# MAC-VO/MAC-VO

Measured on AMD Instinct MI355X. Metric: stereo frames/sec at 640x480 (hot path: cost volume + lookup, keypoint selection, covariance, PGO), higher is better.
Workload: dtype f32 via f16x2 (volume: fp32 operands row-scaled by powers of two and split into two fp16 pieces, three products, fp32 accumulate, scales undone exactly) + f32 (lookup/covariance) + f64 (PGO)

## Files before the change

include/macvo_hip.h:

```cpp
#ifndef MACVO_HIP_H
#define MACVO_HIP_H

#include <stddef.h>
#include <stdint.h>

#ifdef __cplusplus
extern "C" {
#endif

typedef void* mvStream_t;

enum {
    MV_OK = 0,
    MV_ERR_INVALID_ARG = -1,
    MV_ERR_UNSUPPORTED = -2,
    MV_ERR_LAUNCH = -3,
    MV_ERR_WORKSPACE = -4
};

enum {
    MV_F32 = 0,
    MV_F16 = 1,
    MV_BF16 = 2,
    MV_BF16X3 = 3,
// ... 23 lines not shown
int mv_cost_patch_embed_supported(int H2, int W2);
int mv_cost_patch_embed(const float* cost_maps, const void* packed, float* out, int S, int H2, int W2, int token_layout, int operand_type,
                        mvStream_t stream);
int mv_cost_patch_embed_t(const void* cost_maps, int in_dtype, const void* packed, void* out, int out_dtype, int S, int H2, int W2, int token_layout,
                          int operand_type, mvStream_t stream);
size_t mv_volume_pack_bytes(int B, int C, int N, int mode);
int mv_volume_pack(const float* f1, const float* f2, void* packed1, void* packed2, int B, int C, int N1, int N2, int layout,
                   int mode, mvStream_t stream);
int mv_volume_pack_tiled(const float* f1, const float* f2, void* packed1, void* packed2, int B, int C, int N1, int H2, int W2,
                         int layout, int mode, mvStream_t stream);
int mv_corr_volume_packed_supported(int B, int C, int N1, int N2, int mode);
int mv_corr_volume_packed(const void* packed1, const void* packed2, float* out, int B, int C, int N1, int N2, int mode,
                          mvStream_t stream);
int mv_corr_volume_packed_shared(const void* packed1, const void* packed2, float* out, int B, int C, int N1, int N2, int mode, int free_cus,
                                 mvStream_t stream);

const char* mv_corr_volume_last_kernel(void);

int mv_corr_lookup(const float* vol, const float* coords, float* out, int B, int H1, int W1,
                   int H2, int W2, int radius, mvStream_t stream);

int mv_corr_volume_out16_supported(int B, int C, int N1, int N2, int in_dtype, int layout);
int mv_corr_volume_out16(const void* f1, const void* f2, void* out, int B, int C, int N1, int N2, int in_dtype, int layout, mvStream_t stream);
int mv_corr_lookup_vol16(const void* vol_f16, const float* coords, float* out, int B, int H1, int W1, int H2, int W2, int radius,
                         mvStream_t stream);

int mv_corr_lookup_tiled(const float* vol, const float* coords, float* out, int B, int H1, int W1,
                         int H2, int W2, int radius, mvStream_t stream);

int mv_tiled_slice_cells(int H, int W);
int mv_fmap_tile_rows16(const void* f, void* out, int B, int C, int H, int W, mvStream_t stream);
int mv_corr_lookup_tiled_vol16(const void* vol_f16, const float* coords, float* out, int B, int H1, int W1, int H2, int W2, int radius,
                               mvStream_t stream);

int mv_frontend_epilogue(const float* flow, const float* logcov, int cov_is_log, int H, int W,
                         float bl_fx, float bl_fx_sq, float* disparity, float* disparity_cov,
                         float* depth, float* depth_cov, uint8_t* bad_mask, float* match_flow,
                         float* match_cov, mvStream_t stream);

int mv_convex_upsample(const float* flow, const float* mask, float* out, int B, int h, int w,
                       float mask_scale, int exp2_out, mvStream_t stream);
int mv_convex_upsample_m(const float* flow, const void* mask, int mask_dtype, float* out, int B, int h, int w,
                         float mask_scale, int exp2_out, mvStream_t stream);

enum { MV_KP_NODEPTH = 0, MV_KP_FULL = 1, MV_KP_MAPPING = 2,
       MV_KP_RANDOM = 3,
       MV_KP_GRID = 4,
       MV_KP_EXPLICIT = 5
};

typedef struct {
    int32_t H, W;
    int32_t mode;
    int32_t kernel_size;
    int32_t mask_width;
    float max_depth;
    float max_depth_cov;
    float max_match_cov;
} mvKpSelectParams;

size_t mv_kp_select_workspace_bytes(int H, int W);

int mv_kp_select(const float* flow_cov, const float* depth0, const float* depth0_cov,
                 const float* depth1, const float* depth1_cov, const uint8_t* mask_a,
                 const uint8_t* mask_b, const mvKpSelectParams* params , void* workspace,
                 size_t workspace_bytes, int32_t* out_cand, int32_t* out_count, float* out_stats,
// ... 210 lines not shown
    const float *kp0, *kp1;
    const float* vals;
    const float *sigma0, *sigma1;
    const double *cov0, *cov1;
    const float* pos_Tw;
    const double* cov0_world;
    const uint8_t* color;
    const float* K;
    const float* T_BS;
    const float* prior_pose;
    float baseline;
} mvMapFrameLanes;
int mv_map_append_lanes(const mvMapFrameLanes* frames , const mvMapStores* stores_dev , mvStream_t stream);
int mv_map_append_skipped_lanes(const mvMapStores* stores_dev , int lanes, const float* K_dev, const float* T_BS_dev, const float* pose_dev,
                                float baseline, const int64_t* time_ns , mvStream_t stream);
int mv_map_set_pose_lanes(const mvMapStores* stores_dev , int lanes, int frame_idx, const float* pose_dev, mvStream_t stream);

int mv_frontend_epilogue_lanes(const float* flow, const float* logcov, int cov_is_log, int H, int W, float bl_fx,
                               float bl_fx_sq, float* disparity, float* disparity_cov, float* depth, float* depth_cov,
                               uint8_t* bad_mask, float* match_flow, float* match_cov, int lanes, mvStream_t stream);
int mv_kp_select_lanes(const float* flow_cov, const float* depth0, const float* depth0_cov, const float* depth1,
                       const float* depth1_cov, const uint8_t* mask_a, const uint8_t* mask_b,
                       const mvKpSelectParams* params , void* workspace, size_t workspace_bytes,
                       int32_t* out_cand , int32_t* out_count ,
                       float* out_stats , int lanes, mvStream_t stream);
int mv_pose_apply_lanes(const float* pose, const float* pos_Tc, const double* cov, int lanes, const int32_t* n_live ,
                        int cap, float* pos_Tw, double* rot, double* cov_rot, mvStream_t stream);
int mv_frontend_epilogue_select_lanes(const float* flow, const float* logcov, int cov_is_log, float bl_fx, float bl_fx_sq,
                                      float* disparity, float* disparity_cov, float* depth, float* depth_cov,
                                      uint8_t* bad_mask, float* match_flow, float* match_cov, const uint8_t* mask_a,
                                      const uint8_t* mask_b, const mvKpSelectParams* params , void* workspace,
                                      size_t workspace_bytes, int32_t* out_cand, int32_t* out_count, float* out_stats,
                                      int lanes, mvStream_t stream);
int mv_kp_gather_lanes(const int32_t* cand, size_t cand_lane_stride, const int64_t* perm , int lanes,
                       const int32_t* n_live , int cap, int W, int64_t* out_uv ,
                       mvStream_t stream);
int mv_kp_front_lanes(const int32_t* cand, size_t cand_lane_stride, const int64_t* perm_dev, const int64_t* perm_host ,
                      int lanes, const int32_t* n_live , int cap, const float* match_flow, const float* match_cov,
                      const float* depth0, const float* disp0, const float* sdisp0, const float* sdd0, const float* depth1,
                      const float* disp1, const float* sdisp1, const float* sdd1, int H, int W, int edge, float match_cov_default,
                      float fx, float fy, float cx, float cy, int64_t* out_kp0_uv , float* out_kp0,
                      float* out_kp1, uint8_t* out_inbound, float* out_vals , float* out_sigma0,
                      float* out_sigma1, float* out_pos_Tc , mvStream_t stream);
int mv_backend_front_lanes(const int32_t* cand, size_t cand_lane_stride, const int64_t* perm_dev, const int64_t* perm_host, int lanes,
                           const int32_t* n_live, int cap, const float* match_flow, const float* match_cov, const float* depth0,
                           const float* disp0, const float* sdisp0, const float* sdd0, const float* depth1, const float* disp1,
                           const float* sdisp1, const float* sdd1, int edge, float match_cov_default, const mvMatchCovParams* cov_params,
                           int64_t* out_kp0_uv, float* out_kp0, float* out_kp1, uint8_t* out_inbound, float* out_vals, float* out_sigma0,
                           float* out_sigma1, float* out_pos_Tc, double* out_cov0, double* out_cov1, mvStream_t stream);
int mv_backend_front_draw_lanes(const int32_t* cand, size_t cand_lane_stride, const int32_t* count_dev, int count_stride, const uint32_t* state_in,
                                uint32_t* state_out, int num_point, int lanes, int cap, const float* match_flow, const float* match_cov,
                                const float* depth0, const float* disp0, const float* sdisp0, const float* sdd0, const float* depth1,
                                const float* disp1, const float* sdisp1, const float* sdd1, int edge, float match_cov_default,
                                const mvMatchCovParams* cov_params, int64_t* out_perm, int32_t* out_live, int64_t* out_kp0_uv, float* out_kp0,
                                float* out_kp1, uint8_t* out_inbound, float* out_vals, float* out_sigma0, float* out_sigma1, float* out_pos_Tc,
                                double* out_cov0, double* out_cov1, mvStream_t stream);
int mv_kp_track_lanes(const int64_t* kp0_uv, int lanes, const int32_t* n_live , int cap, const float* match_flow,
                      const float* match_cov, const float* depth0, const float* disp0, const float* sdisp0,
                      const float* sdd0, const float* depth1, const float* disp1, const float* sdisp1, const float* sdd1,
                      int H, int W, int edge, float match_cov_default, float* out_kp0, float* out_kp1,
                      uint8_t* out_inbound, float* out_vals , float* out_sigma0, float* out_sigma1,
                      mvStream_t stream);
int mv_backproject_lanes(const float* kp_uv, const float* depth_vals, int depth_stride, size_t depth_lane_stride, float fx,
                         float fy, float cx, float cy, const float* pose, int lanes, const int32_t* n_live ,
                         int cap, float* pos_Tc, float* pos_Tw, double* rot, mvStream_t stream);
int mv_match_cov_pair_lanes(const float* depth_map0, const float* kp_uv0, float* flow_cov0, const double* rot0,
// ... 44 lines not shown
typedef struct {
    const void* fmap1;
    const void* fmap2;
    const float* coords;
    const float* flow;
    const float* logcov;
    const float* flow8;
    const float* cov8;
    const float* up_mask;
    const float* cov_mask;
} mvFrameInputs;

enum {
    MV_FB_VOLUME = 0, MV_FB_TOKENS, MV_FB_DISPARITY, MV_FB_DISPARITY_COV, MV_FB_DEPTH, MV_FB_DEPTH_COV, MV_FB_MATCH_FLOW,
    MV_FB_MATCH_COV, MV_FB_CAND, MV_FB_COUNT, MV_FB_STATS,
    MV_FB_KP0, MV_FB_KP0F, MV_FB_KP1, MV_FB_INBOUND, MV_FB_VALS, MV_FB_SIGMA0, MV_FB_SIGMA1, MV_FB_POS_TC, MV_FB_POS_TW,
    MV_FB_ROT, MV_FB_COV0, MV_FB_COV0W, MV_FB_COV1, MV_FB_VALID, MV_FB_NVALID, MV_FB_POSE64, MV_FB_INFO,
    MV_FB_POSE,
    MV_FB_MAP_UV, MV_FB_MAP_D, MV_FB_MAP_SDD, MV_FB_MAP_TC, MV_FB_MAP_TW, MV_FB_MAP_COV , MV_FB_MAP_COLOR ,
    MV_FB_PERM, MV_FB_LIVE,
    MV_FB_MOTION_IN, MV_FB_PRIOR
};

size_t mv_frame_pipe_arena_bytes(const mvFramePipeConfig* cfg);
int mv_frame_pipe_max_pending(void);
int mv_frame_pipe_default_depth(int lanes, int mapping);
int mv_frame_pipe_create(const mvFramePipeConfig* cfg, void* arena, size_t arena_bytes, mvFramePipe** out);
void mv_frame_pipe_destroy(mvFramePipe* p);
int mv_frame_pipe_set_pose(mvFramePipe* p, const float* pose7_host);
int mv_frame_pipe_enqueue(mvFramePipe* p, const mvFrameInputs* in, mvStream_t in_stream, int with_selector);
int mv_frame_pipe_wait_motion_input(mvFramePipe* p, mvStream_t stream);
int mv_frame_pipe_set_motion(mvFramePipe* p, const float* motion_dev, mvStream_t stream);
int mv_frame_pipe_enqueue_volume(mvFramePipe* p, const mvFrameInputs* in, mvStream_t in_stream);
int mv_frame_pipe_wait_candidates(mvFramePipe* p, int32_t* n_cand );
int mv_frame_pipe_finish(mvFramePipe* p, const int64_t* perm_host, const int32_t* n_sel, float* pose_sink);
int mv_frame_pipe_wait_tracked(mvFramePipe* p, int32_t* n_valid, int32_t* n_cand_map);
int mv_frame_pipe_map_points(mvFramePipe* p, const int64_t* perm_host, int n_sel, const float* image_dev,
                             const mvMapStores* stores );
int mv_frame_pipe_seed_lanes(mvFramePipe* p, const uint64_t* seeds );
int mv_randperm_heads(uint64_t seed, const int64_t* n, int calls, int k, int64_t* out);
int mv_frame_pipe_finish_seeded(mvFramePipe* p, float* pose_sink, int32_t* n_cand_out, int32_t* n_sel_out);
int mv_randperm_state_words(void);
int mv_randperm_max_head(void);
int mv_mt19937_seed(uint64_t seed, uint32_t* state_host);
int mv_randperm_head_lanes(uint32_t* state, const int32_t* n_dev, int n_stride, int lanes, int k, int cap, int64_t* out_perm, int32_t* out_n_sel,
                           int n_sel_stride, mvStream_t stream);
int mv_randperm_heads_emulated(uint64_t seed, const int64_t* n, int calls, int k, int threads, int64_t* out);
int mv_frame_pipe_device_draw(const mvFramePipe* p);
int mv_frame_pipe_volume_tiled(const mvFramePipe* p);
int mv_frame_pipe_host_threads(const mvFramePipe* p);
int mv_frame_pipe_finish_device(mvFramePipe* p, float* pose_sink);
int mv_kp_random_max_point(void);
int mv_kp_random_lanes(uint32_t* state, int lanes, int num_point, int H, int W, int mask_width, int64_t* out_uv, mvStream_t stream);
int mv_kp_random_emulated(uint64_t seed, int calls, int num_point, int H, int W, int mask_width, int threads, int64_t* out);
int mv_kp_random_then_randperm_emulated(uint64_t seed, int calls, int num_point, int H, int W, int mask_width, int threads, int64_t* out, int64_t perm_n,
                                        int perm_k, int64_t* out_perm);
int mv_kp_random_heads(uint64_t seed, int calls, int num_point, int H, int W, int mask_width, int64_t* out);
int mv_kp_grid_count(int H, int W, int mask_width, int num_point);
int mv_kp_grid(int H, int W, int mask_width, int num_point, int64_t* out_uv, mvStream_t stream);
#define MV_KP_TABLE_MAX 4096
int mv_frame_pipe_table_rows(const mvFramePipeConfig* cfg);
int mv_frame_pipe_finish_keypoints(mvFramePipe* p, const int64_t* kp_uv_host, const int32_t* n_sel, float* pose_sink);
int mv_frame_pipe_finish_keypoints_dev(mvFramePipe* p, const int64_t* kp_uv_dev, const int32_t* n_sel_dev, mvStream_t stream, float* pose_sink);
int mv_frame_pipe_finished_counts(mvFramePipe* p, int age, int32_t* n_cand, int32_t* n_sel);
int mv_frame_pipe_wait_finished(mvFramePipe* p, int lag);
int mv_frame_pipe_map_append(mvFramePipe* p, const mvMapStores* stores , int frame_idx, int prev_frame,
// ... 26 lines not shown
```

mac-vo_amd/_lib.py:

```python
from __future__ import annotations

import ctypes as C
import os
import threading

_HERE = os.path.dirname(os.path.abspath(__file__))
LIB_PATH = os.path.join(_HERE, "libmacvo_hip.so")

MV_OK = 0
MV_F32, MV_F16, MV_BF16, MV_BF16X3, MV_BF16X2, MV_PACK_BF16X3, MV_PACK_F16X2 = 0, 1, 2, 3, 4, 5, 6
MV_VOL_ENC16 = 16
MV_LAYOUT_CHW, MV_LAYOUT_HWC = 0, 1
MV_KP_NODEPTH, MV_KP_FULL, MV_KP_MAPPING = 0, 1, 2
MV_KP_RANDOM, MV_KP_GRID, MV_KP_EXPLICIT = 3, 4, 5
MV_KP_TABLE_MAX = 4096
MV_GRAPH_ICP, MV_GRAPH_REPROJ, MV_GRAPH_DISP = 0, 1, 2
MV_COV_MATCH, MV_COV_GMM, MV_COV_NONE = 0, 1, 2
MV_COVMOD_DIAG, MV_COVMOD_NORMALIZE = 1, 2
MV_MOTION_STATIC, MV_MOTION_TARTAN = 0, 1
MV_SOLVE_WORLD, MV_SOLVE_LOCAL = 0, 1
MV_NOCOV_DEPTH, MV_NOCOV_MATCH = 1, 2
ABI_VERSION = 8
MV_MAX_LANES = 64

# ... 27 lines not shown

class mvFramePipeConfig(C.Structure):
    _fields_ = [(n, C.c_int32) for n in (
        "H", "W", "C", "pairs", "iters", "radius", "feat_dtype", "layout", "volume_split", "selector_mode",
        "kp_kernel_size", "kp_mask_width", "num_point", "edgewidth", "min_num_point", "graph_type", "filters",
        "cov_kernel_size", "mapping", "map_num_point", "map_mask_width", "async_backend")] + [(n, C.c_float) for n in (
        "fx", "fy", "cx", "cy", "baseline", "bl_fx", "bl_fx_sq", "match_cov_default", "max_match_cov", "max_depth_cov",
        "max_depth", "min_flow_cov_sq", "min_depth_cov", "filter_min_depth", "map_max_depth", "map_max_depth_cov")] + [("lm", mvLMParams)] + [
        (n, C.c_int32) for n in ("cov_model", "cov_modifiers", "motion_model", "frontend_nocov")] + [("cov_match_cov_default", C.c_float)]


class mvMapStores(C.Structure):
    _fields_ = [(n, C.c_void_p) for n in (
        "K", "baseline", "pose", "T_BS", "need_interp", "time_ns", "pos_Tw", "cov_Tw", "color",
        "pixel1_uv", "pixel2_uv", "pixel1_d", "pixel2_d", "pixel1_disp", "pixel2_disp", "pixel1_disp_cov", "pixel2_disp_cov",
        "obs1_covTc", "obs2_covTc", "pixel1_uv_cov", "pixel2_uv_cov", "pixel1_d_cov", "pixel2_d_cov",
        "frame2match_ranges", "frame2match_num", "frame2map_ranges", "frame2map_num", "match2frame1", "match2frame2",
        "match2point", "point2match_edges", "point2match_deg", "counts")] + [("max_pt_obs", C.c_int32), ("max_frame_range", C.c_int32)] + \
        [("cap_frames", C.c_int64), ("cap_match", C.c_int64), ("cap_points", C.c_int64)] + \
        [("mp_pos_Tw", C.c_void_p), ("mp_cov_Tw", C.c_void_p), ("mp_color", C.c_void_p), ("cap_map_points", C.c_int64)]


class mvMapFrame(C.Structure):
    _fields_ = [("n_rows", C.c_int32), ("table_stride", C.c_int32), ("prev_frame", C.c_int32), ("min_num_point", C.c_int32)] + \
        [(n, C.c_void_p) for n in ("valid", "kp0", "kp1", "vals", "sigma0", "sigma1", "cov0", "cov1", "pos_Tw", "cov0_world",
                                   "color", "K", "T_BS", "prior_pose")] + \
        [("baseline", C.c_float), ("time_ns", C.c_int64), ("out_frame_idx", C.c_void_p)]


class mvMapFrameLanes(C.Structure):
    _fields_ = [("lanes", C.c_int32), ("cap", C.c_int32), ("prev_frame", C.c_int32), ("min_num_point", C.c_int32)] + \
        [(n, C.c_void_p) for n in ("n_rows", "time_ns", "valid", "kp0", "kp1", "vals", "sigma0", "sigma1", "cov0", "cov1", "pos_Tw", "cov0_world",
                                   "color", "K", "T_BS", "prior_pose")] + [("baseline", C.c_float)]


class mvFrameInputs(C.Structure):
    _fields_ = [(n, C.c_void_p) for n in ("fmap1", "fmap2", "coords", "flow", "logcov", "flow8", "cov8", "up_mask",
                                          "cov_mask")]


FB_NAMES = ("VOLUME", "TOKENS", "DISPARITY", "DISPARITY_COV", "DEPTH", "DEPTH_COV", "MATCH_FLOW", "MATCH_COV", "CAND",
            "COUNT", "STATS", "KP0", "KP0F", "KP1", "INBOUND", "VALS", "SIGMA0", "SIGMA1", "POS_TC", "POS_TW", "ROT", "COV0",
            "COV0W", "COV1", "VALID", "NVALID", "POSE64", "INFO", "POSE", "MAP_UV", "MAP_D", "MAP_SDD", "MAP_TC", "MAP_TW", "MAP_COV",
            "MAP_COLOR", "PERM", "LIVE", "MOTION_IN", "PRIOR")
FB = {n: i for i, n in enumerate(FB_NAMES)}

_P = C.c_void_p
SIGNATURES = {
    "mv_abi_version": (C.c_int, []),
    "mv_error_string": (C.c_char_p, [C.c_int]),
    "mv_corr_volume": (C.c_int, [_P, _P, _P, C.c_int, C.c_int, C.c_int, C.c_int, C.c_int, C.c_int, _P]),
    "mv_split_bf16x3": (C.c_int, [_P, _P, C.c_size_t, _P]),
    "mv_corr_volume_last_kernel": (C.c_char_p, []),
    "mv_volume_pack_bytes": (C.c_size_t, [C.c_int, C.c_int, C.c_int, C.c_int]),
    "mv_volume_pack": (C.c_int, [_P, _P, _P, _P, C.c_int, C.c_int, C.c_int, C.c_int, C.c_int, C.c_int, _P]),
    "mv_corr_volume_packed_supported": (C.c_int, [C.c_int, C.c_int, C.c_int, C.c_int, C.c_int]),
    "mv_corr_volume_packed": (C.c_int, [_P, _P, _P, C.c_int, C.c_int, C.c_int, C.c_int, C.c_int, _P]),
    "mv_corr_volume_packed_shared": (C.c_int, [_P, _P, _P, C.c_int, C.c_int, C.c_int, C.c_int, C.c_int, C.c_int, _P]),
    "mv_corr_lookup": (C.c_int, [_P, _P, _P, C.c_int, C.c_int, C.c_int, C.c_int, C.c_int, C.c_int, _P]),
    "mv_corr_lookup_tiled": (C.c_int, [_P, _P, _P, C.c_int, C.c_int, C.c_int, C.c_int, C.c_int, C.c_int, _P]),
    "mv_corr_lookup_vol16": (C.c_int, [_P, _P, _P, C.c_int, C.c_int, C.c_int, C.c_int, C.c_int, C.c_int, _P]),
    "mv_corr_lookup_tiled_vol16": (C.c_int, [_P, _P, _P, C.c_int, C.c_int, C.c_int, C.c_int, C.c_int, C.c_int, _P]),
    "mv_fmap_tile_rows16": (C.c_int, [_P, _P, C.c_int, C.c_int, C.c_int, C.c_int, _P]),
    "mv_tiled_slice_cells": (C.c_int, [C.c_int, C.c_int]),
    "mv_corr_volume_out16_supported": (C.c_int, [C.c_int, C.c_int, C.c_int, C.c_int, C.c_int, C.c_int]),
    "mv_corr_volume_out16": (C.c_int, [_P, _P, _P, C.c_int, C.c_int, C.c_int, C.c_int, C.c_int, C.c_int, _P]),
    "mv_volume_pack_tiled": (C.c_int, [_P, _P, _P, _P, C.c_int, C.c_int, C.c_int, C.c_int, C.c_int, C.c_int, C.c_int, _P]),
    "mv_frontend_epilogue": (C.c_int, [_P, _P, C.c_int, C.c_int, C.c_int, C.c_float, C.c_float,
                                       _P, _P, _P, _P, _P, _P, _P, _P]),
    "mv_convex_upsample": (C.c_int, [_P, _P, _P, C.c_int, C.c_int, C.c_int, C.c_float, C.c_int, _P]),
    "mv_convex_upsample_m": (C.c_int, [_P, _P, C.c_int, _P, C.c_int, C.c_int, C.c_int, C.c_float, C.c_int, _P]),
    "mv_kp_select_workspace_bytes": (C.c_size_t, [C.c_int, C.c_int]),
    "mv_kp_select": (C.c_int, [_P, _P, _P, _P, _P, _P, _P, C.POINTER(mvKpSelectParams), _P, C.c_size_t,
                               _P, _P, _P, _P]),
    "mv_kp_gather": (C.c_int, [_P, _P, C.c_int, C.c_int, _P, _P]),
    "mv_kp_track": (C.c_int, [_P, C.c_int, _P, _P, _P, _P, _P, _P, _P, _P, _P, _P, C.c_int, C.c_int, C.c_int,
                              C.c_float, _P, _P, _P, _P, _P, _P, _P]),
    "mv_match_cov": (C.c_int, [_P, _P, _P, _P, _P, C.POINTER(mvMatchCovParams), C.c_int, _P, _P, _P, _P]),
    "mv_match_cov_pair": (C.c_int, [_P, _P, _P, _P, _P, _P, _P, _P, _P, _P, C.POINTER(mvMatchCovParams), C.c_int, _P]),
    "mv_obs_cov": (C.c_int, [C.c_int, C.c_int32, _P, _P, _P, _P, _P, _P, C.POINTER(mvMatchCovParams), C.c_int, _P, _P, _P, _P]),
    "mv_obs_cov_pair_lanes": (C.c_int, [C.c_int, C.c_int32] + [_P] * 12 + [C.POINTER(mvMatchCovParams), C.c_int, _P, C.c_int, _P]),
    "mv_obs_cov_pair_nomatch_lanes": (C.c_int, [C.c_int, C.c_int32] + [_P] * 11 + [C.c_float, _P, C.POINTER(mvMatchCovParams), C.c_int, _P, C.c_int, _P]),
    "mv_motion_input_lanes": (C.c_int, [C.c_int, C.c_int, C.c_int, _P, C.c_longlong, _P, C.c_longlong] + [C.c_float] * 5 + [_P, _P]),
    "mv_pose_exp_compose": (C.c_int, [C.c_int, _P, _P, C.c_longlong, _P, _P, _P]),
    "mv_pgo_solve_posed_motion": (C.c_int, [C.c_int, _P, _P, C.c_int, C.c_int] + [_P] * 15 + [C.c_int, C.c_float, C.c_float, _P, _P, _P, _P, C.c_int,
                                                                                         C.POINTER(mvLMParams)] + [_P] * 5),
    "mv_pgo_solve_posed_motion_dev": (C.c_int, [C.c_int, _P, _P, C.c_int, C.c_int, C.c_int] + [_P] * 15 + [C.c_int, C.c_float, C.c_float, _P, _P, _P, _P,
                                                                                                         C.c_int, C.POINTER(mvLMParams)] + [_P] * 5),
    "mv_frame_pipe_wait_motion_input": (C.c_int, [_P, _P]),
    "mv_frame_pipe_set_motion": (C.c_int, [_P, _P, _P]),
    "mv_lm_default_params": (None, [C.POINTER(mvLMParams)]),
    "mv_pgo_solve": (C.c_int, [C.c_int, _P, C.c_int, _P, _P, _P, _P, _P, _P, _P, _P, _P, _P, _P, _P, C.c_int,
                               C.POINTER(mvLMParams), _P, _P, _P, _P]),
    "mv_pgo_solve_posed": (C.c_int, [C.c_int, _P, _P, C.c_int, C.c_int] + [_P] * 14 + [C.c_int, C.c_float, C.c_float, _P, _P, _P, _P, C.c_int,
                                     C.POINTER(mvLMParams)] + [_P] * 5),
    "mv_pgo_solve_posed_dev": (C.c_int, [C.c_int, _P, _P, C.c_int, C.c_int, C.c_int] + [_P] * 14 + [C.c_int, C.c_float, C.c_float, _P, _P, _P, _P, C.c_int,
                                         C.POINTER(mvLMParams)] + [_P] * 5),
    "mv_pgo_solve_local": (C.c_int, [C.c_int, _P, C.c_int, _P, _P, _P, _P, _P, _P, _P, _P, _P, _P, _P, _P, _P, C.c_int,
                                     C.POINTER(mvLMParams), _P, _P, _P, _P]),
    "mv_pgo_solve_posed_local": (C.c_int, [C.c_int, _P, _P, C.c_int, C.c_int] + [_P] * 16 + [C.c_int, C.c_float, C.c_float, _P, _P, _P, _P, C.c_int,
                                           C.POINTER(mvLMParams)] + [_P] * 5),
    "mv_pgo_solve_posed_local_dev": (C.c_int, [C.c_int, _P, _P, C.c_int, C.c_int, C.c_int] + [_P] * 16 + [C.c_int, C.c_float, C.c_float, _P, _P, _P, _P, C.c_int,
                                               C.POINTER(mvLMParams)] + [_P] * 5),
    "mv_backend_front_draw_lanes": (C.c_int, [_P, C.c_size_t, _P, C.c_int, _P, _P, C.c_int, C.c_int, C.c_int] + [_P] * 10 +
                                    [C.c_int, C.c_float, C.POINTER(mvMatchCovParams)] + [_P] * 13),
    "mv_backend_front_lanes": (C.c_int, [_P, C.c_size_t, _P, _P, C.c_int, _P, C.c_int] + [_P] * 10 + [C.c_int, C.c_float, C.POINTER(mvMatchCovParams)] +
                               [_P] * 11),
    "mv_backproject": (C.c_int, [_P, _P, C.c_int, C.c_float, C.c_float, C.c_float, C.c_float, _P, C.c_int,
                                 _P, _P, _P, _P]),
    "mv_obs_filter": (C.c_int, [_P, _P, _P, _P, C.c_int, C.c_float, C.c_float, C.c_int, _P, _P, _P]),
    "mv_map_points": (C.c_int, [_P, C.c_int, _P, _P, _P, C.c_int, C.c_int, C.c_float, C.c_float, C.c_float, C.c_float, _P,
                                C.c_float, _P, _P, _P, _P, _P, _P, _P, _P]),
    "mv_local_corr81": (C.c_int, [_P, _P, _P, C.c_int, C.c_int, C.c_int, C.c_int, _P]),
    "mv_map_append": (C.c_int, [C.POINTER(mvMapFrame), C.POINTER(mvMapStores), _P]),
    "mv_body_poses": (C.c_int, [_P, _P, C.c_int, _P, _P]),
    "mv_motion_interpolate": (C.c_int, [_P, _P, C.c_int, _P, _P, _P]),
    "mv_frontend_epilogue_lanes": (C.c_int, [_P, _P, C.c_int, C.c_int, C.c_int, C.c_float, C.c_float,
                                             _P, _P, _P, _P, _P, _P, _P, C.c_int, _P]),
    "mv_pose_apply_lanes": (C.c_int, [_P, _P, _P, C.c_int, _P, C.c_int, _P, _P, _P, _P]),
    "mv_frontend_epilogue_select_lanes": (C.c_int, [_P, _P, C.c_int, C.c_float, C.c_float, _P, _P, _P, _P, _P, _P, _P, _P, _P,
                                                    C.POINTER(mvKpSelectParams), _P, C.c_size_t, _P, _P, _P, C.c_int, _P]),
    "mv_kp_select_lanes": (C.c_int, [_P, _P, _P, _P, _P, _P, _P, C.POINTER(mvKpSelectParams), _P, C.c_size_t,
                                     _P, _P, _P, C.c_int, _P]),
    "mv_kp_gather_lanes": (C.c_int, [_P, C.c_size_t, _P, C.c_int, _P, C.c_int, C.c_int, _P, _P]),
    "mv_kp_track_lanes": (C.c_int, [_P, C.c_int, _P, C.c_int, _P, _P, _P, _P, _P, _P, _P, _P, _P, _P, C.c_int, C.c_int,
                                    C.c_int, C.c_float, _P, _P, _P, _P, _P, _P, _P]),
    "mv_backproject_lanes": (C.c_int, [_P, _P, C.c_int, C.c_size_t, C.c_float, C.c_float, C.c_float, C.c_float, _P,
                                       C.c_int, _P, C.c_int, _P, _P, _P, _P]),
    "mv_match_cov_pair_lanes": (C.c_int, [_P, _P, _P, _P, _P, _P, _P, _P, _P, _P, C.POINTER(mvMatchCovParams), C.c_int, _P,
                                          C.c_int, _P]),
    "mv_obs_filter_lanes": (C.c_int, [_P, _P, _P, _P, C.c_int, C.c_float, C.c_float, C.c_int, _P, C.c_int, _P, _P, _P]),
    "mv_patch_embed_packed_bytes": (C.c_size_t, []),
    "mv_patch_embed_pack": (C.c_int, [_P, _P, _P, _P, _P, _P, _P, C.c_int, _P]),
    "mv_cost_patch_embed_supported": (C.c_int, [C.c_int, C.c_int]),
    "mv_cost_patch_embed": (C.c_int, [_P, _P, _P, C.c_int, C.c_int, C.c_int, C.c_int, C.c_int, _P]),
    "mv_cost_patch_embed_t": (C.c_int, [_P, C.c_int, _P, _P, C.c_int, C.c_int, C.c_int, C.c_int, C.c_int, C.c_int, _P]),
    "mv_frame_pipe_arena_bytes": (C.c_size_t, [C.POINTER(mvFramePipeConfig)]),
    "mv_frame_pipe_max_pending": (C.c_int, []),
    "mv_frame_pipe_default_depth": (C.c_int, [C.c_int, C.c_int]),
    "mv_frame_pipe_create": (C.c_int, [C.POINTER(mvFramePipeConfig), _P, C.c_size_t, C.POINTER(_P)]),
    "mv_frame_pipe_destroy": (None, [_P]),
    "mv_frame_pipe_set_pose": (C.c_int, [_P, _P]),
    "mv_frame_pipe_enqueue": (C.c_int, [_P, C.POINTER(mvFrameInputs), _P, C.c_int]),
    "mv_frame_pipe_enqueue_volume": (C.c_int, [_P, C.POINTER(mvFrameInputs), _P]),
    "mv_frame_pipe_wait_candidates": (C.c_int, [_P, _P]),
    "mv_frame_pipe_finish": (C.c_int, [_P, _P, _P, _P]),
    "mv_map_append_points": (C.c_int, [_P, C.c_int, _P, _P, _P, _P]),
    "mv_map_append_skipped": (C.c_int, [C.POINTER(mvMapStores), _P, _P, _P, C.c_float, C.c_int64, _P]),
    "mv_frame_pipe_set_solve_frame": (C.c_int, [_P, C.c_int]),
    "mv_frame_pipe_skip": (C.c_int, [_P]),
    "mv_frame_pipe_map_skip": (C.c_int, [_P, C.POINTER(mvMapStores), C.c_int, _P, _P, C.c_float, C.c_int64]),
    "mv_kp_front_lanes": (C.c_int, [_P, C.c_size_t, _P, _P, C.c_int, _P, C.c_int] + [_P] * 10 + [C.c_int, C.c_int, C.c_int] +
                          [C.c_float] * 5 + [_P] * 8 + [_P]),
    "mv_frame_pipe_wait_tracked": (C.c_int, [_P, _P, _P]),
    "mv_frame_pipe_map_points": (C.c_int, [_P, _P, C.c_int, _P, _P]),
    "mv_frame_pipe_seed_lanes": (C.c_int, [_P, _P]),
    "mv_frame_pipe_finish_seeded": (C.c_int, [_P, _P, _P, _P]),
    "mv_frame_pipe_map_append": (C.c_int, [_P, C.POINTER(mvMapStores), C.c_int, C.c_int, _P, _P, C.c_float, C.c_int64, _P]),
    "mv_frame_pipe_release": (C.c_int, [_P, _P]),
    "mv_frame_pipe_sync": (C.c_int, [_P, _P, C.c_int]),
    "mv_frame_pipe_time_volume": (C.c_int, [_P, C.c_int]),
    "mv_frame_pipe_volume_times": (C.c_int, [_P, _P, C.c_int, C.POINTER(C.c_int)]),
    "mv_frame_pipe_volume_starts": (C.c_int, [_P, _P, C.c_int, C.POINTER(C.c_int)]),
    "mv_frame_pipe_time_detail": (C.c_int, [_P, C.c_int]),
    "mv_randperm_heads": (C.c_int, [C.c_uint64, _P, C.c_int, C.c_int, _P]),
    "mv_frame_pipe_device_draw": (C.c_int, [_P]),
    "mv_frame_pipe_volume_tiled": (C.c_int, [_P]),
    "mv_frame_pipe_host_threads": (C.c_int, [_P]),
    "mv_frame_pipe_finish_device": (C.c_int, [_P, _P]),
    "mv_frame_pipe_finished_counts": (C.c_int, [_P, C.c_int, _P, _P]),
    "mv_frame_pipe_wait_finished": (C.c_int, [_P, C.c_int]),
    "mv_randperm_state_words": (C.c_int, []),
    "mv_randperm_max_head": (C.c_int, []),
    "mv_mt19937_seed": (C.c_int, [C.c_uint64, _P]),
    "mv_randperm_head_lanes": (C.c_int, [_P, _P, C.c_int, C.c_int, C.c_int, C.c_int, _P, _P, C.c_int, _P]),
    "mv_randperm_heads_emulated": (C.c_int, [C.c_uint64, _P, C.c_int, C.c_int, C.c_int, _P]),
    "mv_kp_random_max_point": (C.c_int, []),
# ... 65 lines not shown
```

mac-vo_amd/csrc/corr_lookup.hip:

```cpp
#include "common.h"

namespace {

struct AxisEntry { float w; int c; };

template <int K, int QPW, int STRIDE, int CELLS>
__device__ __forceinline__ void tap_pairs(const float* blk, const AxisEntry (*ax)[2 * K], int lane, float (&res)[(QPW * K * K + 63) / 64]) {
    constexpr int KK = K * K, NPAIR = QPW * KK, NR = (NPAIR + 63) / 64;
#pragma unroll
    for (int r = 0; r < NR; ++r) {
        const int pair = min(r * 64 + lane, NPAIR - 1);
        const int s = pair / KK, tap = pair - s * KK;
        const int ti = tap / K, tj = tap - ti * K;
        const AxisEntry X = ax[s][ti], Y = ax[s][K + tj];
        const float w = X.w, n = Y.w;
        const bool inblk = ((X.c & Y.c) & 256) != 0;
        const float* p = &blk[s * CELLS + (Y.c & 255) * STRIDE + (X.c & 255)];
        const float e = 1.f - w, so = 1.f - n;
        const float vnw = inblk ? p[0] : 0.f, vne = inblk ? p[1] : 0.f;
        const float vsw = inblk ? p[STRIDE] : 0.f, vse = inblk ? p[STRIDE + 1] : 0.f;
        float r0 = vnw * (so * e);
        r0 = r0 + vne * (so * w);
        r0 = r0 + vsw * (n * e);
        r0 = r0 + vse * (n * w);
        res[r] = r0;
    }
}

template <int K, int QPW, int QPB>
__device__ __forceinline__ void tap_pairs_out(float (*outs)[QPB + 1], int wave, int lane, const float (&res)[(QPW * K * K + 63) / 64]) {
    constexpr int KK = K * K, NPAIR = QPW * KK, NR = (NPAIR + 63) / 64;
#pragma unroll
    for (int r = 0; r < NR; ++r) {
        const int pair = r * 64 + lane;
        if (pair < NPAIR) {
            const int s = pair / KK, tap = pair - s * KK;
            outs[tap][wave * QPW + s] = res[r];
        }
    }
}

template <int R, int QPW, int QPB, typename VT = float>
__global__ __launch_bounds__(64 * (QPB / QPW)) void corr_lookup_kernel(const VT* __restrict__ vol,
                                                                        const float* __restrict__ coords,
                                                                        float* __restrict__ out, int N1, int H2, int W2) {
    constexpr int K = 2 * R + 1;
    constexpr int KK = K * K;
    constexpr int BS = K + 3;
    constexpr int CELLS = BS * BS;
    constexpr int NWAVE = QPB / QPW;
    constexpr int NTHR = 64 * NWAVE;
    constexpr int RPR = 64 / BS;
    constexpr int LPR = RPR * BS;
    constexpr int NROUND = (BS + RPR - 1) / RPR;
    constexpr bool TRIM = (BS - 2) % RPR == 0;
    constexpr int NINNER = (BS - 2) / RPR;
    constexpr int QPA = 64 / (2 * K);
    constexpr int APASS = (QPW + QPA - 1) / QPA;
    static_assert(QPW <= 32 && (QPW & (QPW - 1)) == 0 && QPB % QPW == 0, "bad lookup tiling");

    constexpr int BLK_STRIDE = QPW * CELLS;
    constexpr int BLK_FLOATS = NWAVE * BLK_STRIDE;
    constexpr int OUT_FLOATS = KK * (QPB + 1);
    __shared__ float smem[BLK_FLOATS > OUT_FLOATS ? BLK_FLOATS : OUT_FLOATS];
    float* blk = smem + (threadIdx.x >> 6) * BLK_STRIDE;
    float (*outs)[QPB + 1] = reinterpret_cast<float (*)[QPB + 1]>(smem);

    MV_SMALL_KERNEL_PRIO();
    const int b = blockIdx.y;
    const int q0 = blockIdx.x * QPB;
    const int t = threadIdx.x, lane = t & 63, wave = t >> 6;
    const int slice = H2 * W2;

    const int qmine = q0 + wave * QPW + (lane & (QPW - 1));
    float x = 0.f, y = 0.f;
    if (qmine < N1) {
        x = coords[((size_t)b * 2 + 0) * N1 + qmine];
        y = coords[((size_t)b * 2 + 1) * N1 + qmine];
    }
    const float xc = fminf(fmaxf(x, -1.0e6f), 1.0e6f), yc = fminf(fmaxf(y, -1.0e6f), 1.0e6f);
    const int bx = ((xc == xc) ? (int)floorf(xc) : 0) - R - 1;
    const int by = ((yc == yc) ? (int)floorf(yc) : 0) - R - 1;
    const float frx = xc - floorf(xc), fry = yc - floorf(yc);
    const int margin = ((frx < 0.01f) ? 1 : 0) | ((frx > 0.99f) ? 2 : 0) | ((fry < 0.01f) ? 4 : 0) | ((fry > 0.99f) ? 8 : 0);

    const int cyl = lane / BS, cxl = lane - cyl * BS;
    float v[QPW][NROUND];
#pragma unroll
    for (int s = 0; s < QPW; ++s) {
        const int sbx = __builtin_amdgcn_readlane(bx, s), sby = __builtin_amdgcn_readlane(by, s);
        const int q = q0 + wave * QPW + s;
        const VT* __restrict__ base = vol + ((size_t)b * N1 + q) * slice;
        const int gx = sbx + cxl;
        if (TRIM) {
            const int mg = __builtin_amdgcn_readlane(margin, s);
            const bool okx = lane < LPR && q < N1 && gx >= 0 && gx < W2 && (cxl != 0 || (mg & 1)) && (cxl != BS - 1 || (mg & 2));
#pragma unroll
            for (int k = 0; k < NINNER; ++k) {
                const int row = 1 + k * RPR + cyl, gy = sby + row;
                const bool ok = okx && gy >= 0 && gy < H2;
                v[s][k] = ok ? (float)base[gy * W2 + gx] : 0.f;
            }
// ... 36 lines not shown
    }

#pragma unroll
    for (int s = 0; s < QPW; ++s) {
        if (TRIM) {
#pragma unroll
            for (int k = 0; k < NINNER; ++k)
                if (lane < LPR) blk[s * CELLS + BS + k * LPR + lane] = v[s][k];
            if (lane < 2 * BS) blk[s * CELLS + (lane < BS ? lane : (BS - 2) * BS + lane)] = v[s][NROUND - 1];
        } else {
#pragma unroll
            for (int k = 0; k < NROUND; ++k)
                if (lane < LPR && k * LPR + lane < CELLS) blk[s * CELLS + k * LPR + lane] = v[s][k];
        }
    }
    __syncthreads();

    float res[(QPW * KK + 63) / 64];
    tap_pairs<K, QPW, BS, CELLS>(blk, ax, lane, res);
    __syncthreads();
    tap_pairs_out<K, QPW, QPB>(outs, wave, lane, res);
    __syncthreads();

    for (int idx = t; idx < KK * QPB; idx += NTHR) {
        const int k = idx / QPB, c = idx - k * QPB;
        if (q0 + c < N1) out[((size_t)b * KK + k) * N1 + q0 + c] = outs[k][c];
    }
}


template <int QPW, int QPB, typename VT = float>
__global__ __launch_bounds__(64 * (QPB / QPW)) void corr_lookup_tiled_kernel(const VT* __restrict__ vol,
                                                                              const float* __restrict__ coords,
                                                                              float* __restrict__ out, int N1, int H2, int W2) {
    constexpr int R = 4, K = 9, KK = 81;
    constexpr int BS = 16;
    constexpr int BSP = 18, CELLS = BS * BSP;
    constexpr int NWAVE = QPB / QPW, NTHR = 64 * NWAVE;
    constexpr int QPA = 64 / (2 * K);
    constexpr int APASS = (QPW + QPA - 1) / QPA;
    constexpr int BLK_STRIDE = QPW * CELLS;
    constexpr int BLK_FLOATS = NWAVE * BLK_STRIDE;
    constexpr int OUT_FLOATS = KK * (QPB + 1);
    __shared__ float smem[BLK_FLOATS > OUT_FLOATS ? BLK_FLOATS : OUT_FLOATS];
    float* blk = smem + (threadIdx.x >> 6) * BLK_STRIDE;
    float (*outs)[QPB + 1] = reinterpret_cast<float (*)[QPB + 1]>(smem);

    MV_SMALL_KERNEL_PRIO();
    const int b = blockIdx.y;
    const int q0 = blockIdx.x * QPB;
    const int t = threadIdx.x, lane = t & 63, wave = t >> 6;
    const int tpr = W2 >> 2, tpc = (H2 + 3) >> 2, slice = tpc * tpr * 16;

    const int qmine = q0 + wave * QPW + (lane & (QPW - 1));
    float x = 0.f, y = 0.f;
    if (qmine < N1) {
        x = coords[((size_t)b * 2 + 0) * N1 + qmine];
        y = coords[((size_t)b * 2 + 1) * N1 + qmine];
    }
    const float xc = fminf(fmaxf(x, -1.0e6f), 1.0e6f), yc = fminf(fmaxf(y, -1.0e6f), 1.0e6f);
    const int bx = ((xc == xc) ? (int)floorf(xc) : 0) - R - 1;
    const int by = ((yc == yc) ? (int)floorf(yc) : 0) - R - 1;
    const float frx = xc - floorf(xc), fry = yc - floorf(yc);
    const int x_lo = bx + ((frx < 0.01f) ? 0 : 1), x_hi = bx + ((frx > 0.99f) ? K + 2 : K + 1);
    const int y_lo = by + ((fry < 0.01f) ? 0 : 1), y_hi = by + ((fry > 0.99f) ? K + 2 : K + 1);
    const int tox = bx >> 2, toy = by >> 2;

    constexpr bool H16 = sizeof(VT) == 2;
    constexpr int NLD = H16 ? 2 : 4;
    const int ti = H16 ? (lane >> 3) & 3 : lane >> 4, cell = H16 ? (lane & 7) * 2 : lane & 15;
    const int half_row = H16 ? lane >> 5 : 0;
    float v[QPW][4];
#pragma unroll
    for (int s = 0; s < QPW; ++s) {
        const int stx = __builtin_amdgcn_readlane(tox, s), sty = __builtin_amdgcn_readlane(toy, s);
        const int sxl = __builtin_amdgcn_readlane(x_lo, s), sxh = __builtin_amdgcn_readlane(x_hi, s);
        const int syl = __builtin_amdgcn_readlane(y_lo, s), syh = __builtin_amdgcn_readlane(y_hi, s);
        const int q = q0 + wave * QPW + s;
        const VT* __restrict__ base = vol + ((size_t)b * N1 + q) * slice;
        const int tx = stx + ti;
        const bool okx = q < N1 && tx >= 0 && tx < tpr && 4 * tx + 3 >= sxl && 4 * tx <= sxh;
#pragma unroll
// ... 37 lines not shown
#pragma unroll
        for (int k = 0; k < NLD; ++k) {
            if constexpr (H16)
                *reinterpret_cast<float2*>(&blk[s * CELLS + (4 * (2 * k + half_row) + (cell >> 2)) * BSP + 4 * ti + (cell & 3)]) =
                    make_float2(v[s][2 * k], v[s][2 * k + 1]);
            else
                blk[s * CELLS + (4 * k + (cell >> 2)) * BSP + 4 * ti + (cell & 3)] = v[s][k];
        }
    __syncthreads();

    float res[(QPW * KK + 63) / 64];
    tap_pairs<K, QPW, BSP, CELLS>(blk, ax, lane, res);
    __syncthreads();
    tap_pairs_out<K, QPW, QPB>(outs, wave, lane, res);
    __syncthreads();
    for (int idx = t; idx < KK * QPB; idx += NTHR) {
        const int k = idx / QPB, c = idx - k * QPB;
        if (q0 + c < N1) out[((size_t)b * KK + k) * N1 + q0 + c] = outs[k][c];
    }
}

}

#include <stdlib.h>
static int lookup_small_threshold() {
    static int v = -1;
    if (v < 0) {
        const char* e = getenv("MV_LOOKUP_SMALL");
        v = e ? atoi(e) : 65536;
    }
    return v;
}

extern "C" int mv_corr_lookup(const float* vol, const float* coords, float* out, int B, int H1, int W1,
                              int H2, int W2, int radius, mvStream_t stream) {
    MV_CHECK_ARG(vol && coords && out);
    MV_CHECK_ARG(B > 0 && H1 > 0 && W1 > 0 && H2 > 1 && W2 > 1);
    if (radius < 1 || radius > 4) return MV_ERR_UNSUPPORTED;
    if (B > 65535) return MV_ERR_UNSUPPORTED;
    const int N1 = H1 * W1;
    hipStream_t s = (hipStream_t)stream;
    const bool small = (size_t)B * N1 <= (size_t)lookup_small_threshold();
    static int small_qpb = -1;
    if (small_qpb < 0) { const char* e = getenv("MV_LOOKUP_QPB"); small_qpb = (e && atoi(e) == 8) ? 8 : 16; }
#define MV_LOOKUP(R)                                                                                                  \
    if (small && small_qpb == 8)                                                                                      \
        hipLaunchKernelGGL((corr_lookup_kernel<R, 2, 8>), dim3(mv_ceil_div(N1, 8), B), dim3(256), 0, s, vol, coords,  \
                           out, N1, H2, W2);                                                                          \
    else if (small)                                                                                                   \
        hipLaunchKernelGGL((corr_lookup_kernel<R, 2, 16>), dim3(mv_ceil_div(N1, 16), B), dim3(512), 0, s, vol, coords, \
                           out, N1, H2, W2);                                                                          \
    else                                                                                                              \
        hipLaunchKernelGGL((corr_lookup_kernel<R, 4, 32>), dim3(mv_ceil_div(N1, 32), B), dim3(512), 0, s, vol, coords, \
                           out, N1, H2, W2)
    switch (radius) {
        case 1: MV_LOOKUP(1); break;
        case 2: MV_LOOKUP(2); break;
        case 3: MV_LOOKUP(3); break;
        default: MV_LOOKUP(4); break;
    }
#undef MV_LOOKUP
    return mv_launch_status();
}

extern "C" int mv_corr_lookup_vol16(const void* vol, const float* coords, float* out, int B, int H1, int W1, int H2, int W2, int radius,
                                    mvStream_t stream) {
    MV_CHECK_ARG(vol && coords && out);
    MV_CHECK_ARG(B > 0 && H1 > 0 && W1 > 0 && H2 > 1 && W2 > 1);
    if (radius != 4 || B > 65535) return MV_ERR_UNSUPPORTED;
    const int N1 = H1 * W1;
    hipStream_t s = (hipStream_t)stream;
    const _Float16* v = reinterpret_cast<const _Float16*>(vol);
    if ((size_t)B * N1 <= (size_t)lookup_small_threshold())
        hipLaunchKernelGGL((corr_lookup_kernel<4, 2, 16, _Float16>), dim3(mv_ceil_div(N1, 16), B), dim3(512), 0, s, v, coords, out, N1, H2, W2);
    else
        hipLaunchKernelGGL((corr_lookup_kernel<4, 4, 32, _Float16>), dim3(mv_ceil_div(N1, 32), B), dim3(512), 0, s, v, coords, out, N1, H2, W2);
    return mv_launch_status();
}

extern "C" int mv_corr_lookup_tiled(const float* vol, const float* coords, float* out, int B, int H1, int W1, int H2, int W2,
                                    int radius, mvStream_t stream) {
    MV_CHECK_ARG(vol && coords && out);
    MV_CHECK_ARG(B > 0 && H1 > 0 && W1 > 0 && H2 > 1 && W2 > 1);
    if (radius != 4 || (H2 % 4) || (W2 % 4) || B > 65535) return MV_ERR_UNSUPPORTED;
    const int N1 = H1 * W1;
    hipStream_t s = (hipStream_t)stream;
    if ((size_t)B * N1 <= (size_t)lookup_small_threshold())
        hipLaunchKernelGGL((corr_lookup_tiled_kernel<2, 16>), dim3(mv_ceil_div(N1, 16), B), dim3(512), 0, s, vol, coords, out, N1, H2, W2);
    else
        hipLaunchKernelGGL((corr_lookup_tiled_kernel<4, 32>), dim3(mv_ceil_div(N1, 32), B), dim3(512), 0, s, vol, coords, out, N1, H2, W2);
    return mv_launch_status();
}


extern "C" int mv_corr_lookup_tiled_vol16(const void* vol, const float* coords, float* out, int B, int H1, int W1, int H2, int W2, int radius,
                                          mvStream_t stream) {
    MV_CHECK_ARG(vol && coords && out);
    MV_CHECK_ARG(B > 0 && H1 > 0 && W1 > 0 && H2 > 1 && W2 > 1);
    MV_CHECK_ARG(((uintptr_t)vol & 31) == 0);
    if (radius != 4 || (W2 % 4) || B > 65535) return MV_ERR_UNSUPPORTED;
    const int N1 = H1 * W1;
    hipStream_t s = (hipStream_t)stream;
    const _Float16* v = reinterpret_cast<const _Float16*>(vol);
    if ((size_t)B * N1 <= (size_t)lookup_small_threshold())
        hipLaunchKernelGGL((corr_lookup_tiled_kernel<2, 16, _Float16>), dim3(mv_ceil_div(N1, 16), B), dim3(512), 0, s, v, coords, out, N1, H2, W2);
    else
        hipLaunchKernelGGL((corr_lookup_tiled_kernel<4, 32, _Float16>), dim3(mv_ceil_div(N1, 32), B), dim3(512), 0, s, v, coords, out, N1, H2, W2);
    return mv_launch_status();
}

namespace {
__global__ __launch_bounds__(256) void fmap_tile_rows16_kernel(const uint4* __restrict__ f, uint4* __restrict__ out, int H, int W, int n_out, int cpr, size_t total) {
    const int tpr = W >> 2;
    const size_t n_in = (size_t)H * W;
    for (size_t i = (size_t)blockIdx.x * blockDim.x + threadIdx.x; i < total; i += (size_t)gridDim.x * blockDim.x) {
        const size_t rowi = i / cpr;
        const int ch = (int)(i - rowi * cpr);
        const size_t b = rowi / n_out;
        const int j = (int)(rowi - b * n_out);
        const int tile = j >> 4, cell = j & 15;
        const int ty = tile / tpr, tx = tile - ty * tpr;
        const int y = 4 * ty + (cell >> 2);
        out[i] = y < H ? f[(b * n_in + (size_t)y * W + 4 * tx + (cell & 3)) * cpr + ch] : make_uint4(0u, 0u, 0u, 0u);
    }
}
}

extern "C" int mv_tiled_slice_cells(int H, int W) { return (H > 0 && W > 0 && (W % 4) == 0) ? ((H + 3) / 4) * 4 * W : 0; }

extern "C" int mv_fmap_tile_rows16(const void* f, void* out, int B, int C, int H, int W, mvStream_t stream) {
    MV_CHECK_ARG(f && out && f != out && B > 0 && C > 0 && H > 0 && W > 0);
    MV_CHECK_ARG(((uintptr_t)f & 15) == 0 && ((uintptr_t)out & 15) == 0);
    if ((C % 8) || (W % 4)) return MV_ERR_UNSUPPORTED;
    const int cpr = C / 8, n_out = mv_tiled_slice_cells(H, W);
    const size_t total = (size_t)B * n_out * cpr;
    const int blocks = (int)((total + 255) / 256 < 8192 ? (total + 255) / 256 : 8192);
    hipLaunchKernelGGL(fmap_tile_rows16_kernel, dim3(blocks), dim3(256), 0, (hipStream_t)stream, (const uint4*)f, (uint4*)out, H, W, n_out, cpr, total);
    return mv_launch_status();
}
```

mac-vo_amd/csrc/frame_pipe.hip:

```cpp
#include "common.h"
#include "motion_dev.h"
#include "kp_draw_dev.h"
#include <atomic>
#include <chrono>
#include <stdio.h>
#include <condition_variable>
#include <deque>
#include <mutex>
#include <random>
#include <thread>
#include <vector>
#include <new>
#include <stdlib.h>
#include <string.h>
#if defined(__linux__)
#include <sched.h>
#endif

#define MV_HIP(call)                                   \
    do {                                               \
        if ((call) != hipSuccess) return MV_ERR_LAUNCH; \
    } while (0)
#define MV_TRY(call)               \
    do {                           \
        const int rc_ = (call);    \
        if (rc_ != MV_OK) return rc_; \
    } while (0)

namespace {

#ifndef MV_MAX_PENDING
#define MV_MAX_PENDING 3
#endif
constexpr int MAX_PENDING = MV_MAX_PENDING, N_MAPS = MAX_PENDING + 2, N_CAND = MAX_PENDING + 1, N_PERM = 4, N_INEV = 8, MAX_VOL = 4, MAX_LK = 2;
constexpr int N_MOT = 8;
constexpr int N_BEV = 8;

inline bool kp_new_mode(int m) { return m == MV_KP_RANDOM || m == MV_KP_GRID || m == MV_KP_EXPLICIT; }
inline int frame_rows(const mvFramePipeConfig& c) {
    return c.selector_mode == MV_KP_GRID ? mvkp::grid_of(c.H, c.W, c.kp_mask_width, c.num_point, nullptr) : c.num_point;
}
inline int table_rows(const mvFramePipeConfig& c) {
    const int g = frame_rows(c);
    return g > c.num_point ? g : c.num_point;
}
inline int cap_of(const mvFramePipeConfig& c) {
    const int r = table_rows(c);
    return r > 0 ? r : 1;
}
enum { KPJ_PERM = 0, KPJ_HOST = 1, KPJ_DEV = 2, KPJ_RANDOM = 3, KPJ_GRID = 4 };

struct Maps {
    float *disparity, *disparity_cov, *depth, *depth_cov, *match_flow, *match_cov;
    uint8_t* bad_mask;
    mvDepthMaps dm;
};

struct Backend {
    int64_t *perm, *kp0;
    float *kp0f, *kp1, *vals, *sigma0, *sigma1, *pos_Tc, *pos_Tw;
    uint8_t *inbound, *valid;
    double *rot, *cov0, *cov0w, *cov1, *pose64, *info;
    int32_t* n_valid;
    int32_t* live_dev;
    int32_t n_sel[MV_MAX_LANES];
    mvFrontTables front;
    mvPosedSolve solve;
};
// ... 27 lines not shown
    const int64_t* kp_dev = nullptr;
    const int32_t* nsel_dev = nullptr;
    bool device = false;
    std::vector<int64_t> perm;
    float* pose_sink;
    double t_count = 0, t_submit = 0;
    bool has_sel;
    SelSeg sel;
};

struct Carver {
    char* base;
    size_t off = 0;
    template <typename T>
    T* take(size_t n) {
        off = (off + 255) & ~(size_t)255;
        T* p = base ? reinterpret_cast<T*>(base + off) : nullptr;
        off += n * sizeof(T);
        return p;
    }
};

}

struct mvFramePipe {
    mvFramePipeConfig c;
    int plane, h8, w8, n8, KK;
    int lanes;
    char* arena;
    size_t arena_bytes;
    float* vol[MAX_VOL];
    int n_volbuf;
    float* tok[2 * MAX_LK];
    void* planes[2];
    void* pk[2][2];
    int n2t;
    void* tile16;
    size_t pk_bytes;
    bool packed;
    bool vol16;
    bool tiled;
    int pack_on;
    int sel_on_back;
    hipEvent_t e_lk[N_CAND];
    hipEvent_t e_packed[2];
    float *up_flow, *up_cov;
    Maps maps[N_MAPS];
    void* kp_ws;
    size_t kp_ws_bytes;
    int32_t* cand[N_CAND];
    int32_t* count[N_CAND];
    float* stats[N_CAND];
    Backend be[2];
    mvCovConfig cov;
    float* pose[3];
    float *intr, *bl;
    int32_t* offs;
    int fuse_backend;
    int32_t* h_count[N_CAND];
    int64_t* h_perm[N_PERM];
    hipStream_t s_vol, s_main, s_back, s_side;
    hipStream_t s_lk[MAX_LK];
    int n_lk;
    int alt;
    int free_cus;
    hipEvent_t e_seg[N_INEV];
    bool seg_valid[N_INEV];
    int alt_indep;
    void* kp_ws2;
    int lean_chain;
    bool cand_recorded[N_CAND];
    hipEvent_t vol_free_ev[MAX_VOL];
    int front_on_decoder;

    hipStream_t s_sel;
    SelSeg deferred;
    bool deferred_valid;
    hipEvent_t e_rest[N_INEV];
    hipEvent_t e_in[N_INEV], e_vol_done[MAX_VOL], e_vol_free[MAX_VOL], e_cand[N_CAND], e_backend[N_BEV], e_pgo, e_perm[N_PERM];
    hipEvent_t e_kpin[N_BEV];
    hipEvent_t e_release;
    bool release_valid;
    hipEvent_t e_posed[2];
    hipEvent_t e_solved[2];
    bool vol_free_valid[MAX_VOL], backend_valid[N_BEV], pgo_valid, perm_valid[N_PERM], solved_valid[2];
    long n_enq, n_fin;
    long n_vol;
    hipEvent_t e_in_of[MAX_VOL];
    int lookups_on_main;
    int pose_cur;
    int prior_slot;
    int solve_frame = MV_SOLVE_WORLD;
    bool skipped = false;
    hipEvent_t e_map;
    hipEvent_t e_mapl[2];
    bool mapl_valid[2];
    int newest_maps;
    std::deque<Pending> pending;
    int32_t* cand_m[N_CAND];
    int32_t* count_m[N_CAND];
    float* stats_m[N_CAND];
    int32_t* h_count_m[N_CAND];
// ... 45 lines not shown
    float* pose_norm;
    hipEvent_t e_motion_set[N_MOT], e_motion_used[N_MOT];
    bool motion_used_valid[N_MOT];
    long motion_g[N_MOT];
};

static int wait_if_pending(hipStream_t s, hipEvent_t e) {
    const hipError_t q = hipEventQuery(e);
    if (q == hipSuccess) return MV_OK;
    if (q != hipErrorNotReady) return MV_ERR_LAUNCH;
    return hipStreamWaitEvent(s, e, 0) == hipSuccess ? MV_OK : MV_ERR_LAUNCH;
}

static int affinity_cores() {
#if defined(__linux__)
    cpu_set_t set;
    CPU_ZERO(&set);
    if (sched_getaffinity(0, sizeof(set), &set) == 0) return CPU_COUNT(&set);
#endif
    const unsigned n = std::thread::hardware_concurrency();
    return n ? (int)n : 1;
}

static inline double now_us() {
    return std::chrono::duration<double, std::micro>(std::chrono::steady_clock::now().time_since_epoch()).count();
}

#define MV_ASYNC_DEFAULT(p) (1)
static int wait_issued(mvFramePipe* p, long n);
static int flush_deferred(mvFramePipe* p);
static int issue_selector_segment(mvFramePipe* p, const SelSeg& d);
static int flush_jobs(mvFramePipe* p);
static void launch_thread_main(mvFramePipe* p);

static int layout_alt(int lanes, int mapping) {
    const char* e = getenv("MV_PIPE_LAYOUT");
    if (e && strcmp(e, "classic") == 0) return 0;
    const char* lk = getenv("MV_PIPE_LOOKUPS_ON");
    if (lanes > 2 || mapping || (lk && strcmp(lk, "vol") == 0) || getenv("MV_PIPE_SELECTOR_ON")) return 0;
    return 1;
}

extern "C" int mv_frame_pipe_default_depth(int lanes, int mapping) { return (lanes > 2 || layout_alt(lanes, mapping)) ? 3 : 2; }

static int volbufs_for(int lanes, int mapping) {
    return layout_alt(lanes, mapping) ? 4 : 3;
}

static size_t carve(mvFramePipe* p, char* base) {
    const mvFramePipeConfig& c = p->c;
    Carver a{base};
    const size_t L = p->lanes;
    const size_t plane = p->plane, n8 = p->n8, B = c.pairs, N = (size_t)cap_of(c);
    for (int k = 0; k < p->n_volbuf; ++k) p->vol[k] = a.take<float>(B * n8 * n8);
    for (int k = 0; k < 2 * (L <= 2 ? MAX_LK : 1); ++k) p->tok[k] = a.take<float>(B * p->KK * n8);
    for (int k = 0; k < 2; ++k)
        p->planes[k] = (c.volume_split == 2 || c.volume_split == 3) ? (void*)a.take<uint16_t>(3 * B * n8 * c.C) : nullptr;
    p->pk_bytes = p->packed ? mv_volume_pack_bytes((int)B, c.C, (int)n8, c.volume_split) : 0;
    for (int k = 0; k < 2; ++k)
        for (int o = 0; o < 2; ++o) p->pk[k][o] = p->packed ? (void*)a.take<char>(p->pk_bytes) : nullptr;
    p->tile16 = (c.volume_split == MV_VOL_ENC16 && c.radius == 4 && p->w8 % 4 == 0) ? (void*)a.take<uint16_t>(B * (size_t)mv_tiled_slice_cells(p->h8, p->w8) * c.C) : nullptr;
    const bool no_d = (c.frontend_nocov & MV_NOCOV_DEPTH) != 0, no_m = (c.frontend_nocov & MV_NOCOV_MATCH) != 0;
    p->up_flow = a.take<float>(B * 2 * plane);
    p->up_cov = (no_d && no_m) ? nullptr : a.take<float>(B * 2 * plane);
    for (int k = 0; k < N_MAPS; ++k) {
        Maps& m = p->maps[k];
        m.disparity = a.take<float>(L * plane);
        m.disparity_cov = no_d ? nullptr : a.take<float>(L * plane);
        m.depth = a.take<float>(L * plane);
        m.depth_cov = no_d ? nullptr : a.take<float>(L * plane);
        m.match_flow = a.take<float>(L * 2 * plane);
        m.match_cov = no_m ? nullptr : a.take<float>(L * 3 * plane);
        m.bad_mask = a.take<uint8_t>(L * plane);
    }
    p->kp_ws_bytes = L * mv_kp_select_workspace_bytes(c.H, c.W);
    p->kp_ws = a.take<char>(p->kp_ws_bytes);
    p->kp_ws2 = L <= 2 ? a.take<char>(p->kp_ws_bytes) : nullptr;

    for (int k = 0; k < N_CAND; ++k) {
        p->cand[k] = a.take<int32_t>(L * plane);
        p->count[k] = a.take<int32_t>(L * 4);
        p->stats[k] = a.take<float>(L * 4);
    }
    for (int k = 0; k < 2; ++k) {
        Backend& b = p->be[k];
        b.perm = a.take<int64_t>(L * N);
        b.kp0 = a.take<int64_t>(L * 2 * N);
        b.kp0f = a.take<float>(L * 2 * N);
        b.kp1 = a.take<float>(L * 2 * N);
        b.vals = a.take<float>(L * 11 * N);
        b.sigma0 = a.take<float>(L * 3 * N);
        b.sigma1 = a.take<float>(L * 3 * N);
        b.pos_Tc = a.take<float>(L * 3 * N);
        b.pos_Tw = a.take<float>(L * 3 * N);
        b.inbound = a.take<uint8_t>(L * N);
        b.valid = a.take<uint8_t>(L * N);
        b.rot = a.take<double>(L * 9);
        b.cov0 = a.take<double>(L * 9 * N);
        b.cov0w = a.take<double>(L * 9 * N);
        b.cov1 = a.take<double>(L * 9 * N);
        b.pose64 = a.take<double>(L * 7);
        b.info = a.take<double>(L * 4);
        b.n_valid = a.take<int32_t>(L);
        b.live_dev = a.take<int32_t>(2 * L);
    }
    for (int k = 0; k < 2; ++k) p->rp_state[k] = a.take<uint32_t>(L * (size_t)mv_randperm_state_words());
    if (c.mapping) {
        const size_t MP = c.map_num_point > 0 ? c.map_num_point : 1;
        for (int k = 0; k < N_CAND; ++k) {
            p->cand_m[k] = a.take<int32_t>(plane);
// ... 193 lines not shown
        for (auto& e : p->e_motion_used) MV_HIP(mk(&e));
    }
    for (auto& g : p->motion_g) g = -1;
    for (int k = 0; k < 2; ++k) {
        MV_HIP(mk(&p->e_posed[k]));
        MV_HIP(mk(&p->e_solved[k]));
    }
    MV_HIP(mk(&p->e_pgo));
    for (int k = 0; k < N_CAND; ++k) MV_HIP(mk(&p->e_lk[k]));
    for (auto& e : p->e_seg) MV_HIP(mk(&e));
    MV_HIP(mk(&p->e_maptail));
    for (int k = 0; k < 2; ++k) {
        MV_HIP(mk(&p->e_nvalid[k]));
        MV_HIP(hipHostMalloc((void**)&p->h_nvalid[k], (size_t)p->lanes * sizeof(int32_t), hipHostMallocDefault));
    }
    if (c.mapping) {
        for (int k = 0; k < N_CAND; ++k) MV_HIP(hipHostMalloc((void**)&p->h_count_m[k], 4 * sizeof(int32_t), hipHostMallocDefault));
        MV_HIP(hipHostMalloc((void**)&p->h_perm_m, (size_t)c.map_num_point * sizeof(int64_t), hipHostMallocDefault));
    }
    MV_HIP(mk(&p->e_packed[0]));
    MV_HIP(mk(&p->e_packed[1]));
    MV_HIP(mk(&p->e_map));
    for (int k = 0; k < 2; ++k) {
        MV_HIP(mk(&p->e_mapl[k]));
        p->mapl_valid[k] = false;
    }
    MV_HIP(mk(&p->e_release));
    const size_t N = (size_t)cap_of(c);
    for (int k = 0; k < N_PERM; ++k) {
        MV_HIP(mk(&p->e_perm[k]));
        MV_HIP(hipHostMalloc((void**)&p->h_perm[k], (size_t)p->lanes * N * 2 * sizeof(int64_t), hipHostMallocDefault));
    }
    MV_HIP(hipMemsetAsync(p->kp_ws, 0, p->kp_ws_bytes, p->s_main));
    if (p->kp_ws2) MV_HIP(hipMemsetAsync(p->kp_ws2, 0, p->kp_ws_bytes, p->s_main));
    const int L = p->lanes;
    std::vector<float> ident((size_t)L * 7, 0.f), intr((size_t)L * 4), bl((size_t)L, c.baseline);
    std::vector<int32_t> offs((size_t)L + 1);
    for (int l = 0; l < L; ++l) {
        ident[7 * l + 6] = 1.f;
        intr[4 * l] = c.fx; intr[4 * l + 1] = c.fy; intr[4 * l + 2] = c.cx; intr[4 * l + 3] = c.cy;
    }
    for (int l = 0; l <= L; ++l) offs[l] = (int32_t)(l * N);
    MV_HIP(hipMemcpyAsync(p->pose[0], ident.data(), ident.size() * sizeof(float), hipMemcpyHostToDevice, p->s_main));
    MV_HIP(hipMemcpyAsync(p->intr, intr.data(), intr.size() * sizeof(float), hipMemcpyHostToDevice, p->s_main));
    MV_HIP(hipMemcpyAsync(p->bl, bl.data(), bl.size() * sizeof(float), hipMemcpyHostToDevice, p->s_main));
    MV_HIP(hipMemcpyAsync(p->offs, offs.data(), offs.size() * sizeof(int32_t), hipMemcpyHostToDevice, p->s_main));
    static const float pose_norm[6] = {0.13f, 0.13f, 0.13f, 0.013f, 0.013f, 0.013f};
    if (p->pose_norm) MV_HIP(hipMemcpyAsync(p->pose_norm, pose_norm, sizeof(pose_norm), hipMemcpyHostToDevice, p->s_main));
    { const char* e = getenv("MV_PIPE_FUSE_BACKEND"); p->fuse_backend = (e && atoi(e) == 0) ? 0 : 1; }
    p->time_detail = 1;
    MV_HIP(hipStreamSynchronize(p->s_main));
    return MV_OK;
}

extern "C" int mv_frame_pipe_create(const mvFramePipeConfig* cfg, void* arena, size_t arena_bytes, mvFramePipe** out) {
    MV_CHECK_ARG(out && arena);
    MV_TRY(check_config(cfg));
    mvFramePipe* p = new (std::nothrow) mvFramePipe{};
    if (!p) return MV_ERR_WORKSPACE;
    p->c = *cfg;
    p->plane = cfg->H * cfg->W;
    p->h8 = cfg->H / 8;
    p->w8 = cfg->W / 8;
    p->n8 = p->h8 * p->w8;
    p->KK = (2 * cfg->radius + 1) * (2 * cfg->radius + 1);
    p->lanes = cfg->pairs / 2;
    p->n_volbuf = volbufs_for(p->lanes, cfg->mapping);
    p->packed = (cfg->volume_split == MV_PACK_BF16X3 || cfg->volume_split == MV_PACK_F16X2) &&
                mv_corr_volume_packed_supported(cfg->pairs, cfg->C, p->n8, p->n8, cfg->volume_split);
    p->vol16 = cfg->volume_split == MV_VOL_ENC16 && mv_corr_volume_out16_supported(cfg->pairs, cfg->C, p->n8, p->n8, cfg->feat_dtype, cfg->layout);
    {
        const char* e = getenv("MV_PIPE_TILED");
        const bool want = e ? atoi(e) != 0 : p->vol16;
        p->tiled = want && cfg->radius == 4 && (p->w8 % 4) == 0 &&
                   (p->vol16 ? mv_corr_volume_out16_supported(cfg->pairs, cfg->C, p->n8, mv_tiled_slice_cells(p->h8, p->w8), cfg->feat_dtype, cfg->layout) != 0
                             : (p->packed && (p->h8 % 4) == 0));
        p->n2t = (p->tiled && p->vol16) ? mv_tiled_slice_cells(p->h8, p->w8) : p->n8;
    }
    {
        const char* e = getenv("MV_PIPE_SELECTOR_ON");
        p->sel_on_back = e ? (strcmp(e, "back") == 0 ? 1 : strcmp(e, "own") == 0 ? 2 : strcmp(e, "vol") == 0 ? 3 : strcmp(e, "late") == 0 ? 4 : 0)
                           : (p->lanes <= 2 ? 1 : 0);
    }
    {
        const char* e = getenv("MV_PIPE_PACK_ON");
        p->pack_on = (e && strcmp(e, "back") == 0) ? 1 : (e && strcmp(e, "main") == 0) ? 2 : (e && strcmp(e, "side") == 0) ? 3 : 0;
    }
    p->arena = (char*)arena;
    p->arena_bytes = arena_bytes;
    if (((uintptr_t)arena & 255) != 0 || carve(p, p->arena) > arena_bytes) {
        delete p;
        return MV_ERR_WORKSPACE;
    }
    describe_backend(p);
    p->newest_maps = -1;
    for (auto& r : p->cand_recorded) r = true;
    {
        const char* e = getenv("MV_PIPE_LOOKUPS_ON");
        p->lookups_on_main = (e && strcmp(e, "vol") == 0) ? 0 : 1;
    }
    {
        p->alt = layout_alt(p->lanes, cfg->mapping);
        p->n_lk = p->alt ? 2 : 1;
        if (p->alt) p->sel_on_back = 0;
        p->free_cus = p->alt ? 32 : 0;
        if (const char* e = getenv("MV_PIPE_FREE_CUS")) p->free_cus = atoi(e);
        p->alt_indep = p->alt;
        { const char* e = getenv("MV_PIPE_LEAN"); p->lean_chain = (p->alt && !(e && atoi(e) == 0)) ? 1 : 0; }
        { const char* e = getenv("MV_PIPE_FRONT_ON"); p->front_on_decoder = (p->alt && !(e && strcmp(e, "side") == 0)) ? 1 : 0; }
    }
    const int rc = create_impl(p);
    if (rc != MV_OK) {
        mv_frame_pipe_destroy(p);
        return rc;
    }
    {
        const char* e = getenv("MV_PIPE_ASYNC_BACKEND");
        const int want = cfg->async_backend ? cfg->async_backend : (e ? (atoi(e) ? 1 : -1) : MV_ASYNC_DEFAULT(p));
        p->async_backend = want > 0 ? 1 : 0;
        p->async_explicit = (cfg->async_backend || e) ? 1 : 0;
        if (hipGetDevice(&p->device) != hipSuccess) p->async_backend = 0;
        {
            const char* e3 = getenv("MV_PIPE_LAUNCH_SPIN_US");
            p->spin_us = e3 ? atof(e3) : (affinity_cores() >= 3 ? 250.0 : 0.0);
        }
        { const char* e4 = getenv("MV_PIPE_HOST_STATS"); p->host_stats = e4 ? atoi(e4) : 0; }
        if (p->async_backend) p->worker = std::thread(launch_thread_main, p);
    }
    *out = p;
    return MV_OK;
}

extern "C" int mv_frame_pipe_set_pose(mvFramePipe* p, const float* pose7_host) {
    MV_CHECK_ARG(p && pose7_host);
    MV_TRY(flush_jobs(p));
    if (p->pgo_valid) MV_HIP(hipEventSynchronize(p->e_pgo));
    MV_HIP(hipMemcpy(p->pose[p->pose_cur], pose7_host, (size_t)p->lanes * 7 * sizeof(float), hipMemcpyHostToDevice));
    return MV_OK;
}

typedef int (*mvLookupFn)(const float*, const float*, float*, int, int, int, int, int, int, mvStream_t);
static int lookup_vol16_as_float_ptr(const float* vol, const float* coords, float* out, int B, int H1, int W1, int H2, int W2, int radius, mvStream_t s) {
    return mv_corr_lookup_vol16(vol, coords, out, B, H1, W1, H2, W2, radius, s);
}
static int lookup_tiled_vol16_as_float_ptr(const float* vol, const float* coords, float* out, int B, int H1, int W1, int H2, int W2, int radius, mvStream_t s) {
    return mv_corr_lookup_tiled_vol16(vol, coords, out, B, H1, W1, H2, W2, radius, s);
}
static mvLookupFn lookup_of(const mvFramePipe* p) {
    if (p->vol16) return p->tiled ? lookup_tiled_vol16_as_float_ptr : lookup_vol16_as_float_ptr;
    return p->tiled ? mv_corr_lookup_tiled : mv_corr_lookup;
}

static int issue_volume(mvFramePipe* p, const mvFrameInputs* in, mvStream_t in_stream) {
    const mvFramePipeConfig& c = p->c;
    const long f = p->n_vol;
    const int k = (int)(f % p->n_volbuf);
    const int B = c.pairs;
    hipEvent_t e_in = p->e_in[f % N_INEV];
    MV_HIP(hipEventRecord(e_in, (hipStream_t)in_stream));
    p->e_in_of[k] = e_in;
    MV_TRY(wait_if_pending(p->s_vol, e_in));
    if (p->vol_free_valid[k]) MV_TRY(wait_if_pending(p->s_vol, p->vol_free_ev[k] ? p->vol_free_ev[k] : p->e_vol_free[k]));
    const bool timed = p->n_timed < p->timed_cap;
    if (timed && !p->packed) MV_HIP(hipEventRecord(p->tv0[p->n_timed], p->s_vol));
    if (p->packed) {
        void** pk = p->pk[f & 1];
        hipStream_t sp = p->pack_on == 0 ? p->s_vol : p->pack_on == 1 ? p->s_back : p->pack_on == 2 ? p->s_main : p->s_side;
        if (sp != p->s_vol) {
            MV_TRY(wait_if_pending(sp, e_in));
            if (f >= 2) MV_TRY(wait_if_pending(sp, p->e_vol_done[(f - 2) % p->n_volbuf]));
        }
        if (p->tiled)
            MV_TRY(mv_volume_pack_tiled((const float*)in->fmap1, (const float*)in->fmap2, pk[0], pk[1], B, c.C, p->n8, p->h8, p->w8,
                                        c.layout, c.volume_split, sp));
        else
            MV_TRY(mv_volume_pack((const float*)in->fmap1, (const float*)in->fmap2, pk[0], pk[1], B, c.C, p->n8, p->n8, c.layout,
                                  c.volume_split, sp));
        if (sp != p->s_vol) {
            MV_HIP(hipEventRecord(p->e_packed[f & 1], sp));
            MV_HIP(hipStreamWaitEvent(p->s_vol, p->e_packed[f & 1], 0));
        }
        if (timed) MV_HIP(hipEventRecord(p->tv0[p->n_timed], p->s_vol));
        MV_TRY(mv_corr_volume_packed_shared(pk[0], pk[1], p->vol[k], B, c.C, p->n8, p->n8, c.volume_split, p->free_cus, p->s_vol));
    } else if (c.volume_split == 2 || c.volume_split == 3) {
        const size_t nel = (size_t)B * p->n8 * c.C;
        MV_TRY(mv_split_bf16x3((const float*)in->fmap1, p->planes[0], nel, p->s_vol));
        MV_TRY(mv_split_bf16x3((const float*)in->fmap2, p->planes[1], nel, p->s_vol));
        MV_TRY(mv_corr_volume(p->planes[0], p->planes[1], p->vol[k], B, c.C, p->n8, p->n8,
                              c.volume_split == 2 ? MV_BF16X2 : MV_BF16X3, MV_LAYOUT_HWC, p->s_vol));
    } else if (p->vol16) {
        const void* op2 = in->fmap2;
        if (p->tiled) {
            MV_TRY(mv_fmap_tile_rows16(in->fmap2, p->tile16, B, c.C, p->h8, p->w8, p->s_vol));
            op2 = p->tile16;
        }
        MV_TRY(mv_corr_volume_out16(in->fmap1, op2, p->vol[k], B, c.C, p->n8, p->n2t, c.feat_dtype, c.layout, p->s_vol));
    } else {
        MV_TRY(mv_corr_volume(in->fmap1, in->fmap2, p->vol[k], B, c.C, p->n8, p->n8, c.feat_dtype, c.layout, p->s_vol));
    }
    p->vol_timed[k] = timed ? p->n_timed : -1;
    if (timed) MV_HIP(hipEventRecord(p->tv1[p->n_timed++], p->s_vol));
    MV_HIP(hipEventRecord(p->e_vol_done[k], p->s_vol));
    p->n_vol = f + 1;
    return MV_OK;
}

extern "C" int mv_frame_pipe_enqueue_volume(mvFramePipe* p, const mvFrameInputs* in, mvStream_t in_stream) {
    MV_CHECK_ARG(p && in && in->fmap1 && in->fmap2);
    MV_CHECK_ARG(p->n_vol == p->n_enq);
    MV_CHECK_ARG(p->lookups_on_main);
    const double t_hs = p->host_stats ? now_us() : 0.0;
    MV_TRY(issue_volume(p, in, in_stream));
    if (p->host_stats) p->st_vol += now_us() - t_hs;
    return p->sel_on_back == 3 ? flush_deferred(p) : MV_OK;
}

static int ensure_chain_events(mvFramePipe* p, long f, int cand_slot) {
    if (cand_slot >= 0 && !p->cand_recorded[cand_slot]) {
        MV_HIP(hipEventRecord(p->e_cand[cand_slot], p->s_lk[f % p->n_lk]));
        p->cand_recorded[cand_slot] = true;
    }
    if (p->alt && f >= 0 && !p->seg_valid[f % N_INEV]) {
        MV_HIP(hipEventRecord(p->e_seg[f % N_INEV], p->s_lk[f % p->n_lk]));
        p->seg_valid[f % N_INEV] = true;
    }
    return MV_OK;
}

static int issue_motion_input(mvFramePipe* p, int m, hipStream_t s) {
    const mvFramePipeConfig& c = p->c;
    if (p->motion_read_valid[m]) MV_TRY(wait_if_pending(s, p->e_motion_read[m]));
    const Maps& mp = p->maps[m];
    MV_TRY(mv_motion_input_lanes(p->lanes, c.H, c.W, mp.match_flow, 2LL * p->plane, mp.depth, (long long)p->plane, c.fx, c.fy, c.cx, c.cy, c.bl_fx,
                                 p->motion_in[m], s));
    MV_HIP(hipEventRecord(p->e_motion_in[m], s));
    p->motion_in_valid[m] = true;
    return MV_OK;
}

static int issue_selector_segment(mvFramePipe* p, const SelSeg& d) {
    const mvFramePipeConfig& c = p->c;
    const mvFrameInputs* in = &d.in;
    const int k = d.k, m = d.m, ti = d.ti, B = c.pairs;
    const bool timed = d.timed, with_selector = d.with_selector, up = d.up;
    hipStream_t s = p->s_lk[d.f % p->n_lk];
    if (p->sel_on_back) {
        s = p->sel_on_back == 2 ? p->s_sel : p->sel_on_back == 3 ? p->s_vol : p->s_back;
        MV_HIP(hipStreamWaitEvent(s, p->e_lk[k], 0));
    }
    if (p->async_backend) {
        if (!with_selector) MV_TRY(flush_jobs(p));
        long issued;
        {
            const long need = d.need_issued;
            MV_TRY(wait_issued(p, need < 0 ? 0 : need));
            std::lock_guard<std::mutex> lk(p->mu);
            issued = p->issued;
        }
        const long w = p->dev_draw ? d.need_issued - 1 : issued - 1;
        if (w >= 0 && w < issued) MV_TRY(wait_if_pending(s, p->e_backend[w % N_BEV]));
    } else if (p->n_fin > 0) {
        const long w = p->dev_draw ? d.need_issued - 1 : p->n_fin - 1;
        if (w >= 0 && p->backend_valid[w % N_BEV]) MV_TRY(wait_if_pending(s, p->e_backend[w % N_BEV]));
    }
    if (p->release_valid) MV_TRY(wait_if_pending(s, p->e_release));
    const bool indep = p->alt_indep && !up && (c.selector_mode == MV_KP_NODEPTH || kp_new_mode(c.selector_mode));
    if (p->alt && !indep && d.f > 0) {
        MV_TRY(ensure_chain_events(p, d.f - 1, -1));
        MV_TRY(wait_if_pending(s, p->e_seg[(d.f - 1) % N_INEV]));
    }
    void* const kp_ws = (indep && (d.f & 1)) ? p->kp_ws2 : p->kp_ws;
    Maps& mp = p->maps[m];
    constexpr bool fuse_epi = true;
    const int nocov = c.frontend_nocov;
    if (up) {
        MV_TRY(mv_convex_upsample(in->flow8, in->up_mask, p->up_flow, B, p->h8, p->w8, 0.25f, 0, s));
        if (!nocov) {
            MV_TRY(mv_convex_upsample(in->cov8, in->cov_mask, p->up_cov, B, p->h8, p->w8, 1.0f, 1, s));
        } else if (nocov != (MV_NOCOV_DEPTH | MV_NOCOV_MATCH)) {
            for (int l = 0; l < p->lanes; ++l) {
                const size_t pr = 2 * (size_t)l + ((nocov & MV_NOCOV_DEPTH) ? 1 : 0);
                MV_TRY(mv_convex_upsample(in->cov8 + pr * 2 * p->n8, in->cov_mask + pr * 576 * p->n8, p->up_cov + pr * 2 * p->plane, 1, p->h8, p->w8,
                                          1.0f, 1, s));
            }
        }
        MV_TRY(mv_frontend_epilogue_lanes(p->up_flow, p->up_cov, 0, c.H, c.W, c.bl_fx, c.bl_fx_sq, mp.disparity,
                                          mp.disparity_cov, mp.depth, mp.depth_cov, nullptr, mp.match_flow, mp.match_cov,
                                          p->lanes, s));
    } else if (nocov || !(fuse_epi && with_selector && c.selector_mode == MV_KP_NODEPTH)) {
        MV_TRY(mv_frontend_epilogue_lanes(in->flow, in->logcov, 1, c.H, c.W, c.bl_fx, c.bl_fx_sq, mp.disparity,
                                          mp.disparity_cov, mp.depth, mp.depth_cov, nullptr, mp.match_flow, mp.match_cov,
                                          p->lanes, s));
    }
    const Pending pd{m, d.maps_prev, k, with_selector, ti};
    if (with_selector && c.motion_model == MV_MOTION_TARTAN && !(c.selector_mode == MV_KP_NODEPTH && fuse_epi && !up && !nocov)) MV_TRY(issue_motion_input(p, m, s));
    if (with_selector) {
        mvKpSelectParams sp{c.H, c.W, c.selector_mode, c.kp_kernel_size, c.kp_mask_width, c.max_depth, c.max_depth_cov,
                            c.max_match_cov};
        const bool sel_kernels = !kp_new_mode(c.selector_mode);
        if (!sel_kernels) {
        } else if (c.selector_mode == MV_KP_NODEPTH && fuse_epi && !up && !nocov) {
            MV_TRY(mv_frontend_epilogue_select_lanes(in->flow, in->logcov, 1, c.bl_fx, c.bl_fx_sq, mp.disparity, mp.disparity_cov,
                                                     mp.depth, mp.depth_cov, nullptr, mp.match_flow, mp.match_cov, nullptr,
                                                     nullptr, &sp, kp_ws, p->kp_ws_bytes, p->cand[k], p->count[k],
// ... 35 lines not shown
static int flush_deferred(mvFramePipe* p) {
    if (!p->deferred_valid) return MV_OK;
    p->deferred_valid = false;
    return issue_selector_segment(p, p->deferred);
}
static int selector_of_front_issued(mvFramePipe* p) {
    if (p->sel_on_back != 4 || p->pending.size() <= 1) MV_TRY(flush_deferred(p));
    const long sj = p->pending.empty() ? -1 : p->pending.front().sel_job;
    return sj >= 0 ? wait_issued(p, sj + 1) : MV_OK;
}

extern "C" int mv_frame_pipe_enqueue(mvFramePipe* p, const mvFrameInputs* in, mvStream_t in_stream, int with_selector) {
    MV_CHECK_ARG(p && in && in->fmap1 && in->fmap2);
    const mvFramePipeConfig& c = p->c;
    MV_CHECK_ARG(c.iters == 0 || in->coords);
    const bool up = in->flow8 != nullptr;
    const bool any_cov = c.frontend_nocov != (MV_NOCOV_DEPTH | MV_NOCOV_MATCH);
    MV_CHECK_ARG(up ? (in->up_mask && (!any_cov || (in->cov8 && in->cov_mask))) : (in->flow && (!any_cov || in->logcov)));
    const long f = p->n_enq;
    const int k = (int)(f % N_CAND), m = (int)(f % N_MAPS);
    MV_CHECK_ARG(!with_selector || p->newest_maps >= 0);
    MV_CHECK_ARG(!with_selector || (int)p->pending.size() < MAX_PENDING);
    const int B = c.pairs;
    const double t_hs0 = p->host_stats ? now_us() : 0.0;
    MV_TRY(flush_deferred(p));

    const bool ahead = p->n_vol != f;
    if (!ahead) MV_TRY(issue_volume(p, in, in_stream));
    const int kv = (int)(f % p->n_volbuf);
    const int ti = p->time_detail ? p->vol_timed[kv] : -1;
    const bool timed = ti >= 0;

    const size_t coord_stride = (size_t)B * 2 * p->n8;
    const int lk = (int)(f % p->n_lk);
    hipStream_t s = p->s_lk[lk];
    float* const* tok = p->tok + 2 * lk;
    if (ahead) {
        hipEvent_t e = p->e_rest[f % N_INEV];
        MV_HIP(hipEventRecord(e, (hipStream_t)in_stream));
        MV_TRY(wait_if_pending(s, e));
    }
    if (p->lookups_on_main) {
        MV_HIP(hipStreamWaitEvent(s, p->e_vol_done[kv], 0));
        for (int it = 0; it < c.iters; ++it)
            MV_TRY(lookup_of(p)(p->vol[kv], in->coords + it * coord_stride, tok[it & 1], B, p->h8, p->w8, p->h8, p->w8, c.radius, s));
        const bool lean = p->lean_chain && p->dev_draw && with_selector && c.num_point > 0 && p->n_volbuf > MAX_PENDING;
        if (lean) {
            p->vol_free_ev[kv] = p->e_backend[(p->n_fin + (long)p->pending.size()) % N_BEV];
        } else {
            MV_HIP(hipEventRecord(p->e_vol_free[kv], s));
            p->vol_free_ev[kv] = p->e_vol_free[kv];
        }
        p->vol_free_valid[kv] = true;
        if (timed) MV_HIP(hipEventRecord(p->tv2[ti], s));
    } else {
        for (int it = 0; it < c.iters; ++it)
            MV_TRY(lookup_of(p)(p->vol[kv], in->coords + it * coord_stride, tok[it & 1], B, p->h8, p->w8, p->h8, p->w8, c.radius, p->s_vol));
        MV_HIP(hipEventRecord(p->e_vol_done[kv], p->s_vol));
        MV_HIP(hipStreamWaitEvent(s, p->e_vol_done[kv], 0));
        p->vol_free_valid[kv] = false;
    }

    const double t_hs1 = p->host_stats ? now_us() : 0.0;
    SelSeg d{*in, f, k, m, ti, p->newest_maps, timed, with_selector != 0, up,
             p->n_fin - MAX_PENDING + (long)p->pending.size()};
    if (p->sel_on_back) MV_HIP(hipEventRecord(p->e_lk[k], s));
    const bool late = p->sel_on_back == 4 && with_selector && p->pending.size() >= 2;
    if ((p->sel_on_back == 3 && with_selector) || late) {
        p->deferred = d;
        p->deferred_valid = true;
    } else {
        MV_TRY(issue_selector_segment(p, d));
    }
    if (with_selector) p->pending.push_back(Pending{m, p->newest_maps, k, true, ti, -1, f});
    p->newest_maps = m;
    p->n_enq = f + 1;
    if (p->host_stats) {
        const double t_hs2 = now_us();
        p->st_enq += t_hs2 - t_hs0;
        p->st_enq_lookups += t_hs1 - t_hs0;
        p->st_enq_seg += t_hs2 - t_hs1;
    }
    return MV_OK;
}

extern "C" int mv_frame_pipe_wait_motion_input(mvFramePipe* p, mvStream_t stream) {
    MV_CHECK_ARG(p && p->c.motion_model == MV_MOTION_TARTAN && !p->pending.empty() && p->pending.back().f == p->n_enq - 1);
    const long sj = p->pending.back().sel_job;
    if (sj >= 0) MV_TRY(wait_issued(p, sj + 1));
    else MV_TRY(flush_deferred(p));
    const int m = (int)((p->n_enq - 1) % N_MAPS);
    MV_CHECK_ARG(p->motion_in_valid[m]);
    MV_HIP(hipStreamWaitEvent((hipStream_t)stream, p->e_motion_in[m], 0));
    return MV_OK;
}

extern "C" int mv_frame_pipe_set_motion(mvFramePipe* p, const float* motion_dev, mvStream_t stream) {
    MV_CHECK_ARG(p && motion_dev && p->c.motion_model == MV_MOTION_TARTAN && !p->pending.empty() && p->pending.back().f == p->n_enq - 1);
    const long g = p->n_fin + (long)p->pending.size() - 1;
    const int k = (int)(g % N_MOT);
    hipStream_t s = (hipStream_t)stream;
    if (p->motion_used_valid[k]) {
        MV_TRY(wait_issued(p, g - N_MOT + 1));
        MV_HIP(hipStreamWaitEvent(s, p->e_motion_used[k], 0));
    }
    MV_HIP(hipMemcpyAsync(p->motion_raw[k], motion_dev, (size_t)p->lanes * 6 * sizeof(float), hipMemcpyDeviceToDevice, s));
    MV_HIP(hipEventRecord(p->e_motion_set[k], s));
    p->motion_g[k] = g;
    const int m = (int)((p->n_enq - 1) % N_MAPS);
// ... 119 lines not shown
    src.state_in = p->rp_state[j.g & 1]; src.state_out = p->rp_state[(j.g + 1) & 1];
    if (j.kp == KPJ_PERM) {
        src.kind = j.device ? MV_KPSRC_DRAW : MV_KPSRC_PERM;
        src.cand = p->cand[j.pd.cand]; src.cand_lane_stride = (size_t)p->plane;
        if (j.device) {
            src.n_live_dev = p->count[j.pd.cand]; src.n_live_stride = 4;
            src.out_perm = b.perm; src.out_live = b.live_dev;
        } else {
            src.perm_dev = b.perm; src.perm_host = perm_in_args ? p->h_perm[ps] : nullptr;
            src.n_live = j.n_sel;
        }
    } else if (j.kp == KPJ_RANDOM || j.kp == KPJ_GRID) {
        src.kind = j.kp == KPJ_RANDOM ? MV_KPSRC_RANDOM : MV_KPSRC_GRID;
    } else if (j.kp == KPJ_DEV) {
        src.kind = MV_KPSRC_ROWS;
        src.rows = j.kp_dev; src.n_live_dev = j.nsel_dev; src.n_live_stride = 1; src.out_live = b.live_dev;
    } else {
        src.kind = MV_KPSRC_ROWS;
        src.rows = b.kp0; src.n_live = j.n_sel;
    }
    return src;
}

static int finish_issue(mvFramePipe* p, const FinishJob& j, const int64_t* perm_host) {
    const mvFramePipeConfig& c = p->c;
    const int L = p->lanes, cap = cap_of(c);
    const int n_max = j.n_max;
    const Pending& pd = j.pd;
    const long g = j.g;
    const int k = (int)(g & 1);
    Backend& b = p->be[k];
    const int32_t* n_sel = j.n_sel;
    const bool on_dec = j.device && p->front_on_decoder && p->alt && !p->sel_on_back;
    hipStream_t s = on_dec ? p->s_lk[j.pd.f % p->n_lk] : p->s_back;
    const auto pass_generators = [&] {
        return hipMemcpyAsync(p->rp_state[(g + 1) & 1], p->rp_state[g & 1], (size_t)L * (size_t)mv_randperm_state_words() * sizeof(uint32_t), hipMemcpyDeviceToDevice, s);
    };
    if (n_max == 0 && p->dev_draw) MV_HIP(pass_generators());
    const bool motion = c.motion_model == MV_MOTION_TARTAN;
    float* const prior = motion ? p->prior[g % N_MOT] : nullptr;
    if (motion) {
        MV_HIP(hipStreamWaitEvent(p->s_side, p->e_motion_set[g % N_MOT], 0));
        MV_TRY(mv_pose_exp_compose(L, p->pose[j.pose_from], p->motion_raw[g % N_MOT], 6, p->pose_norm, prior, p->s_side));
        MV_HIP(hipEventRecord(p->e_motion_used[g % N_MOT], p->s_side));
        p->motion_used_valid[g % N_MOT] = true;
    }
    if (n_max == 0) {
        MV_HIP(hipMemcpyAsync(p->pose[j.pose_to], motion ? prior : p->pose[j.pose_from], (size_t)L * 7 * sizeof(float), hipMemcpyDeviceToDevice,
                              p->s_side));
        if (j.pose_sink)
            MV_HIP(hipMemcpyAsync(j.pose_sink, p->pose[j.pose_to], (size_t)L * 7 * sizeof(float), hipMemcpyDeviceToDevice, p->s_side));
        MV_HIP(hipEventRecord(p->e_posed[k], p->s_side));
        MV_HIP(hipEventRecord(p->e_pgo, p->s_side));
        MV_HIP(hipEventRecord(p->e_solved[k], p->s_side));
        MV_TRY(wait_if_pending(s, p->e_cand[pd.cand]));
        MV_HIP(hipEventRecord(p->e_backend[g % N_BEV], s));
        p->pgo_valid = true;
        p->solved_valid[k] = true;
        p->backend_valid[g % N_BEV] = true;
        p->nvalid_valid[k] = false;
        return MV_OK;
    }
    const mvFrontMaps fm{p->maps[pd.maps].match_flow, p->maps[pd.maps].match_cov, p->maps[pd.maps_prev].dm, p->maps[pd.maps].dm};
    const mvFrontTables& t = b.front;

    if (p->solved_valid[k] && s != p->s_side) MV_TRY(wait_if_pending(s, p->e_solved[k]));
    if (p->release_valid) MV_TRY(wait_if_pending(s, p->e_release));
    if (p->mapl_valid[k] && s != p->s_back) MV_TRY(wait_if_pending(s, p->e_mapl[k]));
    const int ps = (int)(g % N_PERM);
    if (!j.device && p->dev_draw) MV_HIP(pass_generators());
    const bool host_rows = !j.device && (j.kp == KPJ_PERM || j.kp == KPJ_HOST);
    const size_t rw = j.kp == KPJ_HOST ? 2 : 1;
    if (host_rows) {
        if (p->perm_valid[ps]) MV_HIP(hipEventSynchronize(p->e_perm[ps]));
        for (int l = 0; l < L; ++l)
            memcpy(p->h_perm[ps] + (size_t)l * cap * rw, perm_host + (size_t)l * cap * rw, (size_t)n_sel[l] * rw * sizeof(int64_t));
    }
    if (j.kp == KPJ_DEV) MV_HIP(hipStreamWaitEvent(s, p->e_kpin[g % N_BEV], 0));
    if (!on_dec) MV_TRY(wait_if_pending(s, p->e_cand[pd.cand]));
    else if (g > 0 && p->backend_valid[(g - 1) % N_BEV]) MV_TRY(wait_if_pending(s, p->e_backend[(g - 1) % N_BEV]));
    const bool prev_here = p->alt && p->last_backend_frame == pd.f - 1;
    if (p->alt && pd.f > 0 && !prev_here) MV_TRY(wait_if_pending(s, p->e_seg[(pd.f - 1) % N_INEV]));
    p->last_backend_frame = pd.f;
    const int ti = pd.ti;
    if (ti >= 0) MV_HIP(hipEventRecord(p->tv4[ti], s));
    const bool perm_in_args = j.kp == KPJ_PERM && L == 1 && n_max <= 256;
    if (!perm_in_args && host_rows) {
        const size_t perm_bytes = ((size_t)(L - 1) * cap + n_sel[L - 1]) * rw * sizeof(int64_t);
        MV_HIP(hipMemcpyAsync(j.kp == KPJ_HOST ? b.kp0 : b.perm, p->h_perm[ps], perm_bytes, hipMemcpyHostToDevice, s));
        MV_HIP(hipEventRecord(p->e_perm[ps], s));
        p->perm_valid[ps] = true;
    }
    const bool fused = p->fuse_backend != 0;
    const mvKpSource src = kp_source_of(p, j, b, ps, perm_in_args);
    const auto obs_filter = [&] {
        return mv_obs_filter_lanes(t.inbound, t.cov0, t.cov1, t.vals, c.filters, c.filter_min_depth, c.max_depth, L, n_sel, cap, b.valid, b.n_valid, s);
    };
    if (fused || src.kind != MV_KPSRC_PERM) {
        MV_TRY(mv_backend_front(src, L, cap, fm, p->cov, t, s));
        if (c.mapping && src.kind != MV_KPSRC_DRAW) MV_TRY(obs_filter());
    } else {
        MV_TRY(mv_kp_front_lanes(src.cand, src.cand_lane_stride, src.perm_dev, src.perm_host, L, n_sel, cap, fm.match_flow, fm.match_cov, fm.f0.depth,
                                 fm.f0.disp, fm.f0.sdisp, fm.f0.sdd, fm.f1.depth, fm.f1.disp, fm.f1.sdisp, fm.f1.sdd, c.H, c.W, c.edgewidth,
                                 c.match_cov_default, c.fx, c.fy, c.cx, c.cy, t.kp0_uv, t.kp0, t.kp1, t.inbound, t.vals, t.sigma0, t.sigma1, t.pos_Tc, s));
    }
    if (!fused) {
        if (c.frontend_nocov & MV_NOCOV_MATCH)
            MV_TRY(mv_obs_cov_pair_nomatch_lanes(c.cov_model, c.cov_modifiers, fm.f0.depth, fm.f0.sdd, t.kp0, t.sigma0, nullptr, t.cov0, nullptr, fm.f1.depth,
                                                 fm.f1.sdd, t.kp1, fm.f1.sdd ? t.vals + 7 * (size_t)L * cap : nullptr, c.cov_match_cov_default, t.cov1,
                                                 &p->cov.cp, L, n_sel, cap, s));
        else
            MV_TRY(mv_obs_cov_pair_lanes(c.cov_model, c.cov_modifiers, fm.f0.depth, fm.f0.sdd, t.kp0, t.sigma0, nullptr, t.cov0, nullptr, fm.f1.depth,
                                         fm.f1.sdd, t.kp1, t.sigma1, t.cov1, &p->cov.cp, L, n_sel, cap, s));
        MV_TRY(obs_filter());
    }
    if (c.mapping) {
        MV_HIP(hipMemcpyAsync(p->h_nvalid[k], b.n_valid, (size_t)L * sizeof(int32_t), hipMemcpyDeviceToHost, s));
        MV_HIP(hipEventRecord(p->e_nvalid[k], s));
        p->nvalid_valid[k] = true;
    }
    MV_HIP(hipEventRecord(p->e_backend[g % N_BEV], s));
    p->backend_valid[g % N_BEV] = true;
    if (ti >= 0) MV_HIP(hipEventRecord(p->tv5[ti], s));

    hipStream_t ss = p->s_side;
    if (ss != s) MV_HIP(hipStreamWaitEvent(ss, p->e_backend[g % N_BEV], 0));
    if (ti >= 0) MV_HIP(hipEventRecord(p->tv6[ti], ss));
    mvPosedSolve sv = b.solve;
    sv.init_pose = p->pose[j.pose_from];
    sv.out_pose_f32 = p->pose[j.pose_to];
    if (p->solve_frame == MV_SOLVE_LOCAL) {
        sv.ref_pose = !j.skipped || g == 0 ? p->pose[j.pose_from] : motion ? p->prior[(g - 1) % N_MOT] : p->pose[(j.pose_from + 2) % 3];
    }
    if (fused) {
        sv.start_pose = prior;
        sv.pose_sink = j.pose_sink;
        sv.n_live = src.out_live ? nullptr : n_sel;
        sv.n_live_dev = src.out_live; sv.n_live_stride = 2;
        MV_TRY(mv_posed_solve(sv, ss));
    } else {
        MV_TRY(mv_pose_apply_lanes(sv.init_pose, sv.pos_Tc, sv.cov_Tc, L, n_sel, cap, sv.pos_Tw, sv.out_rot, sv.cov_Tw, ss));
        MV_HIP(hipEventRecord(p->e_posed[k], ss));
        if (sv.ref_pose)
            MV_TRY(mv_pgo_solve_local(L, sv.offsets, sv.graph_type, motion ? prior : sv.init_pose, sv.ref_pose, sv.intrinsics, sv.baseline, sv.pos_Tw, sv.cov_Tw,
                                      sv.pixel2_uv, sv.pixel2_d, sv.pixel2_disp, sv.pixel2_disp_cov, sv.pixel2_uv_cov, sv.obs2_covTc, sv.valid, sv.min_points,
                                      sv.params, sv.out_pose, sv.out_info, sv.out_pose_f32, ss));
        else
        MV_TRY(mv_pgo_solve(L, sv.offsets, sv.graph_type, motion ? prior : sv.init_pose, sv.intrinsics, sv.baseline, sv.pos_Tw, sv.cov_Tw, sv.pixel2_uv,
                            sv.pixel2_d, sv.pixel2_disp, sv.pixel2_disp_cov, sv.pixel2_uv_cov, sv.obs2_covTc, sv.valid, sv.min_points, sv.params,
                            sv.out_pose, sv.out_info, sv.out_pose_f32, ss));
        if (j.pose_sink)
            MV_HIP(hipMemcpyAsync(j.pose_sink, p->pose[j.pose_to], (size_t)L * 7 * sizeof(float), hipMemcpyDeviceToDevice, ss));
    }
    MV_HIP(hipEventRecord(p->e_solved[k], ss));
    MV_HIP(hipEventRecord(p->e_pgo, ss));
// ... 496 lines not shown

extern "C" int mv_frame_pipe_timeline_backend(mvFramePipe* p, float* ms, int cap_frames, int* n) {
    MV_CHECK_ARG(p && n && cap_frames >= 0 && (cap_frames == 0 || ms));
    MV_TRY(flush_jobs(p));
    if (!p->time_detail) { *n = 0; return MV_OK; }
    MV_HIP(hipStreamSynchronize(p->s_back));
    MV_HIP(hipStreamSynchronize(p->s_side));
    for (int k = 0; k < p->n_lk; ++k) MV_HIP(hipStreamSynchronize(p->s_lk[k]));
    const int m = p->n_timed < cap_frames ? p->n_timed : cap_frames;
    for (int i = 0; i < m; ++i) {
        hipEvent_t evs[4] = {p->tv4[i], p->tv5[i], p->tv6[i], p->tv7[i]};
        for (int j = 0; j < 4; ++j)
            if (hipEventElapsedTime(&ms[4 * i + j], p->tv0[0], evs[j]) != hipSuccess) ms[4 * i + j] = -1.f;
    }
    *n = m;
    return MV_OK;
}

extern "C" int mv_frame_pipe_buffer(mvFramePipe* p, int which, int age, void** ptr, size_t* count) {
    MV_CHECK_ARG(p && ptr && count && age >= 0);
    const mvFramePipeConfig& c = p->c;
    const size_t L = p->lanes, plane = L * p->plane;
    *ptr = nullptr;
    *count = 0;
    const long f = p->n_enq - 1 - age, g = p->n_fin - 1 - age;
    auto front = [&](int depth) { return f >= 0 && age < depth; };
    auto back = [&]() { return g >= 0 && age < 2; };
    const Backend* b = back() ? &p->be[g & 1] : nullptr;
    const size_t N = L * (size_t)cap_of(c);
    switch (which) {
        case MV_FB_VOLUME:
            if (!front(p->n_vol > p->n_enq ? 1 : 2)) break;
            *ptr = p->vol[f % p->n_volbuf]; *count = (size_t)c.pairs * p->n8 * p->n2t; return MV_OK;
        case MV_FB_TOKENS: if (!front(1) || c.iters == 0) break; *ptr = p->tok[2 * (f % p->n_lk) + ((c.iters - 1) & 1)]; *count = (size_t)c.pairs * p->KK * p->n8; return MV_OK;
        case MV_FB_DISPARITY: if (!front(N_MAPS)) break; *ptr = p->maps[f % N_MAPS].disparity; *count = plane; return MV_OK;
        case MV_FB_DISPARITY_COV: if (!front(N_MAPS) || !p->maps[0].disparity_cov) break; *ptr = p->maps[f % N_MAPS].disparity_cov; *count = plane; return MV_OK;
        case MV_FB_DEPTH: if (!front(N_MAPS)) break; *ptr = p->maps[f % N_MAPS].depth; *count = plane; return MV_OK;
        case MV_FB_DEPTH_COV: if (!front(N_MAPS) || !p->maps[0].depth_cov) break; *ptr = p->maps[f % N_MAPS].depth_cov; *count = plane; return MV_OK;
        case MV_FB_MATCH_FLOW: if (!front(N_MAPS)) break; *ptr = p->maps[f % N_MAPS].match_flow; *count = 2 * plane; return MV_OK;
        case MV_FB_MATCH_COV: if (!front(N_MAPS) || !p->maps[0].match_cov) break; *ptr = p->maps[f % N_MAPS].match_cov; *count = 3 * plane; return MV_OK;
        case MV_FB_CAND: if (!front(N_CAND)) break; *ptr = p->cand[f % N_CAND]; *count = plane; return MV_OK;
        case MV_FB_COUNT: if (!front(N_CAND)) break; *ptr = p->count[f % N_CAND]; *count = 4 * L; return MV_OK;
        case MV_FB_STATS: if (!front(N_CAND)) break; *ptr = p->stats[f % N_CAND]; *count = 4 * L; return MV_OK;
        case MV_FB_KP0: if (!b) break; *ptr = b->kp0; *count = 2 * N; return MV_OK;
        case MV_FB_KP0F: if (!b) break; *ptr = b->kp0f; *count = 2 * N; return MV_OK;
        case MV_FB_KP1: if (!b) break; *ptr = b->kp1; *count = 2 * N; return MV_OK;
        case MV_FB_INBOUND: if (!b) break; *ptr = b->inbound; *count = N; return MV_OK;
        case MV_FB_VALS: if (!b) break; *ptr = b->vals; *count = 11 * N; return MV_OK;
        case MV_FB_SIGMA0: if (!b) break; *ptr = b->sigma0; *count = 3 * N; return MV_OK;
        case MV_FB_SIGMA1: if (!b) break; *ptr = b->sigma1; *count = 3 * N; return MV_OK;
        case MV_FB_POS_TC: if (!b) break; *ptr = b->pos_Tc; *count = 3 * N; return MV_OK;
        case MV_FB_POS_TW: if (!b) break; *ptr = b->pos_Tw; *count = 3 * N; return MV_OK;
        case MV_FB_ROT: if (!b) break; *ptr = b->rot; *count = 9 * L; return MV_OK;
        case MV_FB_COV0: if (!b) break; *ptr = b->cov0; *count = 9 * N; return MV_OK;
        case MV_FB_COV0W: if (!b) break; *ptr = b->cov0w; *count = 9 * N; return MV_OK;
        case MV_FB_COV1: if (!b) break; *ptr = b->cov1; *count = 9 * N; return MV_OK;
        case MV_FB_VALID: if (!b) break; *ptr = b->valid; *count = N; return MV_OK;
        case MV_FB_NVALID: if (!b) break; *ptr = b->n_valid; *count = L; return MV_OK;
        case MV_FB_POSE64: if (!b) break; *ptr = b->pose64; *count = 7 * L; return MV_OK;
        case MV_FB_INFO: if (!b) break; *ptr = b->info; *count = 4 * L; return MV_OK;
        case MV_FB_POSE: if (age > 1) break; *ptr = p->pose[(p->pose_cur + 3 - age) % 3]; *count = 7 * L; return MV_OK;
        case MV_FB_PERM: if (!b) break; *ptr = b->perm; *count = N; return MV_OK;
        case MV_FB_LIVE: if (!b || !p->dev_draw) break; *ptr = b->live_dev; *count = 2 * L; return MV_OK;
        case MV_FB_MOTION_IN: if (c.motion_model != MV_MOTION_TARTAN || !front(N_MAPS)) break; *ptr = p->motion_in[f % N_MAPS];
            *count = L * (size_t)motion::OUT_C * motion::OUT_H * motion::OUT_W; return MV_OK;
        case MV_FB_PRIOR: if (c.motion_model != MV_MOTION_TARTAN || !back()) break; *ptr = p->prior[g % N_MOT]; *count = 7 * L; return MV_OK;
        case MV_FB_MAP_UV: if (!c.mapping || age) break; *ptr = p->mp_uvf; *count = 2 * (size_t)p->mp_rows; return MV_OK;
// ... 11 lines not shown
```

mac-vo_amd/csrc/kp_select.hip:

```cpp
#include "common.h"
#include <math.h>

namespace {

#ifdef MV_KP_PROFILE
__device__ long long g_kp_stamps[16];
#define KP_STAMP(i) do { if (threadIdx.x == 0) g_kp_stamps[i] = wall_clock64(); } while (0)
#else
#define KP_STAMP(i)
#endif

constexpr int TILE_W = 64;
constexpr int TILE_H = 16;
constexpr int MAX_R = 7;
constexpr unsigned CAND_FLAG = 0x80000000u;

struct KpWs {
    unsigned long long* cand_bits;
    unsigned* rec_idx;
    float* rec_q;
    float* rec_d;
    int* counters;
    size_t lane_bytes;

    __device__ __forceinline__ KpWs lane(int l) const {
        const size_t o = (size_t)l * lane_bytes;
        return KpWs{(unsigned long long*)((char*)cand_bits + o), (unsigned*)((char*)rec_idx + o), (float*)((char*)rec_q + o),
                    (float*)((char*)rec_d + o), (int*)((char*)counters + o), lane_bytes};
    }
};

__device__ __forceinline__ float flow_quality(const float* __restrict__ fc, int plane, int idx) {
    const float c0 = fc[idx], c1 = fc[plane + idx], c2 = fc[2 * plane + idx];
    return (c0 + c1) - 2.f * c2;
}

__device__ __forceinline__ float nanmin(float a, float b) { return (a < b || a != a) ? a : b; }

template <bool FUSE>
__global__ __launch_bounds__(256) void kp_nms_kernel(const float* __restrict__ fc, const float* __restrict__ d0,
                                                      const float* __restrict__ d0c, const float* __restrict__ d1,
                                                      const float* __restrict__ d1c,
                                                      const uint8_t* __restrict__ mask_a,
                                                      const uint8_t* __restrict__ mask_b, mvKpSelectParams p,
                                                      KpWs ws_all, int words_per_row, mvEpiArgs ef) {
    MV_CHAIN_KERNEL_PRIO();
    const KpWs ws = ws_all.lane(blockIdx.z);
    {
        const size_t lp = (size_t)blockIdx.z * p.H * p.W;
        if (fc) fc += 3 * lp;
        if (d0) d0 += lp;
        if (d0c) d0c += lp;
        if (d1) d1 += lp;
        if (d1c) d1c += lp;
        if (mask_a) mask_a += lp;
        if (mask_b) mask_b += lp;
        if (FUSE) {
            ef.flow += 4 * lp; ef.logcov += 4 * lp;
            if (ef.disparity) ef.disparity += lp;
            if (ef.disparity_cov) ef.disparity_cov += lp;
            if (ef.depth) ef.depth += lp;
            if (ef.depth_cov) ef.depth_cov += lp;
            if (ef.bad_mask) ef.bad_mask += lp;
            if (ef.match_flow) ef.match_flow += 2 * lp;
            if (ef.match_cov) ef.match_cov += 3 * lp;
        }
    }
    __shared__ float tile[TILE_H + 2 * MAX_R][TILE_W + 2 * MAX_R + 1];
    __shared__ float hmin[TILE_H + 2 * MAX_R][TILE_W + 1];
    __shared__ int wg_count, wg_base;
    const int H = p.H, W = p.W, plane = H * W;
    const int r = p.kernel_size >> 1;
    const int x0 = blockIdx.x * TILE_W, y0 = blockIdx.y * TILE_H;
    const int tx = threadIdx.x, ty = threadIdx.y;
    const int tid = ty * 64 + tx;
    const bool mapping = p.mode == MV_KP_MAPPING;
    if (tid == 0) wg_count = 0;

    if (!mapping) {
        const int tw = TILE_W + 2 * r, th = TILE_H + 2 * r;
        constexpr int NST = ((TILE_W + 2 * MAX_R) * (TILE_H + 2 * MAX_R) + 255) / 256;
        float qv[NST];
// ... 387 lines not shown
    int pos = block_exclusive_scan<NT>(cnt, L.wave_tot, total);
    KP_STAMP(4);
    auto emit = [&](unsigned long long bits, int w) {
        const int row = w / words_per_row, col0 = (w - row * words_per_row) * 64;
        while (bits) {
            const int bpos = __ffsll((long long)bits) - 1;
            bits &= bits - 1;
            out_cand[pos++] = row * W + col0 + bpos;
        }
    };
    if (FAST) {
#pragma unroll
        for (int i = 0; i < WPT; ++i)
            if (cw[i]) emit(cw[i], w_begin + i);
    } else {
        for (int w = w_begin; w < w_end; ++w)
            emit(__hip_atomic_load(&ws.cand_bits[w], __ATOMIC_RELAXED, __HIP_MEMORY_SCOPE_AGENT), w);
    }
    KP_STAMP(5);
    if (tid == 0) {
        ws.counters[0] = 0;
        out_count[0] = total;
        out_count[1] = n_rec;
        out_count[2] = 0;
        out_count[3] = 0;
        out_stats[0] = med_f;
        out_stats[1] = thr_f;
        out_stats[2] = med_d;
        out_stats[3] = thr_d;
    }
}

template <int NT, int RPT, int WPT, bool USE_D>
__global__ __launch_bounds__(NT) void kp_finish_kernel(mvKpSelectParams p, KpWs ws_all, int has_flow, int words_per_row,
                                                        int32_t* __restrict__ out_cand, int32_t* __restrict__ out_count,
                                                        float* __restrict__ out_stats) {
    __shared__ MedianLds L;
    extern __shared__ unsigned long long lds_words[];
    MV_CHAIN_KERNEL_PRIO();
    const KpWs ws = ws_all.lane(blockIdx.x);
    out_cand += (size_t)blockIdx.x * p.H * p.W;
    out_count += 4 * blockIdx.x;
    out_stats += 4 * blockIdx.x;
    const int n_rec = p.mode == MV_KP_MAPPING ? 0 : ws.counters[0];
    if (n_rec <= RPT * NT && p.H * words_per_row <= WPT * NT)
        kp_finish_body<NT, true, RPT, WPT, USE_D>(p, ws, has_flow, words_per_row, out_cand, out_count, out_stats, n_rec, L,
                                                  lds_words);
    else
        kp_finish_body<NT, false, RPT, WPT, USE_D>(p, ws, has_flow, words_per_row, out_cand, out_count, out_stats, n_rec, L,
                                                   lds_words);
}

template <int NT, int RPT, int WPT, bool USE_D>
static int launch_finish(const mvKpSelectParams& p, const KpWs& ws, int has_flow, int wpr, int32_t* out_cand,
                         int32_t* out_count, float* out_stats, int lanes, hipStream_t s) {
    const size_t dyn = (size_t)WPT * (NT / (WPT > 5 * 1024 / NT ? 8 : 2)) * sizeof(unsigned long long);
    hipLaunchKernelGGL((kp_finish_kernel<NT, RPT, WPT, USE_D>), dim3(lanes), dim3(NT), dyn, s, p, ws, has_flow, wpr, out_cand,
                       out_count, out_stats);
    return MV_OK;
}

__global__ __launch_bounds__(1024) void kp_map_scan_kernel(const unsigned long long* __restrict__ cand_bits, int n_words,
                                                            int* __restrict__ word_off, int32_t* __restrict__ out_count,
                                                            float* __restrict__ out_stats) {
    __shared__ int wave_tot[16];
    const int tid = threadIdx.x;
    const int per = (n_words + 1023) / 1024;
    const int w_begin = min(tid * per, n_words), w_end = min(w_begin + per, n_words);
    int cnt = 0;
    for (int w = w_begin; w < w_end; ++w) cnt += __popcll(cand_bits[w]);
    int total;
    int pos = block_exclusive_scan<1024>(cnt, wave_tot, total);
    for (int w = w_begin; w < w_end; ++w) {
        word_off[w] = pos;
        pos += __popcll(cand_bits[w]);
    }
    if (tid == 0) {
        out_count[0] = total;
        out_count[1] = out_count[2] = out_count[3] = 0;
        out_stats[0] = NAN;
        out_stats[1] = INFINITY;
        out_stats[2] = NAN;
        out_stats[3] = INFINITY;
    }
}

__global__ __launch_bounds__(256) void kp_map_emit_kernel(const unsigned long long* __restrict__ cand_bits,
                                                           const int* __restrict__ word_off, int n_words, int words_per_row,
                                                           int W, int32_t* __restrict__ out_cand) {
    const int w = blockIdx.x * 4 + (threadIdx.x >> 6);
    if (w >= n_words) return;
    const int lane = threadIdx.x & 63;
    const unsigned long long bits = cand_bits[w];
    if ((bits >> lane) & 1ull) {
        const int rank = __popcll(bits & ((1ull << lane) - 1ull));
        const int row = w / words_per_row, col0 = (w - row * words_per_row) * 64;
        out_cand[word_off[w] + rank] = row * W + col0 + lane;
    }
}

__global__ void kp_gather_kernel(const int32_t* __restrict__ cand, const int64_t* __restrict__ perm, mvLaneCounts cnt,
                                 int cap, size_t cand_lane_stride, int W, int64_t* __restrict__ out_uv) {
    const int i = blockIdx.x * blockDim.x + threadIdx.x;
    const int n_sel = cnt.n[blockIdx.y];
    cand += (size_t)blockIdx.y * cand_lane_stride;
    perm += (size_t)blockIdx.y * cap;
    out_uv += 2 * (size_t)blockIdx.y * cap;
    if (i < n_sel) {
        const int lin = cand[perm[i]];
        out_uv[2 * i + 0] = lin % W;
        out_uv[2 * i + 1] = lin / W;
    }
}

inline size_t align_up(size_t v, size_t a) { return (v + a - 1) / a * a; }

}

extern "C" size_t mv_kp_select_workspace_bytes(int H, int W) {
    if (H <= 0 || W <= 0) return 0;
    const size_t words = (size_t)H * mv_ceil_div(W, 64);
    return align_up(words * 8, 256) + 3 * align_up((size_t)H * W * 4, 256) + 256;
}

static int kp_select_impl(const float* flow_cov, const float* depth0, const float* depth0_cov, const float* depth1,
                          const float* depth1_cov, const uint8_t* mask_a, const uint8_t* mask_b, const mvKpSelectParams* params,
                          void* workspace, size_t workspace_bytes, int32_t* out_cand, int32_t* out_count, float* out_stats,
                          int lanes, mvStream_t stream, const mvEpiArgs* fuse) {
    MV_CHECK_ARG(lanes >= 1 && lanes <= MV_MAX_LANES);
    MV_CHECK_ARG(params && workspace && out_cand && out_count && out_stats);
    const mvKpSelectParams p = *params;
    MV_CHECK_ARG(p.H > 0 && p.W > 0 && p.mask_width >= 0);
    if (p.mode == MV_KP_NODEPTH) {
        MV_CHECK_ARG(flow_cov);
    } else if (p.mode == MV_KP_FULL) {
        MV_CHECK_ARG(depth0 && depth0_cov && depth1 && depth1_cov);
    } else if (p.mode == MV_KP_MAPPING) {
        MV_CHECK_ARG(depth0 && depth0_cov);
    } else {
        return MV_ERR_INVALID_ARG;
    }
    if (p.mode != MV_KP_MAPPING) {
        MV_CHECK_ARG(p.kernel_size >= 1 && (p.kernel_size & 1));
        if (p.kernel_size > 2 * MAX_R + 1) return MV_ERR_UNSUPPORTED;
    }
    const size_t lane_bytes = mv_kp_select_workspace_bytes(p.H, p.W);
    if (workspace_bytes < lane_bytes * (size_t)lanes) return MV_ERR_WORKSPACE;
    if (((uintptr_t)workspace & 7) != 0) return MV_ERR_INVALID_ARG;
    if (p.mode == MV_KP_MAPPING && lanes != 1) return MV_ERR_UNSUPPORTED;

    const int wpr = mv_ceil_div(p.W, 64);
    const size_t words = (size_t)p.H * wpr;
    const size_t plane_bytes = align_up((size_t)p.H * p.W * 4, 256);
    char* base = (char*)workspace;
    KpWs ws;
    ws.cand_bits = (unsigned long long*)base;
    base += align_up(words * 8, 256);
    ws.rec_idx = (unsigned*)base;
    base += plane_bytes;
    ws.rec_q = (float*)base;
    base += plane_bytes;
    ws.rec_d = (float*)base;
    base += plane_bytes;
    ws.counters = (int*)base;
    ws.lane_bytes = lane_bytes;

    hipStream_t s = (hipStream_t)stream;
    dim3 grid(wpr, mv_ceil_div(p.H, TILE_H), lanes), block(64, 4);
    if (fuse)
        hipLaunchKernelGGL(kp_nms_kernel<true>, grid, block, 0, s, flow_cov, depth0, depth0_cov, depth1, depth1_cov, mask_a,
                           mask_b, p, ws, wpr, *fuse);
    else
        hipLaunchKernelGGL(kp_nms_kernel<false>, grid, block, 0, s, flow_cov, depth0, depth0_cov, depth1, depth1_cov, mask_a,
                           mask_b, p, ws, wpr, mvEpiArgs{});
    if (p.mode == MV_KP_MAPPING) {
        const int n_words = p.H * wpr;
        int* word_off = (int*)ws.rec_idx;
        hipLaunchKernelGGL(kp_map_scan_kernel, dim3(1), dim3(1024), 0, s, ws.cand_bits, n_words, word_off, out_count, out_stats);
        hipLaunchKernelGGL(kp_map_emit_kernel, dim3(mv_ceil_div(n_words, 4)), dim3(256), 0, s, ws.cand_bits, word_off, n_words,
                           wpr, p.W, out_cand);
        return mv_launch_status();
    }
    const bool big = (size_t)p.H * wpr > 5 * (size_t)1024;
    const bool full = p.mode == MV_KP_FULL;
    int rc;
    static int small_nt = -1;
    if (small_nt < 0) { const char* e = getenv("MV_KP_FINISH_SMALL_NT"); small_nt = (e && atoi(e) == 512) ? 512 : 1024; }
    if (big) rc = full ? launch_finish<1024, 24, 15, true>(p, ws, flow_cov ? 1 : 0, wpr, out_cand, out_count, out_stats, lanes, s)
                       : launch_finish<1024, 24, 15, false>(p, ws, flow_cov ? 1 : 0, wpr, out_cand, out_count, out_stats, lanes, s);
    else if (small_nt == 512)
        rc = full ? launch_finish<512, 16, 10, true>(p, ws, flow_cov ? 1 : 0, wpr, out_cand, out_count, out_stats, lanes, s)
                  : launch_finish<512, 16, 10, false>(p, ws, flow_cov ? 1 : 0, wpr, out_cand, out_count, out_stats, lanes, s);
    else rc = full ? launch_finish<1024, 16, 5, true>(p, ws, flow_cov ? 1 : 0, wpr, out_cand, out_count, out_stats, lanes, s)
                   : launch_finish<1024, 16, 5, false>(p, ws, flow_cov ? 1 : 0, wpr, out_cand, out_count, out_stats, lanes, s);
    if (rc != MV_OK) return rc;
    return mv_launch_status();
}

extern "C" int mv_kp_select_lanes(const float* flow_cov, const float* depth0, const float* depth0_cov,
                                  const float* depth1, const float* depth1_cov, const uint8_t* mask_a,
                                  const uint8_t* mask_b, const mvKpSelectParams* params, void* workspace,
                                  size_t workspace_bytes, int32_t* out_cand, int32_t* out_count, float* out_stats,
                                  int lanes, mvStream_t stream) {
    return kp_select_impl(flow_cov, depth0, depth0_cov, depth1, depth1_cov, mask_a, mask_b, params, workspace, workspace_bytes,
                          out_cand, out_count, out_stats, lanes, stream, nullptr);
}

extern "C" int mv_frontend_epilogue_select_lanes(const float* flow, const float* logcov, int cov_is_log, float bl_fx,
                                                 float bl_fx_sq, float* disparity, float* disparity_cov, float* depth,
                                                 float* depth_cov, uint8_t* bad_mask, float* match_flow, float* match_cov,
                                                 const uint8_t* mask_a, const uint8_t* mask_b, const mvKpSelectParams* params,
                                                 void* workspace, size_t workspace_bytes, int32_t* out_cand,
                                                 int32_t* out_count, float* out_stats, int lanes, mvStream_t stream) {
    MV_CHECK_ARG(flow && logcov && params && match_cov);
    if (params->mode != MV_KP_NODEPTH) return MV_ERR_UNSUPPORTED;
    const mvEpiArgs ef{flow, logcov, cov_is_log, bl_fx, bl_fx_sq, disparity, disparity_cov, depth, depth_cov, match_flow, match_cov,
                       bad_mask};
    return kp_select_impl(match_cov, nullptr, nullptr, nullptr, nullptr, mask_a, mask_b, params, workspace, workspace_bytes,
                          out_cand, out_count, out_stats, lanes, stream, &ef);
}

extern "C" int mv_kp_select(const float* flow_cov, const float* depth0, const float* depth0_cov,
                            const float* depth1, const float* depth1_cov, const uint8_t* mask_a,
                            const uint8_t* mask_b, const mvKpSelectParams* params, void* workspace,
                            size_t workspace_bytes, int32_t* out_cand, int32_t* out_count, float* out_stats,
                            mvStream_t stream) {
    return mv_kp_select_lanes(flow_cov, depth0, depth0_cov, depth1, depth1_cov, mask_a, mask_b, params, workspace,
                              workspace_bytes, out_cand, out_count, out_stats, 1, stream);
}

extern "C" int mv_kp_gather_lanes(const int32_t* cand, size_t cand_lane_stride, const int64_t* perm, int lanes,
                                  const int32_t* n_live, int cap, int W, int64_t* out_uv, mvStream_t stream) {
    MV_CHECK_ARG(lanes >= 1 && lanes <= MV_MAX_LANES && n_live && cap >= 0 && W > 0);
    mvLaneCounts c{};
    int n_max = 0;
    for (int l = 0; l < lanes; ++l) {
        MV_CHECK_ARG(n_live[l] >= 0 && n_live[l] <= cap);
        c.n[l] = n_live[l];
        n_max = n_live[l] > n_max ? n_live[l] : n_max;
    }
    if (n_max == 0) return MV_OK;
    MV_CHECK_ARG(cand && perm && out_uv);
    hipLaunchKernelGGL(kp_gather_kernel, dim3(mv_ceil_div(n_max, 256), lanes), dim3(256), 0, (hipStream_t)stream, cand, perm,
                       c, cap, cand_lane_stride, W, out_uv);
    return mv_launch_status();
}

extern "C" int mv_kp_gather(const int32_t* cand, const int64_t* perm, int n_sel, int W, int64_t* out_uv,
                            mvStream_t stream) {
    MV_CHECK_ARG(n_sel >= 0);
    const int32_t n = n_sel;
    return mv_kp_gather_lanes(cand, 0, perm, 1, &n, n_sel, W, out_uv, stream);
// ... 2 lines not shown
```

mac-vo_amd/ops.py:

```python
from __future__ import annotations

import ctypes as C
from dataclasses import dataclass

import torch

from . import _lib as L

_DT = {torch.float32: L.MV_F32, torch.float16: L.MV_F16, torch.bfloat16: L.MV_BF16}


_raw_stream = getattr(torch._C, "_cuda_getCurrentRawStream", None)


def _stream() -> int:
    if _raw_stream is not None:
        return _raw_stream(torch.cuda.current_device())
    return torch.cuda.current_stream().cuda_stream


def _ptr(t: torch.Tensor | None) -> int | None:
    return None if t is None else t.data_ptr()


# ... 125 lines not shown
    if first.shape != second.shape or first.dim() != 4:
        raise L.MacvoHipError("local_corr81: first / second must be [B,C,H,W] tensors of the same shape")
    B, Cc, H, W = first.shape
    if out is None:
        out = torch.empty((B, 81, H, W), dtype=torch.float32, device=first.device)
    L.check(lib.mv_local_corr81(first.data_ptr(), second.data_ptr(), out.data_ptr(), B, Cc, H, W, _stream()),
            "mv_local_corr81")
    return out


def corr_lookup(cost_maps: torch.Tensor, coords: torch.Tensor, radius: int = 4, out: torch.Tensor | None = None,
                tiled: bool = False, image_hw: "tuple | None" = None) -> torch.Tensor:
    lib = L.load()
    vol16 = cost_maps.dtype == torch.float16
    cost_maps = _req(cost_maps, torch.float16 if vol16 else torch.float32, "cost_maps")
    coords = _req(coords, torch.float32, "coords")
    B, two, H1, W1 = coords.shape
    assert two == 2
    BN, _, H2, W2 = cost_maps.shape
    if BN != B * H1 * W1:
        raise L.MacvoHipError("corr_lookup: cost_maps / coords shape mismatch")
    if image_hw is not None:
        if not (tiled and vol16) or image_hw[1] != W2 or lib.mv_tiled_slice_cells(int(image_hw[0]), W2) != H2 * W2:
            raise L.MacvoHipError("corr_lookup: image_hw belongs to a tiled fp16 volume of mv_tiled_slice_cells(H2, W2) cells per slice")
        H2 = int(image_hw[0])
    K = 2 * radius + 1
    if out is None:
        out = torch.empty((B, K * K, H1, W1), dtype=torch.float32, device=coords.device)
    name = "mv_corr_lookup" + ("_tiled" if tiled else "") + ("_vol16" if vol16 else "")
    L.check(getattr(lib, name)(cost_maps.data_ptr(), coords.data_ptr(), out.data_ptr(), B, H1, W1, H2, W2, radius, _stream()), name)
    return out


def fmap_tile_rows16(f: torch.Tensor, out: torch.Tensor | None = None) -> torch.Tensor:
    lib = L.load()
    if f.dtype not in (torch.float16, torch.bfloat16) or f.dim() != 4:
        raise L.MacvoHipError("fmap_tile_rows16: a [B, H, W, C] float16 / bfloat16 feature map")
    f = _req(f, f.dtype, "f")
    B, H, W, Cc = f.shape
    cells = lib.mv_tiled_slice_cells(H, W)
    if cells == 0:
        raise L.MacvoHipError("fmap_tile_rows16: W % 4 != 0")
    if out is None:
        out = torch.empty((B, cells // W, W, Cc), dtype=f.dtype, device=f.device)
    assert out.numel() >= B * cells * Cc and out.dtype == f.dtype
    L.check(lib.mv_fmap_tile_rows16(f.data_ptr(), out.data_ptr(), B, Cc, H, W, _stream()), "mv_fmap_tile_rows16")
    return out


def corr_volume_out16(f1: torch.Tensor, f2: torch.Tensor, out: torch.Tensor | None = None, tiled: bool = False,
                      scratch: torch.Tensor | None = None) -> torch.Tensor | None:
    lib = L.load()
    if f1.dtype not in (torch.float16, torch.bfloat16) or f1.dtype != f2.dtype or f1.dim() != 4:
        raise L.MacvoHipError("corr_volume_out16: [B, H, W, C] float16 / bfloat16 feature maps")
    f1, f2 = _req(f1, f1.dtype, "f1"), _req(f2, f2.dtype, "f2")
    B, H1, W1, Cc = f1.shape
    _, H2, W2, _ = f2.shape
    N1, N2 = H1 * W1, H2 * W2
    dt = _DT[f1.dtype]
    if tiled:
        N2 = lib.mv_tiled_slice_cells(H2, W2)
        if N2 == 0:
            return None
    if not lib.mv_corr_volume_out16_supported(B, Cc, N1, N2, dt, L.MV_LAYOUT_HWC):
        return None
    if out is None:
# ... 684 lines not shown
```

mac-vo_amd/pipeline.py:

```python
from __future__ import annotations

import os
import time
from dataclasses import dataclass, field, replace

import torch

from . import ops

_RANGES = os.environ.get("MV_TRACE_RANGES", "0") not in ("", "0")


def traced(name: str):
    def deco(fn):
        if not _RANGES:
            return fn
        import functools

        @functools.wraps(fn)
        def wrapped(*a, **k):
            torch.cuda.nvtx.range_push(name)
            try:
                return fn(*a, **k)
            finally:
# ... 1368 lines not shown
    def volume_starts_ms(self) -> list:
        cap = 1 << 16
        buf = (ops.C.c_float * cap)()
        n = ops.C.c_int(0)
        ops.L.check(self._lib.mv_frame_pipe_volume_starts(self._pipe, buf, cap, ops.C.byref(n)), "mv_frame_pipe_volume_starts")
        return list(buf[: n.value])

    def timeline_ms(self) -> list:
        cap = 1 << 14
        buf = (ops.C.c_float * (4 * cap))()
        n = ops.C.c_int(0)
        ops.L.check(self._lib.mv_frame_pipe_timeline(self._pipe, buf, cap, ops.C.byref(n)), "mv_frame_pipe_timeline")
        return [tuple(buf[4 * i: 4 * i + 4]) for i in range(n.value)]

    def timeline_backend_ms(self) -> list:
        cap = 1 << 14
        buf = (ops.C.c_float * (4 * cap))()
        n = ops.C.c_int(0)
        ops.L.check(self._lib.mv_frame_pipe_timeline_backend(self._pipe, buf, cap, ops.C.byref(n)), "mv_frame_pipe_timeline_backend")
        return [tuple(buf[4 * i: 4 * i + 4]) for i in range(n.value)]

    def synchronize(self) -> None:
        if self._pipe is not None:
            ops.L.check(self._lib.mv_frame_pipe_sync(self._pipe, None, 1), "mv_frame_pipe_sync")

    def run(self, frames, pose_sink: torch.Tensor | None = None, depth: int | None = None):
        depth = self._depth if depth is None else depth
        it = iter(frames) if self.cfg.keyframe_freq == 1 else self._keyframes_of(frames)
        nxt = next(it, None)
        if self._pipe is not None and (self.device_driven or self._hostless):
            i = 0
            lag = min(int(os.environ.get("MV_PIPE_DD_AHEAD", "2")), 6)
            clock = time.perf_counter
            while nxt is not None:
                t0 = clock()
                self.enqueue_frontend(nxt)
                nxt = next(it, None)
                if self._volume_ahead and nxt is not None:
                    self.enqueue_volume(nxt)
                res = self.finish(None, None if pose_sink is None else pose_sink[i])
                t1 = clock()
                i += 1
                if lag >= 0:
                    ops.L.check(self._lib.mv_frame_pipe_wait_finished(self._pipe, lag), "mv_frame_pipe_wait_finished")
                self.host_issue_s += t1 - t0
                self.host_wait_s += clock() - t1
                self.host_frames += 1
                yield res
            self.sync_all()
            return
        state = {"nxt": nxt, "vol": False, "pending": 0}

        def pump():
            while state["nxt"] is not None and state["pending"] < depth:
                self.enqueue_frontend(state["nxt"])
                state["pending"] += 1
                state["nxt"], state["vol"] = next(it, None), False
            if self._volume_ahead and state["nxt"] is not None and not state["vol"]:
                self.enqueue_volume(state["nxt"])
                state["vol"] = True

        pump()
        i = 0
        while state["pending"]:
            res = self.finish(None, None if pose_sink is None else pose_sink[i])
            state["pending"] -= 1
            i += 1
            pump()
            yield res
        self.sync_all()

    def _has_pending(self) -> bool:
        return self._n_fin < self._n_enq - 1
```

Before: 7172.

## Batch two consecutive frames into shared lookup and keypoint-select launches

```diff
diff --git a/include/macvo_hip.h b/include/macvo_hip.h
--- a/include/macvo_hip.h
+++ b/include/macvo_hip.h
@@ -79,6 +79,15 @@
 int mv_fmap_tile_rows16(const void* f, void* out, int B, int C, int H, int W, mvStream_t stream);
 int mv_corr_lookup_tiled_vol16(const void* vol_f16, const float* coords, float* out, int B, int H1, int W1, int H2, int W2, int radius,
                                mvStream_t stream);
+
+enum { MV_LOOKUP_VOL_F32 = 0, MV_LOOKUP_VOL_F16 = 1, MV_LOOKUP_VOL_TILED_F32 = 2, MV_LOOKUP_VOL_TILED_F16 = 3 };
+typedef struct mvLookupFrame {
+    const void* vol;
+    const float* coords;
+    float* out;
+} mvLookupFrame;
+int mv_corr_lookup_frames(const mvLookupFrame* frames , int n_frames , int vol_kind, int pairs_per_frame,
+                          int H1, int W1, int H2, int W2, int radius, mvStream_t stream);
 
 int mv_frontend_epilogue(const float* flow, const float* logcov, int cov_is_log, int H, int W,
                          float bl_fx, float bl_fx_sq, float* disparity, float* disparity_cov,
@@ -355,6 +364,20 @@
                                       const uint8_t* mask_b, const mvKpSelectParams* params , void* workspace,
                                       size_t workspace_bytes, int32_t* out_cand, int32_t* out_count, float* out_stats,
                                       int lanes, mvStream_t stream);
+typedef struct mvKpFrame {
+    const float *flow_cov, *depth0, *depth0_cov, *depth1, *depth1_cov;
+    const uint8_t *mask_a, *mask_b;
+    void* workspace;
+    int32_t* out_cand;
+    int32_t* out_count;
+    float* out_stats;
+    const float *flow, *logcov;
+    float *disparity, *disparity_cov, *depth, *depth_cov, *match_flow, *match_cov;
+    uint8_t* bad_mask;
+} mvKpFrame;
+int mv_kp_select_frames(const mvKpFrame* frames , int n_frames , int lanes_per_frame,
+                        const mvKpSelectParams* params , size_t workspace_bytes, int cov_is_log, float bl_fx, float bl_fx_sq,
+                        mvStream_t stream);
 int mv_kp_gather_lanes(const int32_t* cand, size_t cand_lane_stride, const int64_t* perm , int lanes,
                        const int32_t* n_live , int cap, int W, int64_t* out_uv ,
                        mvStream_t stream);
@@ -465,6 +488,9 @@
 int mv_frame_pipe_wait_motion_input(mvFramePipe* p, mvStream_t stream);
 int mv_frame_pipe_set_motion(mvFramePipe* p, const float* motion_dev, mvStream_t stream);
 int mv_frame_pipe_enqueue_volume(mvFramePipe* p, const mvFrameInputs* in, mvStream_t in_stream);
+int mv_frame_pipe_pair_ok(const mvFramePipe* p);
+int mv_frame_pipe_enqueue_pair(mvFramePipe* p, const mvFrameInputs* in_a, const mvFrameInputs* in_b, mvStream_t in_stream);
+long mv_frame_pipe_pairs(const mvFramePipe* p);
 int mv_frame_pipe_wait_candidates(mvFramePipe* p, int32_t* n_cand );
 int mv_frame_pipe_finish(mvFramePipe* p, const int64_t* perm_host, const int32_t* n_sel, float* pose_sink);
 int mv_frame_pipe_wait_tracked(mvFramePipe* p, int32_t* n_valid, int32_t* n_cand_map);
diff --git a/mac-vo_amd/_lib.py b/mac-vo_amd/_lib.py
--- a/mac-vo_amd/_lib.py
+++ b/mac-vo_amd/_lib.py
@@ -83,6 +83,16 @@
     _fields_ = [("lanes", C.c_int32), ("cap", C.c_int32), ("prev_frame", C.c_int32), ("min_num_point", C.c_int32)] + \
         [(n, C.c_void_p) for n in ("n_rows", "time_ns", "valid", "kp0", "kp1", "vals", "sigma0", "sigma1", "cov0", "cov1", "pos_Tw", "cov0_world",
                                    "color", "K", "T_BS", "prior_pose")] + [("baseline", C.c_float)]
+
+
+class mvLookupFrame(C.Structure):
+    _fields_ = [(n, C.c_void_p) for n in ("vol", "coords", "out")]
+
+
+class mvKpFrame(C.Structure):
+    _fields_ = [(n, C.c_void_p) for n in ("flow_cov", "depth0", "depth0_cov", "depth1", "depth1_cov", "mask_a", "mask_b", "workspace", "out_cand",
+                                          "out_count", "out_stats", "flow", "logcov", "disparity", "disparity_cov", "depth", "depth_cov",
+                                          "match_flow", "match_cov", "bad_mask")]
 
 
 class mvFrameInputs(C.Structure):
@@ -112,6 +122,7 @@
     "mv_corr_lookup_tiled": (C.c_int, [_P, _P, _P, C.c_int, C.c_int, C.c_int, C.c_int, C.c_int, C.c_int, _P]),
     "mv_corr_lookup_vol16": (C.c_int, [_P, _P, _P, C.c_int, C.c_int, C.c_int, C.c_int, C.c_int, C.c_int, _P]),
     "mv_corr_lookup_tiled_vol16": (C.c_int, [_P, _P, _P, C.c_int, C.c_int, C.c_int, C.c_int, C.c_int, C.c_int, _P]),
+    "mv_corr_lookup_frames": (C.c_int, [C.POINTER(mvLookupFrame), C.c_int, C.c_int, C.c_int, C.c_int, C.c_int, C.c_int, C.c_int, C.c_int, _P]),
     "mv_fmap_tile_rows16": (C.c_int, [_P, _P, C.c_int, C.c_int, C.c_int, C.c_int, _P]),
     "mv_tiled_slice_cells": (C.c_int, [C.c_int, C.c_int]),
     "mv_corr_volume_out16_supported": (C.c_int, [C.c_int, C.c_int, C.c_int, C.c_int, C.c_int, C.c_int]),
@@ -173,6 +184,7 @@
                                                     C.POINTER(mvKpSelectParams), _P, C.c_size_t, _P, _P, _P, C.c_int, _P]),
     "mv_kp_select_lanes": (C.c_int, [_P, _P, _P, _P, _P, _P, _P, C.POINTER(mvKpSelectParams), _P, C.c_size_t,
                                      _P, _P, _P, C.c_int, _P]),
+    "mv_kp_select_frames": (C.c_int, [C.POINTER(mvKpFrame), C.c_int, C.c_int, C.POINTER(mvKpSelectParams), C.c_size_t, C.c_int, C.c_float, C.c_float, _P]),
     "mv_kp_gather_lanes": (C.c_int, [_P, C.c_size_t, _P, C.c_int, _P, C.c_int, C.c_int, _P, _P]),
     "mv_kp_track_lanes": (C.c_int, [_P, C.c_int, _P, C.c_int, _P, _P, _P, _P, _P, _P, _P, _P, _P, _P, C.c_int, C.c_int,
                                     C.c_int, C.c_float, _P, _P, _P, _P, _P, _P, _P]),
@@ -194,6 +206,9 @@
     "mv_frame_pipe_set_pose": (C.c_int, [_P, _P]),
     "mv_frame_pipe_enqueue": (C.c_int, [_P, C.POINTER(mvFrameInputs), _P, C.c_int]),
     "mv_frame_pipe_enqueue_volume": (C.c_int, [_P, C.POINTER(mvFrameInputs), _P]),
+    "mv_frame_pipe_pair_ok": (C.c_int, [_P]),
+    "mv_frame_pipe_enqueue_pair": (C.c_int, [_P, C.POINTER(mvFrameInputs), C.POINTER(mvFrameInputs), _P]),
+    "mv_frame_pipe_pairs": (C.c_long, [_P]),
     "mv_frame_pipe_wait_candidates": (C.c_int, [_P, _P]),
     "mv_frame_pipe_finish": (C.c_int, [_P, _P, _P, _P]),
     "mv_map_append_points": (C.c_int, [_P, C.c_int, _P, _P, _P, _P]),
diff --git a/mac-vo_amd/csrc/corr_lookup.hip b/mac-vo_amd/csrc/corr_lookup.hip
--- a/mac-vo_amd/csrc/corr_lookup.hip
+++ b/mac-vo_amd/csrc/corr_lookup.hip
@@ -3,6 +3,14 @@
 namespace {
 
 struct AxisEntry { float w; int c; };
+
+template <typename VT>
+struct LookupFrame2 {
+    const VT* vol;
+    const float* coords;
+    float* out;
+    int pairs_per_frame;
+};
 
 template <int K, int QPW, int STRIDE, int CELLS>
 __device__ __forceinline__ void tap_pairs(const float* blk, const AxisEntry (*ax)[2 * K], int lane, float (&res)[(QPW * K * K + 63) / 64]) {
@@ -43,7 +51,8 @@
 template <int R, int QPW, int QPB, typename VT = float>
 __global__ __launch_bounds__(64 * (QPB / QPW)) void corr_lookup_kernel(const VT* __restrict__ vol,
                                                                         const float* __restrict__ coords,
-                                                                        float* __restrict__ out, int N1, int H2, int W2) {
+                                                                        float* __restrict__ out, int N1, int H2, int W2,
+                                                                        LookupFrame2<VT> fr2) {
     constexpr int K = 2 * R + 1;
     constexpr int KK = K * K;
     constexpr int BS = K + 3;
@@ -67,7 +76,11 @@
     float (*outs)[QPB + 1] = reinterpret_cast<float (*)[QPB + 1]>(smem);
 
     MV_SMALL_KERNEL_PRIO();
-    const int b = blockIdx.y;
+    int b = blockIdx.y;
+    if (b >= fr2.pairs_per_frame) {
+        b -= fr2.pairs_per_frame;
+        vol = fr2.vol; coords = fr2.coords; out = fr2.out;
+    }
     const int q0 = blockIdx.x * QPB;
     const int t = threadIdx.x, lane = t & 63, wave = t >> 6;
     const int slice = H2 * W2;
@@ -170,7 +183,8 @@
 template <int QPW, int QPB, typename VT = float>
 __global__ __launch_bounds__(64 * (QPB / QPW)) void corr_lookup_tiled_kernel(const VT* __restrict__ vol,
                                                                               const float* __restrict__ coords,
-                                                                              float* __restrict__ out, int N1, int H2, int W2) {
+                                                                              float* __restrict__ out, int N1, int H2, int W2,
+                                                                              LookupFrame2<VT> fr2) {
     constexpr int R = 4, K = 9, KK = 81;
     constexpr int BS = 16;
     constexpr int BSP = 18, CELLS = BS * BSP;
@@ -185,7 +199,11 @@
     float (*outs)[QPB + 1] = reinterpret_cast<float (*)[QPB + 1]>(smem);
 
     MV_SMALL_KERNEL_PRIO();
-    const int b = blockIdx.y;
+    int b = blockIdx.y;
+    if (b >= fr2.pairs_per_frame) {
+        b -= fr2.pairs_per_frame;
+        vol = fr2.vol; coords = fr2.coords; out = fr2.out;
+    }
     const int q0 = blockIdx.x * QPB;
     const int t = threadIdx.x, lane = t & 63, wave = t >> 6;
     const int tpr = W2 >> 2, tpc = (H2 + 3) >> 2, slice = tpc * tpr * 16;
@@ -289,82 +307,83 @@
     return v;
 }
 
+static int lookup_launch(int kind, const mvLookupFrame* fr, int n_frames, int B, int H1, int W1, int H2, int W2, int radius, mvStream_t stream) {
+    MV_CHECK_ARG(fr && (n_frames == 1 || n_frames == 2));
+    for (int f = 0; f < n_frames; ++f) MV_CHECK_ARG(fr[f].vol && fr[f].coords && fr[f].out);
+    MV_CHECK_ARG(B > 0 && H1 > 0 && W1 > 0 && H2 > 1 && W2 > 1);
+    if (radius < 1 || radius > 4) return MV_ERR_UNSUPPORTED;
+    if (kind != 0 && radius != 4) return MV_ERR_UNSUPPORTED;
+    if (kind == 2 && (H2 % 4)) return MV_ERR_UNSUPPORTED;
+    if (kind >= 2 && (W2 % 4)) return MV_ERR_UNSUPPORTED;
+    if (kind == 3) for (int f = 0; f < n_frames; ++f) MV_CHECK_ARG(((uintptr_t)fr[f].vol & 31) == 0);
+    const int BT = B * n_frames;
+    if (BT > 65535) return MV_ERR_UNSUPPORTED;
+    const int N1 = H1 * W1;
+    hipStream_t s = (hipStream_t)stream;
+    const mvLookupFrame& f0 = fr[0];
+    const mvLookupFrame& f1 = fr[n_frames - 1];
+    const bool small = (size_t)BT * N1 <= (size_t)lookup_small_threshold();
+    static int small_qpb = -1;
+    if (small_qpb < 0) { const char* e = getenv("MV_LOOKUP_QPB"); small_qpb = (e && atoi(e) == 8) ? 8 : 16; }
+#define MV_LOOKUP_GO(KERNEL, VT, QPB)                                                                                                   \
+    hipLaunchKernelGGL((KERNEL), dim3(mv_ceil_div(N1, QPB), BT), dim3(QPB == 8 ? 256 : 512), 0, s, (const VT*)f0.vol, f0.coords, f0.out, N1, H2, W2, \
+                       (LookupFrame2<VT>{(const VT*)f1.vol, f1.coords, f1.out, B}))
+#define MV_LOOKUP(R)                                                                      \
+    if (small && small_qpb == 8) MV_LOOKUP_GO((corr_lookup_kernel<R, 2, 8>), float, 8);   \
+    else if (small) MV_LOOKUP_GO((corr_lookup_kernel<R, 2, 16>), float, 16);              \
+    else MV_LOOKUP_GO((corr_lookup_kernel<R, 4, 32>), float, 32)
+    if (kind == 0) {
+        switch (radius) {
+            case 1: MV_LOOKUP(1); break;
+            case 2: MV_LOOKUP(2); break;
+            case 3: MV_LOOKUP(3); break;
+            default: MV_LOOKUP(4); break;
+        }
+    } else if (kind == 1) {
+        if (small) MV_LOOKUP_GO((corr_lookup_kernel<4, 2, 16, _Float16>), _Float16, 16);
+        else MV_LOOKUP_GO((corr_lookup_kernel<4, 4, 32, _Float16>), _Float16, 32);
+    } else if (kind == 2) {
+        if (small) MV_LOOKUP_GO((corr_lookup_tiled_kernel<2, 16>), float, 16);
+        else MV_LOOKUP_GO((corr_lookup_tiled_kernel<4, 32>), float, 32);
+    } else {
+        if (small) MV_LOOKUP_GO((corr_lookup_tiled_kernel<2, 16, _Float16>), _Float16, 16);
+        else MV_LOOKUP_GO((corr_lookup_tiled_kernel<4, 32, _Float16>), _Float16, 32);
+    }
+#undef MV_LOOKUP
+#undef MV_LOOKUP_GO
+    return mv_launch_status();
+}
+
 extern "C" int mv_corr_lookup(const float* vol, const float* coords, float* out, int B, int H1, int W1,
                               int H2, int W2, int radius, mvStream_t stream) {
-    MV_CHECK_ARG(vol && coords && out);
-    MV_CHECK_ARG(B > 0 && H1 > 0 && W1 > 0 && H2 > 1 && W2 > 1);
-    if (radius < 1 || radius > 4) return MV_ERR_UNSUPPORTED;
-    if (B > 65535) return MV_ERR_UNSUPPORTED;
-    const int N1 = H1 * W1;
-    hipStream_t s = (hipStream_t)stream;
-    const bool small = (size_t)B * N1 <= (size_t)lookup_small_threshold();
-    static int small_qpb = -1;
-    if (small_qpb < 0) { const char* e = getenv("MV_LOOKUP_QPB"); small_qpb = (e && atoi(e) == 8) ? 8 : 16; }
-#define MV_LOOKUP(R)                                                                                                  \
-    if (small && small_qpb == 8)                                                                                      \
-        hipLaunchKernelGGL((corr_lookup_kernel<R, 2, 8>), dim3(mv_ceil_div(N1, 8), B), dim3(256), 0, s, vol, coords,  \
-                           out, N1, H2, W2);                                                                          \
-    else if (small)                                                                                                   \
-        hipLaunchKernelGGL((corr_lookup_kernel<R, 2, 16>), dim3(mv_ceil_div(N1, 16), B), dim3(512), 0, s, vol, coords, \
-                           out, N1, H2, W2);                                                                          \
-    else                                                                                                              \
-        hipLaunchKernelGGL((corr_lookup_kernel<R, 4, 32>), dim3(mv_ceil_div(N1, 32), B), dim3(512), 0, s, vol, coords, \
-                           out, N1, H2, W2)
-    switch (radius) {
-        case 1: MV_LOOKUP(1); break;
-        case 2: MV_LOOKUP(2); break;
-        case 3: MV_LOOKUP(3); break;
-        default: MV_LOOKUP(4); break;
-    }
-#undef MV_LOOKUP
-    return mv_launch_status();
+    const mvLookupFrame fr{vol, coords, out};
+    return lookup_launch(0, &fr, 1, B, H1, W1, H2, W2, radius, stream);
 }
 
 extern "C" int mv_corr_lookup_vol16(const void* vol, const float* coords, float* out, int B, int H1, int W1, int H2, int W2, int radius,
                                     mvStream_t stream) {
-    MV_CHECK_ARG(vol && coords && out);
-    MV_CHECK_ARG(B > 0 && H1 > 0 && W1 > 0 && H2 > 1 && W2 > 1);
-    if (radius != 4 || B > 65535) return MV_ERR_UNSUPPORTED;
-    const int N1 = H1 * W1;
-    hipStream_t s = (hipStream_t)stream;
-    const _Float16* v = reinterpret_cast<const _Float16*>(vol);
-    if ((size_t)B * N1 <= (size_t)lookup_small_threshold())
-        hipLaunchKernelGGL((corr_lookup_kernel<4, 2, 16, _Float16>), dim3(mv_ceil_div(N1, 16), B), dim3(512), 0, s, v, coords, out, N1, H2, W2);
-    else
-        hipLaunchKernelGGL((corr_lookup_kernel<4, 4, 32, _Float16>), dim3(mv_ceil_div(N1, 32), B), dim3(512), 0, s, v, coords, out, N1, H2, W2);
-    return mv_launch_status();
+    const mvLookupFrame fr{vol, coords, out};
+    return lookup_launch(1, &fr, 1, B, H1, W1, H2, W2, radius, stream);
 }
 
 extern "C" int mv_corr_lookup_tiled(const float* vol, const float* coords, float* out, int B, int H1, int W1, int H2, int W2,
                                     int radius, mvStream_t stream) {
-    MV_CHECK_ARG(vol && coords && out);
-    MV_CHECK_ARG(B > 0 && H1 > 0 && W1 > 0 && H2 > 1 && W2 > 1);
-    if (radius != 4 || (H2 % 4) || (W2 % 4) || B > 65535) return MV_ERR_UNSUPPORTED;
-    const int N1 = H1 * W1;
-    hipStream_t s = (hipStream_t)stream;
-    if ((size_t)B * N1 <= (size_t)lookup_small_threshold())
-        hipLaunchKernelGGL((corr_lookup_tiled_kernel<2, 16>), dim3(mv_ceil_div(N1, 16), B), dim3(512), 0, s, vol, coords, out, N1, H2, W2);
-    else
-        hipLaunchKernelGGL((corr_lookup_tiled_kernel<4, 32>), dim3(mv_ceil_div(N1, 32), B), dim3(512), 0, s, vol, coords, out, N1, H2, W2);
-    return mv_launch_status();
-}
-
+    const mvLookupFrame fr{vol, coords, out};
+    return lookup_launch(2, &fr, 1, B, H1, W1, H2, W2, radius, stream);
+}
 
 extern "C" int mv_corr_lookup_tiled_vol16(const void* vol, const float* coords, float* out, int B, int H1, int W1, int H2, int W2, int radius,
                                           mvStream_t stream) {
-    MV_CHECK_ARG(vol && coords && out);
-    MV_CHECK_ARG(B > 0 && H1 > 0 && W1 > 0 && H2 > 1 && W2 > 1);
-    MV_CHECK_ARG(((uintptr_t)vol & 31) == 0);
-    if (radius != 4 || (W2 % 4) || B > 65535) return MV_ERR_UNSUPPORTED;
-    const int N1 = H1 * W1;
-    hipStream_t s = (hipStream_t)stream;
-    const _Float16* v = reinterpret_cast<const _Float16*>(vol);
-    if ((size_t)B * N1 <= (size_t)lookup_small_threshold())
-        hipLaunchKernelGGL((corr_lookup_tiled_kernel<2, 16, _Float16>), dim3(mv_ceil_div(N1, 16), B), dim3(512), 0, s, v, coords, out, N1, H2, W2);
-    else
-        hipLaunchKernelGGL((corr_lookup_tiled_kernel<4, 32, _Float16>), dim3(mv_ceil_div(N1, 32), B), dim3(512), 0, s, v, coords, out, N1, H2, W2);
-    return mv_launch_status();
-}
+    const mvLookupFrame fr{vol, coords, out};
+    return lookup_launch(3, &fr, 1, B, H1, W1, H2, W2, radius, stream);
+}
+
+extern "C" int mv_corr_lookup_frames(const mvLookupFrame* frames, int n_frames, int vol_kind, int pairs_per_frame, int H1, int W1, int H2, int W2,
+                                     int radius, mvStream_t stream) {
+    MV_CHECK_ARG(vol_kind >= MV_LOOKUP_VOL_F32 && vol_kind <= MV_LOOKUP_VOL_TILED_F16);
+    return lookup_launch(vol_kind, frames, n_frames, pairs_per_frame, H1, W1, H2, W2, radius, stream);
+}
+
 
 namespace {
 __global__ __launch_bounds__(256) void fmap_tile_rows16_kernel(const uint4* __restrict__ f, uint4* __restrict__ out, int H, int W, int n_out, int cpr, size_t total) {
diff --git a/mac-vo_amd/csrc/frame_pipe.hip b/mac-vo_amd/csrc/frame_pipe.hip
--- a/mac-vo_amd/csrc/frame_pipe.hip
+++ b/mac-vo_amd/csrc/frame_pipe.hip
@@ -34,6 +34,7 @@
 #endif
 constexpr int MAX_PENDING = MV_MAX_PENDING, N_MAPS = MAX_PENDING + 2, N_CAND = MAX_PENDING + 1, N_PERM = 4, N_INEV = 8, MAX_VOL = 4, MAX_LK = 2;
 constexpr int N_MOT = 8;
+static_assert(MAX_PENDING < 2 || (N_MAPS >= 5 && N_CAND >= 4 && MAX_VOL >= 4), "slot rotation does not cover two pairs in flight");
 constexpr int N_BEV = 8;
 
 inline bool kp_new_mode(int m) { return m == MV_KP_RANDOM || m == MV_KP_GRID || m == MV_KP_EXPLICIT; }
@@ -127,6 +128,7 @@
     float* vol[MAX_VOL];
     int n_volbuf;
     float* tok[2 * MAX_LK];
+    float* tok_newest;
     void* planes[2];
     void* pk[2][2];
     int n2t;
@@ -163,6 +165,13 @@
     bool seg_valid[N_INEV];
     int alt_indep;
     void* kp_ws2;
+    void* kp_wsx[2 * MAX_LK];
+    int lk_of[N_INEV];
+    bool last_paired;
+    int front_lk[N_BEV];
+    long vol_free_g[MAX_VOL];
+    int pair_on;
+    long n_pairs;
     int lean_chain;
     bool cand_recorded[N_CAND];
     hipEvent_t vol_free_ev[MAX_VOL];
@@ -274,6 +283,7 @@
 static int issue_selector_segment(mvFramePipe* p, const SelSeg& d);
 static int flush_jobs(mvFramePipe* p);
 static void launch_thread_main(mvFramePipe* p);
+extern "C" int mv_frame_pipe_pair_ok(const mvFramePipe* p);
 
 static int layout_alt(int lanes, int mapping) {
     const char* e = getenv("MV_PIPE_LAYOUT");
@@ -318,6 +328,10 @@
     p->kp_ws_bytes = L * mv_kp_select_workspace_bytes(c.H, c.W);
     p->kp_ws = a.take<char>(p->kp_ws_bytes);
     p->kp_ws2 = L <= 2 ? a.take<char>(p->kp_ws_bytes) : nullptr;
+    p->kp_wsx[0] = p->kp_ws;
+    p->kp_wsx[2] = p->kp_ws2;
+    p->kp_wsx[1] = L == 1 ? a.take<char>(p->kp_ws_bytes) : nullptr;
+    p->kp_wsx[3] = L == 1 ? a.take<char>(p->kp_ws_bytes) : nullptr;
 
     for (int k = 0; k < N_CAND; ++k) {
         p->cand[k] = a.take<int32_t>(L * plane);
@@ -577,7 +591,8 @@
         MV_HIP(hipHostMalloc((void**)&p->h_perm[k], (size_t)p->lanes * N * 2 * sizeof(int64_t), hipHostMallocDefault));
     }
     MV_HIP(hipMemsetAsync(p->kp_ws, 0, p->kp_ws_bytes, p->s_main));
-    if (p->kp_ws2) MV_HIP(hipMemsetAsync(p->kp_ws2, 0, p->kp_ws_bytes, p->s_main));
+    for (int k = 1; k < 2 * MAX_LK; ++k)
+        if (p->kp_wsx[k]) MV_HIP(hipMemsetAsync(p->kp_wsx[k], 0, p->kp_ws_bytes, p->s_main));
     const int L = p->lanes;
     std::vector<float> ident((size_t)L * 7, 0.f), intr((size_t)L * 4), bl((size_t)L, c.baseline);
     std::vector<int32_t> offs((size_t)L + 1);
@@ -640,6 +655,9 @@
     describe_backend(p);
     p->newest_maps = -1;
     for (auto& r : p->cand_recorded) r = true;
+    for (auto& g : p->vol_free_g) g = -1;
+    for (auto& l : p->front_lk) l = -1;
+    { const char* e = getenv("MV_PIPE_PAIR"); p->pair_on = (e && atoi(e) != 0) ? 1 : 0; }
     {
         const char* e = getenv("MV_PIPE_LOOKUPS_ON");
         p->lookups_on_main = (e && strcmp(e, "vol") == 0) ? 0 : 1;
@@ -705,7 +723,10 @@
     MV_HIP(hipEventRecord(e_in, (hipStream_t)in_stream));
     p->e_in_of[k] = e_in;
     MV_TRY(wait_if_pending(p->s_vol, e_in));
-    if (p->vol_free_valid[k]) MV_TRY(wait_if_pending(p->s_vol, p->vol_free_ev[k] ? p->vol_free_ev[k] : p->e_vol_free[k]));
+    if (p->vol_free_valid[k]) {
+        if (p->vol_free_g[k] >= 0 && p->vol_free_g[k] < p->n_fin) MV_TRY(wait_issued(p, p->vol_free_g[k] + 1));
+        MV_TRY(wait_if_pending(p->s_vol, p->vol_free_ev[k] ? p->vol_free_ev[k] : p->e_vol_free[k]));
+    }
     const bool timed = p->n_timed < p->timed_cap;
     if (timed && !p->packed) MV_HIP(hipEventRecord(p->tv0[p->n_timed], p->s_vol));
     if (p->packed) {
@@ -752,7 +773,7 @@
 
 extern "C" int mv_frame_pipe_enqueue_volume(mvFramePipe* p, const mvFrameInputs* in, mvStream_t in_stream) {
     MV_CHECK_ARG(p && in && in->fmap1 && in->fmap2);
-    MV_CHECK_ARG(p->n_vol == p->n_enq);
+    MV_CHECK_ARG(p->n_vol == p->n_enq || (p->n_vol == p->n_enq + 1 && mv_frame_pipe_pair_ok(p)));
     MV_CHECK_ARG(p->lookups_on_main);
     const double t_hs = p->host_stats ? now_us() : 0.0;
     MV_TRY(issue_volume(p, in, in_stream));
@@ -762,11 +783,11 @@
 
 static int ensure_chain_events(mvFramePipe* p, long f, int cand_slot) {
     if (cand_slot >= 0 && !p->cand_recorded[cand_slot]) {
-        MV_HIP(hipEventRecord(p->e_cand[cand_slot], p->s_lk[f % p->n_lk]));
+        MV_HIP(hipEventRecord(p->e_cand[cand_slot], p->s_lk[p->lk_of[f % N_INEV]]));
         p->cand_recorded[cand_slot] = true;
     }
     if (p->alt && f >= 0 && !p->seg_valid[f % N_INEV]) {
-        MV_HIP(hipEventRecord(p->e_seg[f % N_INEV], p->s_lk[f % p->n_lk]));
+        MV_HIP(hipEventRecord(p->e_seg[f % N_INEV], p->s_lk[p->lk_of[f % N_INEV]]));
         p->seg_valid[f % N_INEV] = true;
     }
     return MV_OK;
@@ -788,7 +809,8 @@
     const mvFrameInputs* in = &d.in;
     const int k = d.k, m = d.m, ti = d.ti, B = c.pairs;
     const bool timed = d.timed, with_selector = d.with_selector, up = d.up;
-    hipStream_t s = p->s_lk[d.f % p->n_lk];
+    const int lk = p->lk_of[d.f % N_INEV];
+    hipStream_t s = p->s_lk[lk];
     if (p->sel_on_back) {
         s = p->sel_on_back == 2 ? p->s_sel : p->sel_on_back == 3 ? p->s_vol : p->s_back;
         MV_HIP(hipStreamWaitEvent(s, p->e_lk[k], 0));
@@ -814,7 +836,7 @@
         MV_TRY(ensure_chain_events(p, d.f - 1, -1));
         MV_TRY(wait_if_pending(s, p->e_seg[(d.f - 1) % N_INEV]));
     }
-    void* const kp_ws = (indep && (d.f & 1)) ? p->kp_ws2 : p->kp_ws;
+    void* const kp_ws = indep ? p->kp_wsx[2 * lk] : p->kp_ws;
     Maps& mp = p->maps[m];
     constexpr bool fuse_epi = true;
     const int nocov = c.frontend_nocov;
@@ -916,9 +938,12 @@
     const bool timed = ti >= 0;
 
     const size_t coord_stride = (size_t)B * 2 * p->n8;
-    const int lk = (int)(f % p->n_lk);
+    const int lk = (p->last_paired && p->n_lk == 2) ? (p->lk_of[(f - 1) % N_INEV] ^ 1) : (int)(f % p->n_lk);
+    p->lk_of[f % N_INEV] = lk;
+    p->last_paired = false;
     hipStream_t s = p->s_lk[lk];
     float* const* tok = p->tok + 2 * lk;
+    if (c.iters > 0) p->tok_newest = tok[(c.iters - 1) & 1];
     if (ahead) {
         hipEvent_t e = p->e_rest[f % N_INEV];
         MV_HIP(hipEventRecord(e, (hipStream_t)in_stream));
@@ -930,10 +955,12 @@
             MV_TRY(lookup_of(p)(p->vol[kv], in->coords + it * coord_stride, tok[it & 1], B, p->h8, p->w8, p->h8, p->w8, c.radius, s));
         const bool lean = p->lean_chain && p->dev_draw && with_selector && c.num_point > 0 && p->n_volbuf > MAX_PENDING;
         if (lean) {
-            p->vol_free_ev[kv] = p->e_backend[(p->n_fin + (long)p->pending.size()) % N_BEV];
+            p->vol_free_g[kv] = p->n_fin + (long)p->pending.size();
+            p->vol_free_ev[kv] = p->e_backend[p->vol_free_g[kv] % N_BEV];
         } else {
             MV_HIP(hipEventRecord(p->e_vol_free[kv], s));
             p->vol_free_ev[kv] = p->e_vol_free[kv];
+            p->vol_free_g[kv] = -1;
         }
         p->vol_free_valid[kv] = true;
         if (timed) MV_HIP(hipEventRecord(p->tv2[ti], s));
@@ -959,6 +986,113 @@
     if (with_selector) p->pending.push_back(Pending{m, p->newest_maps, k, true, ti, -1, f});
     p->newest_maps = m;
     p->n_enq = f + 1;
+    if (p->host_stats) {
+        const double t_hs2 = now_us();
+        p->st_enq += t_hs2 - t_hs0;
+        p->st_enq_lookups += t_hs1 - t_hs0;
+        p->st_enq_seg += t_hs2 - t_hs1;
+    }
+    return MV_OK;
+}
+
+extern "C" int mv_frame_pipe_pair_ok(const mvFramePipe* p) {
+    if (!p) return 0;
+    const mvFramePipeConfig& c = p->c;
+    return p->pair_on && p->lanes == 1 && p->dev_draw && p->alt && p->n_lk == 2 && p->lean_chain && p->front_on_decoder && !p->sel_on_back && p->lookups_on_main &&
+           p->fuse_backend && !c.mapping && c.motion_model == MV_MOTION_STATIC && c.num_point > 0 && !c.frontend_nocov && p->n_volbuf >= 4 && MAX_PENDING >= 2 &&
+           (c.selector_mode == MV_KP_NODEPTH || c.selector_mode == MV_KP_FULL) ? 1 : 0;
+}
+extern "C" long mv_frame_pipe_pairs(const mvFramePipe* p) { return p ? p->n_pairs : 0; }
+
+extern "C" int mv_frame_pipe_enqueue_pair(mvFramePipe* p, const mvFrameInputs* in_a, const mvFrameInputs* in_b, mvStream_t in_stream) {
+    MV_CHECK_ARG(p && in_a);
+    if (!in_b) return mv_frame_pipe_enqueue(p, in_a, in_stream, 1);
+    MV_CHECK_ARG(mv_frame_pipe_pair_ok(p));
+    const mvFramePipeConfig& c = p->c;
+    const mvFrameInputs* in[2] = {in_a, in_b};
+    for (const mvFrameInputs* x : in)
+        MV_CHECK_ARG(x->fmap1 && x->fmap2 && (c.iters == 0 || x->coords) && x->flow && x->logcov && !x->flow8);
+    MV_CHECK_ARG(p->newest_maps >= 0 && p->pending.empty());
+    const long f = p->n_enq, g = p->n_fin;
+    MV_CHECK_ARG(p->n_vol >= f && p->n_vol <= f + 2);
+    const int B = c.pairs;
+    const double t_hs0 = p->host_stats ? now_us() : 0.0;
+    MV_TRY(wait_issued(p, g - 2 > 0 ? g - 2 : 0));
+
+    const bool ahead = p->n_vol != f;
+    while (p->n_vol < f + 2) MV_TRY(issue_volume(p, in[p->n_vol - f], in_stream));
+    const int lk = p->lk_of[(f - 1) % N_INEV] ^ 1;
+    hipStream_t s = p->s_lk[lk];
+    int kv[2], k[2], m[2], ti[2];
+    for (int i = 0; i < 2; ++i) {
+        p->lk_of[(f + i) % N_INEV] = lk;
+        kv[i] = (int)((f + i) % p->n_volbuf);
+        k[i] = (int)((f + i) % N_CAND);
+        m[i] = (int)((f + i) % N_MAPS);
+        ti[i] = p->time_detail ? p->vol_timed[kv[i]] : -1;
+    }
+    if (ahead) {
+        hipEvent_t e = p->e_rest[f % N_INEV];
+        MV_HIP(hipEventRecord(e, (hipStream_t)in_stream));
+        MV_TRY(wait_if_pending(s, e));
+    }
+    MV_HIP(hipStreamWaitEvent(s, p->e_vol_done[kv[1]], 0));
+    const size_t coord_stride = (size_t)B * 2 * p->n8;
+    float* const tok[2] = {p->tok[2 * lk], p->tok[2 * lk + 1]};
+    const int kind = p->vol16 ? (p->tiled ? MV_LOOKUP_VOL_TILED_F16 : MV_LOOKUP_VOL_F16) : (p->tiled ? MV_LOOKUP_VOL_TILED_F32 : MV_LOOKUP_VOL_F32);
+    for (int it = 0; it < c.iters; ++it) {
+        const mvLookupFrame fr[2] = {{p->vol[kv[0]], in[0]->coords + it * coord_stride, tok[0]}, {p->vol[kv[1]], in[1]->coords + it * coord_stride, tok[1]}};
+        MV_TRY(mv_corr_lookup_frames(fr, 2, kind, B, p->h8, p->w8, p->h8, p->w8, c.radius, s));
+    }
+    if (c.iters > 0) p->tok_newest = tok[1];
+    for (int i = 0; i < 2; ++i) {
+        p->vol_free_g[kv[i]] = g;
+        p->vol_free_ev[kv[i]] = p->e_backend[g % N_BEV];
+        p->vol_free_valid[kv[i]] = true;
+        if (ti[i] >= 0) MV_HIP(hipEventRecord(p->tv2[ti[i]], s));
+    }
+    const double t_hs1 = p->host_stats ? now_us() : 0.0;
+
+    if (g - 3 >= 0 && p->backend_valid[(g - 3) % N_BEV]) MV_TRY(wait_if_pending(s, p->e_backend[(g - 3) % N_BEV]));
+    if (p->release_valid) MV_TRY(wait_if_pending(s, p->e_release));
+    const bool indep = p->alt_indep && c.selector_mode == MV_KP_NODEPTH;
+    if (!indep) {
+        MV_TRY(ensure_chain_events(p, f - 1, -1));
+        MV_TRY(wait_if_pending(s, p->e_seg[(f - 1) % N_INEV]));
+    }
+    mvKpSelectParams sp{c.H, c.W, c.selector_mode, c.kp_kernel_size, c.kp_mask_width, c.max_depth, c.max_depth_cov, c.max_match_cov};
+    mvKpFrame kf[2] = {};
+    for (int i = 0; i < 2; ++i) {
+        Maps& mp = p->maps[m[i]];
+        kf[i].flow_cov = mp.match_cov;
+        kf[i].workspace = p->kp_wsx[2 * lk + i];
+        kf[i].out_cand = p->cand[k[i]]; kf[i].out_count = p->count[k[i]]; kf[i].out_stats = p->stats[k[i]];
+        if (indep) {
+            kf[i].flow = in[i]->flow; kf[i].logcov = in[i]->logcov;
+            kf[i].disparity = mp.disparity; kf[i].disparity_cov = mp.disparity_cov; kf[i].depth = mp.depth; kf[i].depth_cov = mp.depth_cov;
+            kf[i].match_flow = mp.match_flow; kf[i].match_cov = mp.match_cov;
+        } else {
+            MV_TRY(mv_frontend_epilogue_lanes(in[i]->flow, in[i]->logcov, 1, c.H, c.W, c.bl_fx, c.bl_fx_sq, mp.disparity, mp.disparity_cov, mp.depth, mp.depth_cov,
+                                              nullptr, mp.match_flow, mp.match_cov, 1, s));
+            const Maps& m0 = p->maps[i == 0 ? p->newest_maps : m[0]];
+            if (c.selector_mode == MV_KP_FULL) { kf[i].depth0 = m0.depth; kf[i].depth0_cov = m0.depth_cov; kf[i].depth1 = mp.depth; kf[i].depth1_cov = mp.depth_cov; }
+        }
+    }
+    MV_TRY(mv_kp_select_frames(kf, 2, 1, &sp, p->kp_ws_bytes, 1, c.bl_fx, c.bl_fx_sq, s));
+    for (int i = 0; i < 2; ++i) {
+        p->cand_recorded[k[i]] = !indep;
+        p->seg_valid[(f + i) % N_INEV] = !indep;
+        if (!indep) {
+            MV_HIP(hipEventRecord(p->e_cand[k[i]], s));
+            MV_HIP(hipEventRecord(p->e_seg[(f + i) % N_INEV], s));
+        }
+        if (ti[i] >= 0) MV_HIP(hipEventRecord(p->tv3[ti[i]], s));
+        p->pending.push_back(Pending{m[i], i == 0 ? p->newest_maps : m[0], k[i], true, ti[i], -1, f + i});
+    }
+    p->newest_maps = m[1];
+    p->n_enq = f + 2;
+    p->last_paired = true;
+    p->n_pairs += 1;
     if (p->host_stats) {
         const double t_hs2 = now_us();
         p->st_enq += t_hs2 - t_hs0;
@@ -1144,7 +1278,8 @@
     Backend& b = p->be[k];
     const int32_t* n_sel = j.n_sel;
     const bool on_dec = j.device && p->front_on_decoder && p->alt && !p->sel_on_back;
-    hipStream_t s = on_dec ? p->s_lk[j.pd.f % p->n_lk] : p->s_back;
+    const int my_lk = on_dec ? p->lk_of[j.pd.f % N_INEV] : -1;
+    hipStream_t s = on_dec ? p->s_lk[my_lk] : p->s_back;
     const auto pass_generators = [&] {
         return hipMemcpyAsync(p->rp_state[(g + 1) & 1], p->rp_state[g & 1], (size_t)L * (size_t)mv_randperm_state_words() * sizeof(uint32_t), hipMemcpyDeviceToDevice, s);
     };
@@ -1170,6 +1305,7 @@
         p->pgo_valid = true;
         p->solved_valid[k] = true;
         p->backend_valid[g % N_BEV] = true;
+        p->front_lk[g % N_BEV] = my_lk;
         p->nvalid_valid[k] = false;
         return MV_OK;
     }
@@ -1190,7 +1326,8 @@
     }
     if (j.kp == KPJ_DEV) MV_HIP(hipStreamWaitEvent(s, p->e_kpin[g % N_BEV], 0));
     if (!on_dec) MV_TRY(wait_if_pending(s, p->e_cand[pd.cand]));
-    else if (g > 0 && p->backend_valid[(g - 1) % N_BEV]) MV_TRY(wait_if_pending(s, p->e_backend[(g - 1) % N_BEV]));
+    else if (g > 0 && p->backend_valid[(g - 1) % N_BEV] && p->front_lk[(g - 1) % N_BEV] != my_lk)
+        MV_TRY(wait_if_pending(s, p->e_backend[(g - 1) % N_BEV]));
     const bool prev_here = p->alt && p->last_backend_frame == pd.f - 1;
     if (p->alt && pd.f > 0 && !prev_here) MV_TRY(wait_if_pending(s, p->e_seg[(pd.f - 1) % N_INEV]));
     p->last_backend_frame = pd.f;
@@ -1233,6 +1370,7 @@
     }
     MV_HIP(hipEventRecord(p->e_backend[g % N_BEV], s));
     p->backend_valid[g % N_BEV] = true;
+    p->front_lk[g % N_BEV] = my_lk;
     if (ti >= 0) MV_HIP(hipEventRecord(p->tv5[ti], s));
 
     hipStream_t ss = p->s_side;
@@ -1795,7 +1933,7 @@
         case MV_FB_VOLUME:
             if (!front(p->n_vol > p->n_enq ? 1 : 2)) break;
             *ptr = p->vol[f % p->n_volbuf]; *count = (size_t)c.pairs * p->n8 * p->n2t; return MV_OK;
-        case MV_FB_TOKENS: if (!front(1) || c.iters == 0) break; *ptr = p->tok[2 * (f % p->n_lk) + ((c.iters - 1) & 1)]; *count = (size_t)c.pairs * p->KK * p->n8; return MV_OK;
+        case MV_FB_TOKENS: if (!front(1) || c.iters == 0 || !p->tok_newest) break; *ptr = p->tok_newest; *count = (size_t)c.pairs * p->KK * p->n8; return MV_OK;
         case MV_FB_DISPARITY: if (!front(N_MAPS)) break; *ptr = p->maps[f % N_MAPS].disparity; *count = plane; return MV_OK;
         case MV_FB_DISPARITY_COV: if (!front(N_MAPS) || !p->maps[0].disparity_cov) break; *ptr = p->maps[f % N_MAPS].disparity_cov; *count = plane; return MV_OK;
         case MV_FB_DEPTH: if (!front(N_MAPS)) break; *ptr = p->maps[f % N_MAPS].depth; *count = plane; return MV_OK;
diff --git a/mac-vo_amd/csrc/kp_select.hip b/mac-vo_amd/csrc/kp_select.hip
--- a/mac-vo_amd/csrc/kp_select.hip
+++ b/mac-vo_amd/csrc/kp_select.hip
@@ -30,6 +30,18 @@
     }
 };
 
+struct KpNmsFrame {
+    const float *fc, *d0, *d0c, *d1, *d1c;
+    const uint8_t *mask_a, *mask_b;
+    KpWs ws;
+    mvEpiArgs ef;
+};
+struct KpFinFrame {
+    KpWs ws;
+    int32_t *out_cand, *out_count;
+    float* out_stats;
+};
+
 __device__ __forceinline__ float flow_quality(const float* __restrict__ fc, int plane, int idx) {
     const float c0 = fc[idx], c1 = fc[plane + idx], c2 = fc[2 * plane + idx];
     return (c0 + c1) - 2.f * c2;
@@ -38,16 +50,22 @@
 __device__ __forceinline__ float nanmin(float a, float b) { return (a < b || a != a) ? a : b; }
 
 template <bool FUSE>
-__global__ __launch_bounds__(256) void kp_nms_kernel(const float* __restrict__ fc, const float* __restrict__ d0,
-                                                      const float* __restrict__ d0c, const float* __restrict__ d1,
-                                                      const float* __restrict__ d1c,
-                                                      const uint8_t* __restrict__ mask_a,
-                                                      const uint8_t* __restrict__ mask_b, mvKpSelectParams p,
-                                                      KpWs ws_all, int words_per_row, mvEpiArgs ef) {
+__global__ __launch_bounds__(256) void kp_nms_kernel(KpNmsFrame fr0, KpNmsFrame fr1, int lanes_per_frame, mvKpSelectParams p, int words_per_row) {
     MV_CHAIN_KERNEL_PRIO();
-    const KpWs ws = ws_all.lane(blockIdx.z);
+    const bool second = (int)blockIdx.z >= lanes_per_frame;
+    const int lz = (int)blockIdx.z - (second ? lanes_per_frame : 0);
+    const KpNmsFrame& fr = second ? fr1 : fr0;
+    const float* __restrict__ fc = fr.fc;
+    const float* __restrict__ d0 = fr.d0;
+    const float* __restrict__ d0c = fr.d0c;
+    const float* __restrict__ d1 = fr.d1;
+    const float* __restrict__ d1c = fr.d1c;
+    const uint8_t* __restrict__ mask_a = fr.mask_a;
+    const uint8_t* __restrict__ mask_b = fr.mask_b;
+    mvEpiArgs ef = fr.ef;
+    const KpWs ws = fr.ws.lane(lz);
     {
-        const size_t lp = (size_t)blockIdx.z * p.H * p.W;
+        const size_t lp = (size_t)lz * p.H * p.W;
         if (fc) fc += 3 * lp;
         if (d0) d0 += lp;
         if (d0c) d0c += lp;
@@ -501,16 +519,18 @@
 }
 
 template <int NT, int RPT, int WPT, bool USE_D>
-__global__ __launch_bounds__(NT) void kp_finish_kernel(mvKpSelectParams p, KpWs ws_all, int has_flow, int words_per_row,
-                                                        int32_t* __restrict__ out_cand, int32_t* __restrict__ out_count,
-                                                        float* __restrict__ out_stats) {
+__global__ __launch_bounds__(NT) void kp_finish_kernel(mvKpSelectParams p, KpFinFrame fr0, KpFinFrame fr1, int lanes_per_frame, int has_flow,
+                                                        int words_per_row) {
     __shared__ MedianLds L;
     extern __shared__ unsigned long long lds_words[];
     MV_CHAIN_KERNEL_PRIO();
-    const KpWs ws = ws_all.lane(blockIdx.x);
-    out_cand += (size_t)blockIdx.x * p.H * p.W;
-    out_count += 4 * blockIdx.x;
-    out_stats += 4 * blockIdx.x;
+    const bool second = (int)blockIdx.x >= lanes_per_frame;
+    const int lz = (int)blockIdx.x - (second ? lanes_per_frame : 0);
+    const KpFinFrame& fr = second ? fr1 : fr0;
+    const KpWs ws = fr.ws.lane(lz);
+    int32_t* __restrict__ out_cand = fr.out_cand + (size_t)lz * p.H * p.W;
+    int32_t* __restrict__ out_count = fr.out_count + 4 * lz;
+    float* __restrict__ out_stats = fr.out_stats + 4 * lz;
     const int n_rec = p.mode == MV_KP_MAPPING ? 0 : ws.counters[0];
     if (n_rec <= RPT * NT && p.H * words_per_row <= WPT * NT)
         kp_finish_body<NT, true, RPT, WPT, USE_D>(p, ws, has_flow, words_per_row, out_cand, out_count, out_stats, n_rec, L,
@@ -521,11 +541,10 @@
 }
 
 template <int NT, int RPT, int WPT, bool USE_D>
-static int launch_finish(const mvKpSelectParams& p, const KpWs& ws, int has_flow, int wpr, int32_t* out_cand,
-                         int32_t* out_count, float* out_stats, int lanes, hipStream_t s) {
+static int launch_finish(const mvKpSelectParams& p, const KpFinFrame& f0, const KpFinFrame& f1, int lanes_per_frame, int has_flow, int wpr,
+                         int lanes, hipStream_t s) {
     const size_t dyn = (size_t)WPT * (NT / (WPT > 5 * 1024 / NT ? 8 : 2)) * sizeof(unsigned long long);
-    hipLaunchKernelGGL((kp_finish_kernel<NT, RPT, WPT, USE_D>), dim3(lanes), dim3(NT), dyn, s, p, ws, has_flow, wpr, out_cand,
-                       out_count, out_stats);
+    hipLaunchKernelGGL((kp_finish_kernel<NT, RPT, WPT, USE_D>), dim3(lanes), dim3(NT), dyn, s, p, f0, f1, lanes_per_frame, has_flow, wpr);
     return MV_OK;
 }
 
@@ -592,62 +611,80 @@
     return align_up(words * 8, 256) + 3 * align_up((size_t)H * W * 4, 256) + 256;
 }
 
-static int kp_select_impl(const float* flow_cov, const float* depth0, const float* depth0_cov, const float* depth1,
-                          const float* depth1_cov, const uint8_t* mask_a, const uint8_t* mask_b, const mvKpSelectParams* params,
-                          void* workspace, size_t workspace_bytes, int32_t* out_cand, int32_t* out_count, float* out_stats,
-                          int lanes, mvStream_t stream, const mvEpiArgs* fuse) {
-    MV_CHECK_ARG(lanes >= 1 && lanes <= MV_MAX_LANES);
-    MV_CHECK_ARG(params && workspace && out_cand && out_count && out_stats);
+static int kp_select_frames_impl(const mvKpFrame* frames, int n_frames, int lpf, const mvKpSelectParams* params, size_t workspace_bytes, bool fuse,
+                                 int cov_is_log, float bl_fx, float bl_fx_sq, mvStream_t stream) {
+    MV_CHECK_ARG(frames && (n_frames == 1 || n_frames == 2));
+    const int lanes = lpf * n_frames;
+    MV_CHECK_ARG(lpf >= 1 && lanes <= MV_MAX_LANES);
+    MV_CHECK_ARG(params);
     const mvKpSelectParams p = *params;
     MV_CHECK_ARG(p.H > 0 && p.W > 0 && p.mask_width >= 0);
-    if (p.mode == MV_KP_NODEPTH) {
-        MV_CHECK_ARG(flow_cov);
-    } else if (p.mode == MV_KP_FULL) {
-        MV_CHECK_ARG(depth0 && depth0_cov && depth1 && depth1_cov);
-    } else if (p.mode == MV_KP_MAPPING) {
-        MV_CHECK_ARG(depth0 && depth0_cov);
-    } else {
-        return MV_ERR_INVALID_ARG;
-    }
+    for (int f = 0; f < n_frames; ++f) {
+        const mvKpFrame& k = frames[f];
+        MV_CHECK_ARG(k.workspace && k.out_cand && k.out_count && k.out_stats);
+        if (p.mode == MV_KP_NODEPTH) {
+            MV_CHECK_ARG(k.flow_cov);
+        } else if (p.mode == MV_KP_FULL) {
+            MV_CHECK_ARG(k.depth0 && k.depth0_cov && k.depth1 && k.depth1_cov);
+        } else if (p.mode == MV_KP_MAPPING) {
+            MV_CHECK_ARG(k.depth0 && k.depth0_cov);
+        } else {
+            return MV_ERR_INVALID_ARG;
+        }
+        if (fuse) MV_CHECK_ARG(k.flow && k.logcov && k.match_cov);
+    }
+    if (fuse && p.mode != MV_KP_NODEPTH) return MV_ERR_UNSUPPORTED;
     if (p.mode != MV_KP_MAPPING) {
         MV_CHECK_ARG(p.kernel_size >= 1 && (p.kernel_size & 1));
         if (p.kernel_size > 2 * MAX_R + 1) return MV_ERR_UNSUPPORTED;
     }
     const size_t lane_bytes = mv_kp_select_workspace_bytes(p.H, p.W);
-    if (workspace_bytes < lane_bytes * (size_t)lanes) return MV_ERR_WORKSPACE;
-    if (((uintptr_t)workspace & 7) != 0) return MV_ERR_INVALID_ARG;
+    if (workspace_bytes < lane_bytes * (size_t)lpf) return MV_ERR_WORKSPACE;
+    for (int f = 0; f < n_frames; ++f)
+        if (((uintptr_t)frames[f].workspace & 7) != 0) return MV_ERR_INVALID_ARG;
     if (p.mode == MV_KP_MAPPING && lanes != 1) return MV_ERR_UNSUPPORTED;
 
     const int wpr = mv_ceil_div(p.W, 64);
     const size_t words = (size_t)p.H * wpr;
     const size_t plane_bytes = align_up((size_t)p.H * p.W * 4, 256);
-    char* base = (char*)workspace;
-    KpWs ws;
-    ws.cand_bits = (unsigned long long*)base;
-    base += align_up(words * 8, 256);
-    ws.rec_idx = (unsigned*)base;
-    base += plane_bytes;
-    ws.rec_q = (float*)base;
-    base += plane_bytes;
-    ws.rec_d = (float*)base;
-    base += plane_bytes;
-    ws.counters = (int*)base;
-    ws.lane_bytes = lane_bytes;
+    KpNmsFrame nf[2];
+    KpFinFrame ff[2];
+    for (int f = 0; f < 2; ++f) {
+        const mvKpFrame& k = frames[f < n_frames ? f : 0];
+        char* base = (char*)k.workspace;
+        KpWs ws;
+        ws.cand_bits = (unsigned long long*)base;
+        base += align_up(words * 8, 256);
+        ws.rec_idx = (unsigned*)base;
+        base += plane_bytes;
+        ws.rec_q = (float*)base;
+        base += plane_bytes;
+        ws.rec_d = (float*)base;
+        base += plane_bytes;
+        ws.counters = (int*)base;
+        ws.lane_bytes = lane_bytes;
+        const mvEpiArgs ef = fuse ? mvEpiArgs{k.flow, k.logcov, cov_is_log, bl_fx, bl_fx_sq, k.disparity, k.disparity_cov, k.depth, k.depth_cov, k.match_flow,
+                                              k.match_cov, k.bad_mask}
+                                  : mvEpiArgs{};
+        nf[f] = KpNmsFrame{k.flow_cov, k.depth0, k.depth0_cov, k.depth1, k.depth1_cov, k.mask_a, k.mask_b, ws, ef};
+        ff[f] = KpFinFrame{ws, k.out_cand, k.out_count, k.out_stats};
+    }
+    const KpWs& ws = nf[0].ws;
+    const bool has_flow = frames[0].flow_cov != nullptr;
+    for (int f = 1; f < n_frames; ++f) MV_CHECK_ARG((frames[f].flow_cov != nullptr) == has_flow);
 
     hipStream_t s = (hipStream_t)stream;
     dim3 grid(wpr, mv_ceil_div(p.H, TILE_H), lanes), block(64, 4);
     if (fuse)
-        hipLaunchKernelGGL(kp_nms_kernel<true>, grid, block, 0, s, flow_cov, depth0, depth0_cov, depth1, depth1_cov, mask_a,
-                           mask_b, p, ws, wpr, *fuse);
+        hipLaunchKernelGGL(kp_nms_kernel<true>, grid, block, 0, s, nf[0], nf[1], lpf, p, wpr);
     else
-        hipLaunchKernelGGL(kp_nms_kernel<false>, grid, block, 0, s, flow_cov, depth0, depth0_cov, depth1, depth1_cov, mask_a,
-                           mask_b, p, ws, wpr, mvEpiArgs{});
+        hipLaunchKernelGGL(kp_nms_kernel<false>, grid, block, 0, s, nf[0], nf[1], lpf, p, wpr);
     if (p.mode == MV_KP_MAPPING) {
         const int n_words = p.H * wpr;
         int* word_off = (int*)ws.rec_idx;
-        hipLaunchKernelGGL(kp_map_scan_kernel, dim3(1), dim3(1024), 0, s, ws.cand_bits, n_words, word_off, out_count, out_stats);
+        hipLaunchKernelGGL(kp_map_scan_kernel, dim3(1), dim3(1024), 0, s, ws.cand_bits, n_words, word_off, frames[0].out_count, frames[0].out_stats);
         hipLaunchKernelGGL(kp_map_emit_kernel, dim3(mv_ceil_div(n_words, 4)), dim3(256), 0, s, ws.cand_bits, word_off, n_words,
-                           wpr, p.W, out_cand);
+                           wpr, p.W, frames[0].out_cand);
         return mv_launch_status();
     }
     const bool big = (size_t)p.H * wpr > 5 * (size_t)1024;
@@ -655,13 +692,13 @@
     int rc;
     static int small_nt = -1;
     if (small_nt < 0) { const char* e = getenv("MV_KP_FINISH_SMALL_NT"); small_nt = (e && atoi(e) == 512) ? 512 : 1024; }
-    if (big) rc = full ? launch_finish<1024, 24, 15, true>(p, ws, flow_cov ? 1 : 0, wpr, out_cand, out_count, out_stats, lanes, s)
-                       : launch_finish<1024, 24, 15, false>(p, ws, flow_cov ? 1 : 0, wpr, out_cand, out_count, out_stats, lanes, s);
+    if (big) rc = full ? launch_finish<1024, 24, 15, true>(p, ff[0], ff[1], lpf, has_flow ? 1 : 0, wpr, lanes, s)
+                       : launch_finish<1024, 24, 15, false>(p, ff[0], ff[1], lpf, has_flow ? 1 : 0, wpr, lanes, s);
     else if (small_nt == 512)
-        rc = full ? launch_finish<512, 16, 10, true>(p, ws, flow_cov ? 1 : 0, wpr, out_cand, out_count, out_stats, lanes, s)
-                  : launch_finish<512, 16, 10, false>(p, ws, flow_cov ? 1 : 0, wpr, out_cand, out_count, out_stats, lanes, s);
-    else rc = full ? launch_finish<1024, 16, 5, true>(p, ws, flow_cov ? 1 : 0, wpr, out_cand, out_count, out_stats, lanes, s)
-                   : launch_finish<1024, 16, 5, false>(p, ws, flow_cov ? 1 : 0, wpr, out_cand, out_count, out_stats, lanes, s);
+        rc = full ? launch_finish<512, 16, 10, true>(p, ff[0], ff[1], lpf, has_flow ? 1 : 0, wpr, lanes, s)
+                  : launch_finish<512, 16, 10, false>(p, ff[0], ff[1], lpf, has_flow ? 1 : 0, wpr, lanes, s);
+    else rc = full ? launch_finish<1024, 16, 5, true>(p, ff[0], ff[1], lpf, has_flow ? 1 : 0, wpr, lanes, s)
+                   : launch_finish<1024, 16, 5, false>(p, ff[0], ff[1], lpf, has_flow ? 1 : 0, wpr, lanes, s);
     if (rc != MV_OK) return rc;
     return mv_launch_status();
 }
@@ -671,8 +708,10 @@
                                   const uint8_t* mask_b, const mvKpSelectParams* params, void* workspace,
                                   size_t workspace_bytes, int32_t* out_cand, int32_t* out_count, float* out_stats,
                                   int lanes, mvStream_t stream) {
-    return kp_select_impl(flow_cov, depth0, depth0_cov, depth1, depth1_cov, mask_a, mask_b, params, workspace, workspace_bytes,
-                          out_cand, out_count, out_stats, lanes, stream, nullptr);
+    mvKpFrame k{};
+    k.flow_cov = flow_cov; k.depth0 = depth0; k.depth0_cov = depth0_cov; k.depth1 = depth1; k.depth1_cov = depth1_cov;
+    k.mask_a = mask_a; k.mask_b = mask_b; k.workspace = workspace; k.out_cand = out_cand; k.out_count = out_count; k.out_stats = out_stats;
+    return kp_select_frames_impl(&k, 1, lanes, params, workspace_bytes, false, 0, 0.f, 0.f, stream);
 }
 
 extern "C" int mv_frontend_epilogue_select_lanes(const float* flow, const float* logcov, int cov_is_log, float bl_fx,
@@ -682,11 +721,20 @@
                                                  void* workspace, size_t workspace_bytes, int32_t* out_cand,
                                                  int32_t* out_count, float* out_stats, int lanes, mvStream_t stream) {
     MV_CHECK_ARG(flow && logcov && params && match_cov);
-    if (params->mode != MV_KP_NODEPTH) return MV_ERR_UNSUPPORTED;
-    const mvEpiArgs ef{flow, logcov, cov_is_log, bl_fx, bl_fx_sq, disparity, disparity_cov, depth, depth_cov, match_flow, match_cov,
-                       bad_mask};
-    return kp_select_impl(match_cov, nullptr, nullptr, nullptr, nullptr, mask_a, mask_b, params, workspace, workspace_bytes,
-                          out_cand, out_count, out_stats, lanes, stream, &ef);
+    mvKpFrame k{};
+    k.flow_cov = match_cov; k.mask_a = mask_a; k.mask_b = mask_b; k.workspace = workspace;
+    k.out_cand = out_cand; k.out_count = out_count; k.out_stats = out_stats;
+    k.flow = flow; k.logcov = logcov; k.disparity = disparity; k.disparity_cov = disparity_cov; k.depth = depth; k.depth_cov = depth_cov;
+    k.match_flow = match_flow; k.match_cov = match_cov; k.bad_mask = bad_mask;
+    return kp_select_frames_impl(&k, 1, lanes, params, workspace_bytes, true, cov_is_log, bl_fx, bl_fx_sq, stream);
+}
+
+extern "C" int mv_kp_select_frames(const mvKpFrame* frames, int n_frames, int lanes_per_frame, const mvKpSelectParams* params, size_t workspace_bytes,
+                                   int cov_is_log, float bl_fx, float bl_fx_sq, mvStream_t stream) {
+    MV_CHECK_ARG(frames && (n_frames == 1 || n_frames == 2));
+    const bool fuse = frames[0].flow != nullptr;
+    for (int f = 1; f < n_frames; ++f) MV_CHECK_ARG((frames[f].flow != nullptr) == fuse);
+    return kp_select_frames_impl(frames, n_frames, lanes_per_frame, params, workspace_bytes, fuse, cov_is_log, bl_fx, bl_fx_sq, stream);
 }
 
 extern "C" int mv_kp_select(const float* flow_cov, const float* depth0, const float* depth0_cov,
diff --git a/mac-vo_amd/ops.py b/mac-vo_amd/ops.py
--- a/mac-vo_amd/ops.py
+++ b/mac-vo_amd/ops.py
@@ -181,6 +181,28 @@
     return out
 
 
+def corr_lookup_frames(cost_maps: "list[torch.Tensor]", coords: "list[torch.Tensor]", radius: int = 4, outs: "list[torch.Tensor] | None" = None,
+                       tiled: bool = False) -> "list[torch.Tensor]":
+    lib = L.load()
+    n = len(cost_maps)
+    if n not in (1, 2) or len(coords) != n:
+        raise L.MacvoHipError("corr_lookup_frames: one or two frames")
+    vol16 = cost_maps[0].dtype == torch.float16
+    cost_maps = [_req(v, torch.float16 if vol16 else torch.float32, "cost_maps") for v in cost_maps]
+    coords = [_req(c, torch.float32, "coords") for c in coords]
+    B, two, H1, W1 = coords[0].shape
+    _, _, H2, W2 = cost_maps[0].shape
+    for v, c in zip(cost_maps, coords):
+        if tuple(c.shape) != (B, 2, H1, W1) or tuple(v.shape) != (B * H1 * W1, 1, H2, W2):
+            raise L.MacvoHipError("corr_lookup_frames: every frame has the same shapes, cost_maps [B*N1, 1, H2, W2] and coords [B, 2, H1, W1]")
+    K = 2 * radius + 1
+    if outs is None:
+        outs = [torch.empty((B, K * K, H1, W1), dtype=torch.float32, device=c.device) for c in coords]
+    fr = (L.mvLookupFrame * n)(*[L.mvLookupFrame(v.data_ptr(), c.data_ptr(), o.data_ptr()) for v, c, o in zip(cost_maps, coords, outs)])
+    L.check(lib.mv_corr_lookup_frames(fr, n, (2 if tiled else 0) + (1 if vol16 else 0), B, H1, W1, H2, W2, radius, _stream()), "mv_corr_lookup_frames")
+    return outs
+
+
 def fmap_tile_rows16(f: torch.Tensor, out: torch.Tensor | None = None) -> torch.Tensor:
     lib = L.load()
     if f.dtype not in (torch.float16, torch.bfloat16) or f.dim() != 4:
diff --git a/mac-vo_amd/pipeline.py b/mac-vo_amd/pipeline.py
--- a/mac-vo_amd/pipeline.py
+++ b/mac-vo_amd/pipeline.py
@@ -1424,6 +1424,10 @@
             i = 0
             lag = min(int(os.environ.get("MV_PIPE_DD_AHEAD", "2")), 6)
             clock = time.perf_counter
+            if self._pairs_ok():
+                yield from self._run_pairs(it, nxt, pose_sink, lag)
+                self.sync_all()
+                return
             while nxt is not None:
                 t0 = clock()
                 self.enqueue_frontend(nxt)
@@ -1462,5 +1466,68 @@
             yield res
         self.sync_all()
 
+    def _pairs_ok(self) -> bool:
+        return (self._pipe is not None and self.device_driven and self.cfg.keyframe_freq == 1 and self.pose_net is None
+                and getattr(self, "_map", None) is None and getattr(self, "_maps", None) is None
+                and bool(self._lib.mv_frame_pipe_pair_ok(self._pipe)))
+
+    @staticmethod
+    def _pairable(x: FrameInputs) -> bool:
+        return x.keypoints is None and x.flow8 is None and x.flow is not None and x.cov_is_log
+
+    @property
+    def pairs_enqueued(self) -> int:
+        return 0 if self._pipe is None else int(self._lib.mv_frame_pipe_pairs(self._pipe))
+
+    def _enqueue_pair(self, a: FrameInputs, b: FrameInputs) -> None:
+        for x in (a, b):
+            if x.ready is not None:
+                torch.cuda.current_stream().wait_event(x.ready)
+        ops.L.check(self._lib.mv_frame_pipe_enqueue_pair(self._pipe, ops.C.byref(self._inputs(a)), ops.C.byref(self._inputs(b)), ops._stream()),
+                    "mv_frame_pipe_enqueue_pair")
+        self._n_enq += 2
+        self._kps += [(None, None), (None, None)]
+
+    def _run_pairs(self, it, nxt, pose_sink, lag):
+        buf = [] if nxt is None else [nxt]
+        clock = time.perf_counter
+
+        def fill():
+            while len(buf) < 2:
+                x = next(it, None)
+                if x is None:
+                    return
+                buf.append(x)
+
+        ahead, i = 0, 0
+        while True:
+            fill()
+            if not buf:
+                return
+            t0 = clock()
+            a = buf.pop(0)
+            if buf and self._pairable(a) and self._pairable(buf[0]):
+                self._enqueue_pair(a, buf.pop(0))
+                n = 2
+            else:
+                self.enqueue_frontend(a)
+                n = 1
+            ahead = max(0, ahead - n)
+            fill()
+            if self._volume_ahead:
+                want = 2 if (len(buf) == 2 and self._pairable(buf[0]) and self._pairable(buf[1])) else min(1, len(buf))
+                while ahead < want:
+                    self.enqueue_volume(buf[ahead])
+                    ahead += 1
+            res = [self.finish(None, None if pose_sink is None else pose_sink[i + k]) for k in range(n)]
+            t1 = clock()
+            i += n
+            if lag >= 0:
+                ops.L.check(self._lib.mv_frame_pipe_wait_finished(self._pipe, lag), "mv_frame_pipe_wait_finished")
+            self.host_issue_s += t1 - t0
+            self.host_wait_s += clock() - t1
+            self.host_frames += n
+            yield from res
+
     def _has_pending(self) -> bool:
         return self._n_fin < self._n_enq - 1
```

New measurement: 6985. 2.6% lower.
